# google/deepvariant

Hardware: AMD Instinct MI355X
Metric: candidate pileups/sec (encode+CNN) (higher is better)
Workload: dtype u8 (encoder) / f16 MFMA, f32 accumulate (CNN); 1 GPU; configs[1] shape: synthetic 30x Illumina pileups, WGS 100x221x7, HIP encode + Inception-v3 MFMA on 1 MI355X per rank, random-init weights; parallelism=interval shards x1, all-gather of probs, collective_world_size=1

## Files before the change

deepvariant_amd/csrc/conv_common.h:

```cpp
#ifndef DV_CONV_COMMON_H_
#define DV_CONV_COMMON_H_

#include <hip/hip_runtime.h>

#include <cstddef>
#include <cstdint>

namespace dv {
namespace convk {

typedef _Float16 half8_t __attribute__((ext_vector_type(8)));
typedef _Float16 half4_t __attribute__((ext_vector_type(4)));
typedef float float16_t __attribute__((ext_vector_type(16)));

constexpr int kConvThreads = 256;
constexpr int kChunk = 16;

struct TensorGeom {
  int h, w;
  int halo;
  int hp, wp;
  int groups;
};

struct ConvBranch {
  const float* shift;
  _Float16* out;
  float* out32;
  TensorGeom og;
  int lo_groups;
  int out_goff;
  int Cout;
  int relu;
  int sub0;
  int avgpool;
};

constexpr int kMaxBranches = 4;

struct ConvArgs {
  const _Float16* in;
  const _Float16* w;
  ConvBranch br[kMaxBranches];
  int n_branches;
  TensorGeom ig;
  int N, Cin;
  int OH, OW;
  int KH, KW, stride, pad_h, pad_w;
  int M;
  int n_chunks;
  int n_slabs;
  size_t in_bytes;
  unsigned img_bytes;
  unsigned chunk_stride;
  int n_tiles;
  int band;
  int cu_pair;
  float rcp_ow, rcp_ohow;
  const int* blank_row;
  const _Float16* blank_src;
  const int* blank_need;
  int split;
  int split_tiles;
  _Float16* side_pool_out;
  TensorGeom side_pool_og;
  int side_pool_goff;
  int tile_g, tile_p;
  float rcp_tile_p;
  int wide_in;
  unsigned lo_off;
};

typedef unsigned int uint4_t __attribute__((ext_vector_type(4)));
typedef float float2_t __attribute__((ext_vector_type(2)));
typedef _Float16 half2_t __attribute__((ext_vector_type(2)));

__device__ __forceinline__ void divmod_small(int m, int d, float rcp, int& q, int& r) {
  q = static_cast<int>(static_cast<float>(m) * rcp);
  r = m - q * d;
  if (r < 0) {
    r += d;
    --q;
  }
  if (r >= d) {
    r -= d;
    ++q;
  }
}

__device__ __forceinline__ float avg_finish(float c0, float c1, float c2, float inv, float sh, bool shift_relu) {
#pragma clang fp contract(off)
  const float v = (c0 + c1 + c2) * inv;
  return shift_relu ? fmaxf(v + sh, 0.f) : v;
}

__device__ __forceinline__ void load_shifts(const float* shift, int cbase, int hi, float2_t (&shv)[4][2]) {
#pragma unroll
  for (int q = 0; q < 4; ++q) {
    float4 lo = make_float4(0.f, 0.f, 0.f, 0.f), up = lo;
    if (shift != nullptr) {
      typedef float f4_t __attribute__((ext_vector_type(4)));
      typedef const f4_t __attribute__((address_space(4))) * const_f4_ptr;
      const_f4_ptr sp = (const_f4_ptr)(reinterpret_cast<uintptr_t>(shift + (cbase + 8 * q)));
      const f4_t l4 = sp[0], u4 = sp[1];
      lo = make_float4(l4[0], l4[1], l4[2], l4[3]);
      up = make_float4(u4[0], u4[1], u4[2], u4[3]);
    }
    shv[q][0] = hi ? float2_t{up.x, up.y} : float2_t{lo.x, lo.y};
    shv[q][1] = hi ? float2_t{up.z, up.w} : float2_t{lo.z, lo.w};
  }
}

template <int PT>
__device__ __forceinline__ void epilogue_subtile(const float16_t (&acc)[PT], const ConvBranch& b, int cbase,
                                                 const int (&pn)[PT], const int (&poh)[PT], const int (&pow_)[PT],
                                                 const bool (&mvalid)[PT], int lane) {
  const int hi = lane >> 5;
  const half2_t zero2 = {static_cast<_Float16>(0.f), static_cast<_Float16>(0.f)};
  const unsigned gstride = static_cast<unsigned>(b.og.hp * b.og.wp);
  float2_t shv[4][2];
  load_shifts(b.shift, cbase, hi, shv);
  if (b.out32 != nullptr) {
#pragma unroll
    for (int pt = 0; pt < PT; ++pt) {
      const float16_t a = acc[pt];
      const unsigned obase = static_cast<unsigned>(
          ((pn[pt] * b.og.groups + b.out_goff) * b.og.hp + poh[pt] + b.og.halo) * b.og.wp + pow_[pt] + b.og.halo);
#pragma unroll
      for (int q = 0; q < 4; ++q) {
        float4 v = make_float4(a[4 * q] + shv[q][0][0], a[4 * q + 1] + shv[q][0][1], a[4 * q + 2] + shv[q][1][0],
                               a[4 * q + 3] + shv[q][1][1]);
        if (b.relu) v = make_float4(fmaxf(v.x, 0.f), fmaxf(v.y, 0.f), fmaxf(v.z, 0.f), fmaxf(v.w, 0.f));
        const int group = cbase / 8 + q;
        if (mvalid[pt] && group * 8 < b.Cout) {
          *reinterpret_cast<float4*>(b.out32 + (static_cast<size_t>(obase) + static_cast<size_t>(group) * gstride) * 8 +
                                     4 * hi) = v;
        }
      }
    }
    return;
  }
  uint4_t* outp = reinterpret_cast<uint4_t*>(b.out);
#pragma unroll
  for (int pt = 0; pt < PT; ++pt) {
    const float16_t a = acc[pt];
    const unsigned obase = static_cast<unsigned>(
        ((pn[pt] * b.og.groups + b.out_goff) * b.og.hp + poh[pt] + b.og.halo) * b.og.wp +
        pow_[pt] + b.og.halo);
    unsigned pk[4][2];
    unsigned pl[4][2];
#pragma unroll
    for (int q = 0; q < 4; ++q) {
#pragma unroll
      for (int hq = 0; hq < 2; ++hq) {
        const float2_t v = float2_t{a[4 * q + 2 * hq], a[4 * q + 2 * hq + 1]} + shv[q][hq];
        half2_t h = __builtin_convertvector(v, half2_t);
        if (b.relu) h = __builtin_elementwise_max(h, zero2);
        pk[q][hq] = __builtin_bit_cast(unsigned, h);
        if (b.lo_groups > 0) {
          const float2_t x = b.relu ? float2_t{fmaxf(v[0], 0.f), fmaxf(v[1], 0.f)} : v;
          const float2_t r = x - __builtin_convertvector(h, float2_t);
          pl[q][hq] = __builtin_bit_cast(unsigned, __builtin_convertvector(r, half2_t));
        }
      }
    }
#pragma unroll
    for (int t = 0; t < 2; ++t) {
      const auto d0 = __builtin_amdgcn_permlane32_swap(pk[2 * t][0], pk[2 * t + 1][0], false, false);
      const auto d1 = __builtin_amdgcn_permlane32_swap(pk[2 * t][1], pk[2 * t + 1][1], false, false);
      const uint4_t piece = {d0[0], d1[0], d0[1], d1[1]};
      const int group = cbase / 8 + 2 * t + hi;
#ifdef DV_ABLATE_EPI
      if (mvalid[pt] && group * 8 < b.Cout && piece[0] == 0x7e017e01u) {
#else
      if (mvalid[pt] && group * 8 < b.Cout) {
#endif
        outp[obase + static_cast<unsigned>(group) * gstride] = piece;
      }
      if (b.lo_groups > 0) {
        const auto e0 = __builtin_amdgcn_permlane32_swap(pl[2 * t][0], pl[2 * t + 1][0], false, false);
        const auto e1 = __builtin_amdgcn_permlane32_swap(pl[2 * t][1], pl[2 * t + 1][1], false, false);
        const uint4_t lo_piece = {e0[0], e1[0], e0[1], e1[1]};
        if (mvalid[pt] && group * 8 < b.Cout) {
          outp[obase + static_cast<unsigned>(group + b.lo_groups) * gstride] = lo_piece;
        }
      }
    }
  }
}

__device__ __forceinline__ int branch_of(const ConvArgs& p, int sub) {
  int bi = 0;
#pragma unroll
  for (int i = 1; i < kMaxBranches; ++i) bi += (i < p.n_branches && sub >= p.br[i].sub0) ? 1 : 0;
  return bi;
}

template <int NB, int PT>
__device__ __forceinline__ void conv_epilogue(const float16_t (&acc)[NB][PT], const ConvArgs& p,
                                              int n_tile, const int (&pn)[PT], const int (&poh)[PT],
                                              const int (&pow_)[PT], const bool (&mvalid)[PT],
                                              int lane) {
#pragma unroll
  for (int nb = 0; nb < NB; ++nb) {
    const int sub = n_tile * NB + nb;
    const ConvBranch& b = p.br[branch_of(p, sub)];
    const int cbase = (sub - b.sub0) * 32;
    if (cbase >= b.Cout) continue;
    epilogue_subtile<PT>(acc[nb], b, cbase, pn, poh, pow_, mvalid, lane);
  }
}

__device__ __forceinline__ void avg_pool_group(const float4* src, int y, int x, int H, int W, int lane, float inv,
                                               const float* shift, float (&o)[8]) {
  auto column = [&](int xc, bool wanted, float (&v)[8]) {
    float r[3][8];
#pragma unroll
    for (int dy = 0; dy < 3; ++dy) {
      const int yy = y + dy - 1;
      const bool ok = wanted && yy >= 0 && yy < H;
      float4 lo = make_float4(0.f, 0.f, 0.f, 0.f), up = lo;
      if (ok) {
        lo = src[yy * W + xc];
        up = src[256 + yy * W + xc];
      }
      r[dy][0] = lo.x; r[dy][1] = lo.y; r[dy][2] = lo.z; r[dy][3] = lo.w;
      r[dy][4] = up.x; r[dy][5] = up.y; r[dy][6] = up.z; r[dy][7] = up.w;
    }
#pragma unroll
    for (int j = 0; j < 8; ++j) v[j] = r[0][j] + r[1][j] + r[2][j];
  };
  float col[3][8];
  column(x, true, col[1]);
  const bool first = lane == 0, last = lane == 63;
  const int xe = first ? x - 1 : x + 1;
  float edge[8];
  column(xe, (first || last) && xe >= 0 && xe < W, edge);
#pragma unroll
  for (int j = 0; j < 8; ++j) {
    const int vi = __builtin_bit_cast(int, col[1][j]);
    const float from_left = __builtin_bit_cast(float, __builtin_amdgcn_update_dpp(0, vi, 0x138, 0xf, 0xf, false));
    const float from_right = __builtin_bit_cast(float, __builtin_amdgcn_update_dpp(0, vi, 0x130, 0xf, 0xf, false));
    col[0][j] = x == 0 ? 0.f : first ? edge[j] : from_left;
    col[2][j] = x == W - 1 ? 0.f : last ? edge[j] : from_right;
  }
  float sh[8] = {0, 0, 0, 0, 0, 0, 0, 0};
  if (shift != nullptr) {
    const float4 s0 = *reinterpret_cast<const float4*>(shift);
    const float4 s1 = *reinterpret_cast<const float4*>(shift + 4);
    sh[0] = s0.x; sh[1] = s0.y; sh[2] = s0.z; sh[3] = s0.w;
    sh[4] = s1.x; sh[5] = s1.y; sh[6] = s1.z; sh[7] = s1.w;
  }
#pragma unroll
  for (int j = 0; j < 8; ++j) o[j] = avg_finish(col[0][j], col[1][j], col[2][j], inv, sh[j], shift != nullptr);
}

template <int NB, int PT>
__device__ __forceinline__ void conv_epilogue_avg(const float16_t (&acc)[NB][PT], const ConvArgs& p, int n_tile,
                                                  int pix_block, const int (&pn)[PT], const int (&poh)[PT],
                                                  const int (&pow_)[PT], const bool (&mvalid)[PT], int lane,
                                                  int wave, _Float16* smem) {
  static_assert(PT == 2 && NB % 2 == 0, "256-pixel blocks, subtiles pooled in pairs");
  const int hi = lane >> 5;
  float* tile = reinterpret_cast<float*>(smem);
  const int my_slot = wave * 64 + lane;
  int il, pix, y, x;
  divmod_small(my_slot, p.tile_p, p.rcp_tile_p, il, pix);
  divmod_small(pix, p.OW, p.rcp_ow, y, x);
  const int n = pix_block * p.tile_g + il;
  const bool live = il < p.tile_g && n < p.N;
  const int H = p.OH, W = p.OW;
  const int map0 = il * p.tile_p;
  const float inv = 1.0f / static_cast<float>(((y > 0) + (y < H - 1) + 1) * ((x > 0) + (x < W - 1) + 1));
#pragma unroll
  for (int half = 0; half < NB / 2; ++half) {
    bool any_pooled = false;
#pragma unroll
    for (int nbl = 0; nbl < 2; ++nbl) {
      const int sub = n_tile * NB + 2 * half + nbl;
      const ConvBranch& b = p.br[branch_of(p, sub)];
      const int cbase = (sub - b.sub0) * 32;
      if (cbase >= b.Cout) continue;
      if (b.avgpool == 0) {
        epilogue_subtile<PT>(acc[2 * half + nbl], b, cbase, pn, poh, pow_, mvalid, lane);
      } else {
        any_pooled = true;
      }
    }
    if (!any_pooled) continue;
    __syncthreads();
#pragma unroll
    for (int nbl = 0; nbl < 2; ++nbl) {
      const int sub = n_tile * NB + 2 * half + nbl;
      const ConvBranch& b = p.br[branch_of(p, sub)];
      const int cbase = (sub - b.sub0) * 32;
      if (cbase >= b.Cout || b.avgpool == 0) continue;
#pragma unroll
      for (int pt = 0; pt < PT; ++pt) {
        const float16_t a = acc[2 * half + nbl][pt];
        const int slot = (wave * PT + pt) * 32 + (lane & 31);
#pragma unroll
        for (int q = 0; q < 4; ++q) {
          reinterpret_cast<float4*>(tile)[((nbl * 4 + q) * 2 + hi) * 256 + slot] =
              make_float4(a[4 * q], a[4 * q + 1], a[4 * q + 2], a[4 * q + 3]);
        }
      }
    }
    __syncthreads();
#pragma unroll
    for (int nbl = 0; nbl < 2; ++nbl) {
      const int sub = n_tile * NB + 2 * half + nbl;
      const ConvBranch& b = p.br[branch_of(p, sub)];
      const int cbase = (sub - b.sub0) * 32;
      if (cbase >= b.Cout || b.avgpool == 0 || !live) continue;
      const unsigned gstride = static_cast<unsigned>(b.og.hp * b.og.wp);
      const unsigned obase = static_cast<unsigned>(
          ((n * b.og.groups + b.out_goff) * b.og.hp + y + b.og.halo) * b.og.wp + x + b.og.halo);
      for (int q8 = 0; q8 < 4; ++q8) {
        const int group = cbase / 8 + q8;
        if (group * 8 >= b.Cout) break;
        const float4* src = reinterpret_cast<const float4*>(tile) + (nbl * 4 + q8) * 2 * 256 + map0;
        float o[8];
        avg_pool_group(src, y, x, H, W, lane, inv, b.shift != nullptr ? b.shift + group * 8 : nullptr, o);
        const size_t at = static_cast<size_t>(obase) + static_cast<size_t>(group) * gstride;
        if (b.out32 != nullptr) {
          float4* d = reinterpret_cast<float4*>(b.out32 + at * 8);
          d[0] = make_float4(o[0], o[1], o[2], o[3]);
          d[1] = make_float4(o[4], o[5], o[6], o[7]);
        } else {
          half8_t h;
#pragma unroll
          for (int j = 0; j < 8; ++j) h[j] = static_cast<_Float16>(o[j]);
          reinterpret_cast<uint4_t*>(b.out)[at] = __builtin_bit_cast(uint4_t, h);
          if (b.lo_groups > 0) {
            half8_t l;
#pragma unroll
            for (int j = 0; j < 8; ++j) l[j] = static_cast<_Float16>(o[j] - static_cast<float>(h[j]));
            reinterpret_cast<uint4_t*>(b.out)[at + static_cast<size_t>(b.lo_groups) * gstride] = __builtin_bit_cast(uint4_t, l);
          }
        }
      }
    }
  }
}

}
}

#endif
```

deepvariant_amd/csrc/conv_mfma.hip:

```cpp
#include <algorithm>
#include <cstdlib>
#include <type_traits>

#include "conv_mfma.h"

using namespace dv::convk;

namespace {

constexpr int prefetch_depth(int , int ) { return 4; }

struct ChunkWalk {
  int kh, kw;
  unsigned tap_off;
  unsigned chunk_off;
  __device__ __forceinline__ unsigned off() const { return chunk_off + tap_off; }
  __device__ __forceinline__ void advance(const ConvArgs& p) {
    const bool row_end = ++kw == p.KW;
    kw = row_end ? 0 : kw;
    tap_off += row_end ? static_cast<unsigned>((p.ig.wp - p.KW + 1) * 16) : 16u;
    kh += row_end ? 1 : 0;
    const bool taps_end = kh == p.KH;
    kh = taps_end ? 0 : kh;
    tap_off = taps_end ? 0u : tap_off;
// ... 18 lines not shown
__device__ __forceinline__ void conv_slab(const ConvArgs& p, const __amdgpu_buffer_rsrc_t rsrc,
                                          const _Float16* wslab, ChunkWalk& walk,
                                          const unsigned (&base)[PT],
                                          uint4_t (&xf)[prefetch_depth(NB, PT)][PT],
                                          float16_t (&acc)[NB][PT], SidePool<PT>* sp = nullptr) {
  constexpr int BN = NB * 32;
  constexpr int kPrefetch = prefetch_depth(NB, PT);
  half8_t wf[2][NB];
#pragma unroll
  for (int nb = 0; nb < NB; ++nb) {
    wf[0][nb] = *reinterpret_cast<const half8_t*>(wslab + (nb * 32) * 8);
  }
#pragma unroll
  for (int j = 0; j < R; ++j) {
#ifndef DV_ABLATE_W
    if (j + 1 < R) {
#pragma unroll
      for (int nb = 0; nb < NB; ++nb) {
        wf[(j + 1) & 1][nb] = *reinterpret_cast<const half8_t*>(
            wslab + (j + 1) * BN * kChunk + (nb * 32) * 8);
      }
    }
#else
    if (j + 1 < R) {
#pragma unroll
      for (int nb = 0; nb < NB; ++nb) wf[(j + 1) & 1][nb] = wf[j & 1][nb];
    }
#endif
    __builtin_amdgcn_sched_barrier(0);
    constexpr int kDiv = SPLIT ? 2 : 1;
    const int slot = ((S0 + j) / kDiv) % kPrefetch;
    half8_t xh[PT];
#pragma unroll
    for (int pt = 0; pt < PT; ++pt) xh[pt] = __builtin_bit_cast(half8_t, xf[slot][pt]);
#pragma unroll
    for (int nb = 0; nb < NB; ++nb) {
#pragma unroll
      for (int pt = 0; pt < PT; ++pt) {
        acc[nb][pt] =
            __builtin_amdgcn_mfma_f32_32x32x16_f16(wf[j & 1][nb], xh[pt], acc[nb][pt], 0, 0, 0);
      }
    }
    if constexpr (POOL) {
      if (sp->cc_mod == sp->my_tile) {
#pragma unroll
        for (int pt = 0; pt < PT; ++pt) sp->best[pt] = __builtin_elementwise_max(sp->best[pt], xh[pt]);
      }
      if (sp->tap == sp->taps - 1) {
        if (sp->cc < sp->n_cc && sp->cc_mod == sp->my_tile) {
          const _Float16 lowest = static_cast<_Float16>(-65504.f);
#pragma unroll
          for (int pt = 0; pt < PT; ++pt) {
            if (sp->ok[pt]) sp->out[sp->at[pt]] = __builtin_bit_cast(uint4_t, sp->best[pt]);
            sp->best[pt] = half8_t{lowest, lowest, lowest, lowest, lowest, lowest, lowest, lowest};
          }
        }
#pragma unroll
        for (int pt = 0; pt < PT; ++pt) sp->at[pt] += sp->gstride2;
        sp->tap = 0;
        ++sp->cc;
        sp->cc_mod = sp->cc_mod + 1 == sp->n_tiles ? 0 : sp->cc_mod + 1;
      } else {
        ++sp->tap;
      }
    }
    if (!SPLIT || ((S0 + j) & 1)) {
#ifndef DV_ABLATE_X
      const unsigned soff = walk.off();
#pragma unroll
      for (int pt = 0; pt < PT; ++pt) {
        xf[slot][pt] = __builtin_amdgcn_raw_buffer_load_b128(rsrc, base[pt], soff, 0);
      }
#endif
      walk.advance(p);
    }
    __builtin_amdgcn_sched_barrier(0);
  }
}

template <int NB, int PT, int R>
__device__ __forceinline__ void conv_slab_wide(const ConvArgs& p, const __amdgpu_buffer_rsrc_t rsrc,
                                               const _Float16* wslab, ChunkWalk& walk, const unsigned (&base)[PT],
                                               uint4_t (&xf)[prefetch_depth(NB, PT)][PT], float16_t (&acc)[NB][PT]) {
  constexpr int BN = NB * 32;
  static_assert(prefetch_depth(NB, PT) == 4 && R % 2 == 0, "two (hi, lo) pairs in flight");
  half8_t wf[2][NB];
#pragma unroll
  for (int nb = 0; nb < NB; ++nb) wf[0][nb] = *reinterpret_cast<const half8_t*>(wslab + (nb * 32) * 8);
#pragma unroll
  for (int j = 0; j < R; ++j) {
    if (j + 1 < R) {
#pragma unroll
      for (int nb = 0; nb < NB; ++nb) {
        wf[(j + 1) & 1][nb] = *reinterpret_cast<const half8_t*>(wslab + (j + 1) * BN * kChunk + (nb * 32) * 8);
      }
    }
    __builtin_amdgcn_sched_barrier(0);
#pragma unroll
    for (int part = 0; part < 2; ++part) {
      const int slot = (2 * j + part) & 3;
      half8_t xh[PT];
#pragma unroll
      for (int pt = 0; pt < PT; ++pt) xh[pt] = __builtin_bit_cast(half8_t, xf[slot][pt]);
#pragma unroll
      for (int nb = 0; nb < NB; ++nb) {
#pragma unroll
        for (int pt = 0; pt < PT; ++pt) {
          acc[nb][pt] = __builtin_amdgcn_mfma_f32_32x32x16_f16(wf[j & 1][nb], xh[pt], acc[nb][pt], 0, 0, 0);
        }
      }
      const unsigned soff = walk.off() + (part ? p.lo_off : 0u);
#pragma unroll
      for (int pt = 0; pt < PT; ++pt) xf[slot][pt] = __builtin_amdgcn_raw_buffer_load_b128(rsrc, base[pt], soff, 0);
      if (part) walk.advance(p);
    }
    __builtin_amdgcn_sched_barrier(0);
  }
}

template <int NB, int PT>
__device__ __forceinline__ void copy_blank_wave(const ConvArgs& p, int n_tile, const int (&pn)[PT],
                                                const int (&poh)[PT], const int (&pow_)[PT],
                                                const bool (&mvalid)[PT], int lane) {
  const ConvBranch& b = p.br[0];
  const unsigned gstride = static_cast<unsigned>(b.og.hp * b.og.wp);
  const int hi = lane >> 5;
  const uint4_t* src = reinterpret_cast<const uint4_t*>(p.blank_src);
  uint4_t* dst = reinterpret_cast<uint4_t*>(b.out);
  uint4_t v[PT][NB * 2];
  unsigned at[PT][NB * 2];
  bool ok[PT][NB * 2];
#pragma unroll
  for (int pt = 0; pt < PT; ++pt) {
    const unsigned rel = static_cast<unsigned>((poh[pt] + b.og.halo) * b.og.wp + pow_[pt] + b.og.halo);
#pragma unroll
    for (int j = 0; j < NB * 2; ++j) {
      const int g = n_tile * NB * 4 + 2 * j + hi;
      ok[pt][j] = mvalid[pt] && g * 8 < b.Cout;
      at[pt][j] = static_cast<unsigned>(b.out_goff + g) * gstride + rel;
      v[pt][j] = ok[pt][j] ? src[at[pt][j]] : uint4_t{0u, 0u, 0u, 0u};
    }
  }
#pragma unroll
  for (int pt = 0; pt < PT; ++pt) {
    const unsigned img = static_cast<unsigned>(pn[pt] * b.og.groups) * gstride;
#pragma unroll
    for (int j = 0; j < NB * 2; ++j) {
      if (ok[pt][j]) dst[img + at[pt][j]] = v[pt][j];
    }
  }
}

template <int NB, int PT, int MINB = (NB * PT >= 8 ? 1 : 2), int SLAB = kSlabChunks, int WAVES = 4,
          bool SPLIT = false, bool SIDE_POOL = false, bool AVG = false, bool WIDE = false>
__global__ __launch_bounds__(WAVES * 64, MINB) void conv_mfma_kernel(ConvArgs p) {
  constexpr int BN = NB * 32;
  constexpr int kThreads = WAVES * 64;
  constexpr int SLAB_HALFS = SLAB * BN * kChunk;
  constexpr int SLAB_PIECES = SLAB_HALFS / 8;
  constexpr int W_PER_THREAD = SLAB_PIECES / kThreads;
  static_assert(SLAB_PIECES % kThreads == 0, "slab does not split evenly over the block");
  constexpr int kPrefetch = prefetch_depth(NB, PT);
  extern __shared__ __attribute__((aligned(16))) _Float16 smem[];

  const int tid = threadIdx.x;
  const int lane = tid & 63;
  const int wave = tid >> 6;
  const int nwg = gridDim.x;
  const int xq = nwg >> 3, xr = nwg & 7;
  const int xcd = blockIdx.x & 7;
  int xi = blockIdx.x >> 3;
  if (p.cu_pair) {
    const int cnt = xcd < xr ? xq + 1 : xq;
    if (xi < cnt / 64 * 64) {
      const int w = xi & 63;
      xi = (xi & ~63) + (w & 31) * 2 + (w >> 5);
    }
  }
  const int logical = (xcd < xr ? xcd * (xq + 1) : xr * (xq + 1) + (xcd - xr) * xq) + xi;
  const int n_tile = logical % p.n_tiles;
  int pix_block = logical / p.n_tiles;
  int band_r = 0;
  if (p.band) {
    band_r = pix_block % p.band;
    pix_block /= p.band;
  }
  const int m_block = pix_block * (32 * PT * WAVES);

  int n0 = 0;
  unsigned base[PT];
  int pn[PT], poh[PT], pow_[PT];
  bool mvalid[PT];
  const int ohow = p.OH * p.OW;
#pragma unroll
  for (int pt = 0; pt < PT; ++pt) {
    const int m = m_block + (wave * PT + pt) * 32 + (lane & 31);
    int n, pix, oh, ow, iy;
    if constexpr (AVG) {
      int il;
      divmod_small((wave * PT + pt) * 32 + (lane & 31), p.tile_p, p.rcp_tile_p, il, pix);
      n = pix_block * p.tile_g + il;
      mvalid[pt] = il < p.tile_g && n < p.N;
      n = min(n, p.N - 1);
      divmod_small(pix, p.OW, p.rcp_ow, oh, ow);
      iy = oh * p.stride - p.pad_h + p.ig.halo;
    } else if (p.band) {
      mvalid[pt] = m < p.N * p.OW;
      divmod_small(mvalid[pt] ? m : 0, p.OW, p.rcp_ow, n, ow);
      oh = band_r;
      iy = p.ig.halo;
    } else {
      mvalid[pt] = m < p.M;
      divmod_small(mvalid[pt] ? m : 0, ohow, p.rcp_ohow, n, pix);
      divmod_small(pix, p.OW, p.rcp_ow, oh, ow);
      iy = oh * p.stride - p.pad_h + p.ig.halo;
    }
    const int ix = ow * p.stride - p.pad_w + p.ig.halo;
    if (pt == 0) n0 = __builtin_amdgcn_readfirstlane(n);
    base[pt] = mvalid[pt]
                   ? static_cast<unsigned>(((((n - n0) * p.ig.groups + (lane >> 5)) * p.ig.hp + iy) *
                                                p.ig.wp + ix) * 16)
                   : 0x80000000u;
    pn[pt] = n;
    poh[pt] = oh;
    pow_[pt] = ow;
  }

  bool wave_blank = false;
  if (p.blank_row != nullptr) {
    auto range_blank = [&](int m_lo, int m_hi) -> bool {
      m_hi = min(m_hi, p.M);
      if (m_lo >= m_hi) return false;
      int nf, pf, nl, pl, ohf, owf;
      divmod_small(m_lo, ohow, p.rcp_ohow, nf, pf);
      divmod_small(m_hi - 1, ohow, p.rcp_ohow, nl, pl);
      divmod_small(pf, p.OW, p.rcp_ow, ohf, owf);
      return nf == nl && ohf >= p.blank_row[nf];
    };
    if (range_blank(m_block, m_block + 32 * PT * WAVES)) {
      bool wanted = true;
      if (p.blank_need != nullptr) {
        int nf, pf, ohf, owf;
        divmod_small(m_block, ohow, p.rcp_ohow, nf, pf);
        divmod_small(pf, p.OW, p.rcp_ow, ohf, owf);
        wanted = ohf < p.blank_need[nf];
      }
      if (wanted) copy_blank_wave<NB, PT>(p, n_tile, pn, poh, pow_, mvalid, lane);
      return;
    }
    const int m_wave = m_block + wave * (32 * PT);
    wave_blank = __builtin_amdgcn_readfirstlane(range_blank(m_wave, m_wave + 32 * PT) ? 1 : 0) != 0;
  }

  const size_t in_off = static_cast<size_t>(n0) * p.img_bytes;
  const size_t in_left = p.in_bytes - in_off;
  const __amdgpu_buffer_rsrc_t rsrc = __builtin_amdgcn_make_buffer_rsrc(
      const_cast<char*>(reinterpret_cast<const char*>(p.in) + in_off), 0,
      static_cast<unsigned>(in_left < 0x7fffffffu ? in_left : 0x7fffffffu), 0x00020000);

  const uint4* wsrc = reinterpret_cast<const uint4*>(p.w) +
                      static_cast<size_t>(band_r * p.n_tiles + n_tile) * p.n_slabs * (kSlabChunks * BN * 2);
  uint4_t wreg[W_PER_THREAD];
#define DV_LOAD_SLAB(s_)                                                                   \
  {                                                                                        \
    const uint4_t* src_ = reinterpret_cast<const uint4_t*>(wsrc) +                         \
                          static_cast<size_t>(s_) * SLAB_PIECES + tid;                     \
    _Pragma("unroll") for (int j_ = 0; j_ < W_PER_THREAD; ++j_) wreg[j_] =                \
        src_[j_ * kThreads];                                                           \
  }
#define DV_STORE_SLAB(buf_)                                                                \
  {                                                                                        \
    uint4_t* dst_ = reinterpret_cast<uint4_t*>(smem + (buf_) * SLAB_HALFS) + tid;          \
    _Pragma("unroll") for (int j_ = 0; j_ < W_PER_THREAD; ++j_) dst_[j_ * kThreads] = \
        wreg[j_];                                                                          \
  }

  uint4_t xf[kPrefetch][PT];
  float16_t acc[NB][PT];
#pragma unroll
  for (int nb = 0; nb < NB; ++nb)
#pragma unroll
    for (int pt = 0; pt < PT; ++pt)
#pragma unroll
      for (int i = 0; i < 16; ++i) acc[nb][pt][i] = 0.f;

  ChunkWalk walk{0, 0, 0u, 0u};
  DV_LOAD_SLAB(0)
#pragma unroll
  for (int d = 0; d < kPrefetch; ++d) {
    const unsigned soff = walk.off() + (WIDE && (d & 1) ? p.lo_off : 0u);
#pragma unroll
    for (int pt = 0; pt < PT; ++pt) {
      xf[d][pt] = __builtin_amdgcn_raw_buffer_load_b128(rsrc, base[pt], soff, 0);
    }
    if (!WIDE || (d & 1)) walk.advance(p);
  }
  DV_STORE_SLAB(0)
  __syncthreads();

  const int frag_off = (lane >> 5) * (BN * 8) + (lane & 31) * 8;
  if (wave_blank) {
    const int n_full_b = p.n_chunks / SLAB;
    for (int s = 0; s < n_full_b; ++s) {
      const int next = s + 1 < (p.n_chunks + SLAB - 1) / SLAB ? s + 1 : s;
      DV_LOAD_SLAB(next)
      DV_STORE_SLAB((s + 1) & 1)
      __syncthreads();
    }
    copy_blank_wave<NB, PT>(p, n_tile, pn, poh, pow_, mvalid, lane);
    return;
  }
  SidePool<PT> side;
  auto k_loop = [&](auto split_tag, auto pool_tag, const int n_chunks) {
    constexpr bool S = decltype(split_tag)::value;
    constexpr bool P = decltype(pool_tag)::value;
    SidePool<PT>* const sp = P ? &side : nullptr;
    const int tile_slabs = (n_chunks + SLAB - 1) / SLAB;
#ifdef DV_ABLATE_LOOP
    const int n_full = n_chunks < 0 ? 1 : 0;
    const int rem = 0;
#else
    const int n_full = n_chunks / SLAB;
    const int rem = n_chunks - n_full * SLAB;
#endif
    for (int s = 0; s < n_full; ++s) {
      const int next = s + 1 < tile_slabs ? s + 1 : s;
      DV_LOAD_SLAB(next)
      if constexpr (WIDE) {
        conv_slab_wide<NB, PT, SLAB>(p, rsrc, smem + (s & 1) * SLAB_HALFS + frag_off, walk, base, xf, acc);
      } else {
        conv_slab<NB, PT, SLAB, 0, S, P>(p, rsrc, smem + (s & 1) * SLAB_HALFS + frag_off, walk, base, xf, acc, sp);
      }
      DV_STORE_SLAB((s + 1) & 1)
      __syncthreads();
    }
    if (rem) {
      const _Float16* wslab = smem + (n_full & 1) * SLAB_HALFS + frag_off;
      if constexpr (WIDE) {
        conv_slab_wide<NB, PT, 4>(p, rsrc, wslab, walk, base, xf, acc);
        if constexpr (SLAB > 4) {
          if (rem > 4) conv_slab_wide<NB, PT, 4>(p, rsrc, wslab + 4 * BN * kChunk, walk, base, xf, acc);
        }
      } else {
      conv_slab<NB, PT, 4, 0, S, P>(p, rsrc, wslab, walk, base, xf, acc, sp);
      if constexpr (SLAB > 4) {
        if (rem > 4) conv_slab<NB, PT, 4, 4, S, P>(p, rsrc, wslab + 4 * BN * kChunk, walk, base, xf, acc, sp);
      }
      }
    }
  };
  if constexpr (SPLIT) {
    if (n_tile < p.split_tiles) {
      k_loop(std::true_type{}, std::false_type{}, p.n_chunks);
    } else {
      k_loop(std::false_type{}, std::false_type{}, p.n_chunks >> 1);
    }
  } else if constexpr (SIDE_POOL) {
    side.tap = 0;
    side.cc = 0;
    side.cc_mod = 0;
    side.n_tiles = p.n_tiles;
    side.my_tile = n_tile;
    side.taps = p.KH * p.KW;
    side.n_cc = p.Cin / kChunk;
    side.gstride2 = 2u * static_cast<unsigned>(p.side_pool_og.hp * p.side_pool_og.wp);
    side.out = reinterpret_cast<uint4_t*>(p.side_pool_out);
#pragma unroll
    for (int pt = 0; pt < PT; ++pt) {
      const _Float16 lowest = static_cast<_Float16>(-65504.f);
      side.best[pt] = half8_t{lowest, lowest, lowest, lowest, lowest, lowest, lowest, lowest};
      side.ok[pt] = mvalid[pt];
      side.at[pt] = static_cast<unsigned>(
          ((pn[pt] * p.side_pool_og.groups + p.side_pool_goff + (lane >> 5)) * p.side_pool_og.hp + poh[pt] +
           p.side_pool_og.halo) * p.side_pool_og.wp + pow_[pt] + p.side_pool_og.halo);
    }
    k_loop(std::false_type{}, std::true_type{}, p.n_chunks);
  } else {
    k_loop(std::false_type{}, std::false_type{}, p.n_chunks);
  }
#undef DV_LOAD_SLAB
#undef DV_STORE_SLAB

  if constexpr (AVG) {
    conv_epilogue_avg<NB, PT>(acc, p, n_tile, pix_block, pn, poh, pow_, mvalid, lane, wave, smem);
  } else {
    conv_epilogue<NB, PT>(acc, p, n_tile, pn, poh, pow_, mvalid, lane);
  }
}

template <int NB, int PT>
__global__ __launch_bounds__(512, 1) void conv_resident_kernel(ConvArgs p) {
  constexpr int BN = NB * 32;
  constexpr int WAVES = 8, kThreads = WAVES * 64;
  constexpr int SLAB_HALFS = kSlabChunks * BN * kChunk;
  constexpr int kPrefetch = prefetch_depth(NB, PT);
  extern __shared__ __attribute__((aligned(16))) _Float16 smem[];
  const int tid = threadIdx.x, lane = tid & 63, wave = tid >> 6;
  const int blk = blockIdx.x;
  const int n_tile = (blk >> 3) % p.n_tiles;
  const int seq = (blk & 7) + 8 * ((blk >> 3) / p.n_tiles);
  const int n_seq = 8 * ((static_cast<int>(gridDim.x) >> 3) / p.n_tiles);
  {
    const uint4_t* wsrc = reinterpret_cast<const uint4_t*>(p.w) +
                          static_cast<size_t>(n_tile) * p.n_slabs * (kSlabChunks * BN * 2);
    uint4_t* wdst = reinterpret_cast<uint4_t*>(smem);
    const int pieces = p.n_slabs * (kSlabChunks * BN * 2);
    for (int i = tid; i < pieces; i += kThreads) wdst[i] = wsrc[i];
  }
  __syncthreads();
  const int frag_off = (lane >> 5) * (BN * 8) + (lane & 31) * 8;
  const int ohow = p.OH * p.OW;
  const int n_full = p.n_chunks / kSlabChunks;
  const int rem = p.n_chunks - n_full * kSlabChunks;
  const int n_wave_tiles = (p.M + 32 * PT - 1) / (32 * PT);
  for (int wt = seq * WAVES + wave; wt < n_wave_tiles; wt += n_seq * WAVES) {
    int n0 = 0;
    unsigned base[PT];
    int pn[PT], poh[PT], pow_[PT];
    bool mvalid[PT];
#pragma unroll
    for (int pt = 0; pt < PT; ++pt) {
      const int m = (wt * PT + pt) * 32 + (lane & 31);
      int n, pix, oh, ow;
      mvalid[pt] = m < p.M;
      divmod_small(mvalid[pt] ? m : 0, ohow, p.rcp_ohow, n, pix);
      divmod_small(pix, p.OW, p.rcp_ow, oh, ow);
      const int iy = oh * p.stride - p.pad_h + p.ig.halo;
      const int ix = ow * p.stride - p.pad_w + p.ig.halo;
      if (pt == 0) n0 = __builtin_amdgcn_readfirstlane(n);
      base[pt] = mvalid[pt]
                     ? static_cast<unsigned>(((((n - n0) * p.ig.groups + (lane >> 5)) * p.ig.hp + iy) *
                                                  p.ig.wp + ix) * 16)
                     : 0x80000000u;
      pn[pt] = n;
      poh[pt] = oh;
      pow_[pt] = ow;
    }
    const size_t in_off = static_cast<size_t>(n0) * p.img_bytes;
    const size_t in_left = p.in_bytes - in_off;
    const __amdgpu_buffer_rsrc_t rsrc = __builtin_amdgcn_make_buffer_rsrc(
        const_cast<char*>(reinterpret_cast<const char*>(p.in) + in_off), 0,
        static_cast<unsigned>(in_left < 0x7fffffffu ? in_left : 0x7fffffffu), 0x00020000);
    uint4_t xf[kPrefetch][PT];
    float16_t acc[NB][PT];
#pragma unroll
    for (int nb = 0; nb < NB; ++nb)
#pragma unroll
      for (int pt = 0; pt < PT; ++pt)
#pragma unroll
        for (int i = 0; i < 16; ++i) acc[nb][pt][i] = 0.f;
    ChunkWalk walk{0, 0, 0u, 0u};
#pragma unroll
    for (int d = 0; d < kPrefetch; ++d) {
      const unsigned soff = walk.off();
#pragma unroll
      for (int pt = 0; pt < PT; ++pt) {
        xf[d][pt] = __builtin_amdgcn_raw_buffer_load_b128(rsrc, base[pt], soff, 0);
      }
      walk.advance(p);
    }
    for (int s = 0; s < n_full; ++s) {
      conv_slab<NB, PT, kSlabChunks>(p, rsrc, smem + s * SLAB_HALFS + frag_off, walk, base, xf, acc);
    }
    if (rem) {
      const _Float16* wslab = smem + n_full * SLAB_HALFS + frag_off;
      conv_slab<NB, PT, 4>(p, rsrc, wslab, walk, base, xf, acc);
      if (rem > 4) conv_slab<NB, PT, 4, 4>(p, rsrc, wslab + 4 * BN * kChunk, walk, base, xf, acc);
    }
    conv_epilogue<NB, PT>(acc, p, n_tile, pn, poh, pow_, mvalid, lane);
  }
}

template <int NB, int PT>
__device__ __forceinline__ void resident_rows(const ConvArgs& p, const __amdgpu_buffer_rsrc_t rsrc,
                                              const _Float16* wfrag, const unsigned (&base)[PT],
                                              float16_t (&acc)[NB][PT]) {
  constexpr int BN = NB * 32;
  constexpr int SLAB_HALFS = kSlabChunks * BN * kChunk;
  constexpr int kPrefetch = prefetch_depth(NB, PT);
  const int n_full = p.n_chunks / kSlabChunks;
  const int rem = p.n_chunks - n_full * kSlabChunks;
  uint4_t xf[kPrefetch][PT];
#pragma unroll
  for (int nb = 0; nb < NB; ++nb)
#pragma unroll
    for (int pt = 0; pt < PT; ++pt)
#pragma unroll
      for (int i = 0; i < 16; ++i) acc[nb][pt][i] = 0.f;
  ChunkWalk walk{0, 0, 0u, 0u};
#pragma unroll
  for (int d = 0; d < kPrefetch; ++d) {
    const unsigned soff = walk.off();
#pragma unroll
    for (int pt = 0; pt < PT; ++pt) xf[d][pt] = __builtin_amdgcn_raw_buffer_load_b128(rsrc, base[pt], soff, 0);
    walk.advance(p);
  }
  for (int s = 0; s < n_full; ++s) {
    conv_slab<NB, PT, kSlabChunks>(p, rsrc, wfrag + s * SLAB_HALFS, walk, base, xf, acc);
  }
  if (rem) {
    const _Float16* wslab = wfrag + n_full * SLAB_HALFS;
    conv_slab<NB, PT, 4>(p, rsrc, wslab, walk, base, xf, acc);
    if (rem > 4) conv_slab<NB, PT, 4, 4>(p, rsrc, wslab + 4 * BN * kChunk, walk, base, xf, acc);
  }
}

template <int NB>
__device__ __forceinline__ void pack_row(const float16_t (&acc)[NB], const ConvArgs& p, int n_tile, int hi,
                                         unsigned (&pk)[NB][4][2]) {
  const ConvBranch& b = p.br[0];
  const half2_t zero2 = {static_cast<_Float16>(0.f), static_cast<_Float16>(0.f)};
#pragma unroll
  for (int nb = 0; nb < NB; ++nb) {
    const int cbase = (n_tile * NB + nb) * 32;
#pragma unroll
    for (int q = 0; q < 4; ++q) {
      typedef float f4_t __attribute__((ext_vector_type(4)));
      typedef const f4_t __attribute__((address_space(4))) * const_f4_ptr;
      const_f4_ptr sp = (const_f4_ptr)(reinterpret_cast<uintptr_t>(b.shift + (cbase + 8 * q)));
      const f4_t l4 = sp[0], u4 = sp[1];
      const float2_t s0 = hi ? float2_t{u4[0], u4[1]} : float2_t{l4[0], l4[1]};
      const float2_t s1 = hi ? float2_t{u4[2], u4[3]} : float2_t{l4[2], l4[3]};
      const float2_t v0 = float2_t{acc[nb][4 * q], acc[nb][4 * q + 1]} + s0;
      const float2_t v1 = float2_t{acc[nb][4 * q + 2], acc[nb][4 * q + 3]} + s1;
      pk[nb][q][0] = __builtin_bit_cast(unsigned, __builtin_elementwise_max(__builtin_convertvector(v0, half2_t), zero2));
      pk[nb][q][1] = __builtin_bit_cast(unsigned, __builtin_elementwise_max(__builtin_convertvector(v1, half2_t), zero2));
    }
  }
}

__device__ __forceinline__ unsigned pk_max(unsigned a, unsigned b) {
  return __builtin_bit_cast(unsigned, __builtin_elementwise_max(__builtin_bit_cast(half2_t, a),
                                                                __builtin_bit_cast(half2_t, b)));
}

template <int NB>
__global__ __launch_bounds__(512, 1) void conv_pool_resident_kernel(ConvArgs p) {
  constexpr int BN = NB * 32;
  constexpr int WAVES = 8, kThreads = WAVES * 64;
// ... 192 lines not shown
    for (int i = 0; i < 16; ++i) acc[nb][0][i] = 0.f;

  half8_t win[2][9];
#define DV_LOAD_WINDOW(slot_, cc_)                                                          \
  {                                                                                         \
    const unsigned so_ = static_cast<unsigned>(cc_) * p.chunk_stride;                       \
    _Pragma("unroll") for (int t_ = 0; t_ < 9; ++t_) win[slot_][t_] = __builtin_bit_cast(  \
        half8_t, __builtin_amdgcn_raw_buffer_load_b128(rsrc, base,                          \
                                                       so_ + (t_ / 3) * row_b + (t_ % 3) * 16, 0)); \
  }
  DV_LOAD_WINDOW(0, 0)
  __syncthreads();
  const _Float16* wfrag = smem + (lane >> 5) * (BN * 8) + (lane & 31) * 8;
  for (int cc = 0; cc < p.n_chunks; cc += 2) {
    if (cc + 1 < p.n_chunks) DV_LOAD_WINDOW(1, cc + 1)
#pragma unroll
    for (int half = 0; half < 2; ++half) {
      if (half == 1) {
        if (cc + 1 >= p.n_chunks) break;
        if (cc + 2 < p.n_chunks) DV_LOAD_WINDOW(0, cc + 2)
      }
      half8_t x = win[half][0];
#pragma unroll
      for (int t = 1; t < 9; ++t) x = __builtin_elementwise_max(x, win[half][t]);
      const _Float16* wc = wfrag + (cc + half) * (BN * kChunk);
#pragma unroll
      for (int nb = 0; nb < NB; ++nb) {
        const half8_t wf = *reinterpret_cast<const half8_t*>(wc + nb * 32 * 8);
        acc[nb][0] = __builtin_amdgcn_mfma_f32_32x32x16_f16(wf, x, acc[nb][0], 0, 0, 0);
      }
    }
  }
#undef DV_LOAD_WINDOW
  conv_epilogue<NB, PT>(acc, p, n_tile, pn, poh, pow_, mvalid, lane);
}

template <int NB>
constexpr size_t conv_lds_bytes() {
  return static_cast<size_t>(2) * kSlabChunks * NB * 32 * kChunk * 2;
}

void launch_conv6(const ConvArgs& a, hipStream_t stream) {
  const long rows = a.band ? a.band : 1;
  const long row_px = a.band ? static_cast<long>(a.N) * a.OW : a.M;
  const long blocks = rows * ((row_px + 127) / 128) * a.n_tiles;
  constexpr size_t lds = static_cast<size_t>(2) * 4 * 192 * kChunk * 2;
  if (a.wide_in) {
    hipLaunchKernelGGL((conv_mfma_kernel<6, 1, 2, 4, 4, false, false, false, true>), dim3(static_cast<unsigned>(blocks)),
                       dim3(kConvThreads), lds, stream, a);
    return;
  }
  hipLaunchKernelGGL((conv_mfma_kernel<6, 1, 2, 4>), dim3(static_cast<unsigned>(blocks)), dim3(kConvThreads), lds,
                     stream, a);
}

template <int NB>
void launch_conv(const ConvArgs& a, hipStream_t stream) {
  const int n_tiles = a.n_tiles;
  const long rows = a.band ? a.band : 1;
  const long row_px = a.band ? static_cast<long>(a.N) * a.OW : a.M;
  auto blocks = [&](int px) { return rows * ((row_px + px - 1) / px) * n_tiles; };
  const long blocks2 = blocks(256);
  if constexpr (NB == 4) {
    if (a.side_pool_out != nullptr) {
      if (blocks2 >= 512) {
        hipLaunchKernelGGL((conv_mfma_kernel<NB, 2, 2, kSlabChunks, 4, false, true>), dim3(static_cast<unsigned>(blocks2)),
                           dim3(kConvThreads), conv_lds_bytes<NB>(), stream, a);
      } else {
        hipLaunchKernelGGL((conv_mfma_kernel<NB, 1, 2, kSlabChunks, 4, false, true>), dim3(static_cast<unsigned>(blocks(128))),
                           dim3(kConvThreads), conv_lds_bytes<NB>(), stream, a);
      }
      return;
    }
  }
  if (a.wide_in) {
    if constexpr (NB >= 2 && NB <= 4) {
      if constexpr (NB == 4) {
        if (a.tile_g > 0) {
          const long tiles = (static_cast<long>(a.N) + a.tile_g - 1) / a.tile_g * n_tiles;
          hipLaunchKernelGGL((conv_mfma_kernel<NB, 2, 2, kSlabChunks, 4, false, false, true, true>),
                             dim3(static_cast<unsigned>(tiles)), dim3(kConvThreads), conv_lds_bytes<NB>(), stream, a);
          return;
        }
      }
      if (blocks2 >= 512) {
        hipLaunchKernelGGL((conv_mfma_kernel<NB, 2, 2, kSlabChunks, 4, false, false, false, true>),
                           dim3(static_cast<unsigned>(blocks2)), dim3(kConvThreads), conv_lds_bytes<NB>(), stream, a);
      } else {
        hipLaunchKernelGGL((conv_mfma_kernel<NB, 1, 2, kSlabChunks, 4, false, false, false, true>),
                           dim3(static_cast<unsigned>(blocks(128))), dim3(kConvThreads), conv_lds_bytes<NB>(), stream, a);
      }
      return;
    }
  }
  if constexpr (NB == 4) {
    if (a.tile_g > 0) {
      const long tiles = (static_cast<long>(a.N) + a.tile_g - 1) / a.tile_g * n_tiles;
      hipLaunchKernelGGL((conv_mfma_kernel<NB, 2, 2, kSlabChunks, 4, false, false, true>),
                         dim3(static_cast<unsigned>(tiles)), dim3(kConvThreads), conv_lds_bytes<NB>(), stream, a);
      return;
    }
  }
  if (a.split) {
    static const long pt2_min = getenv("DV_SPLIT_PT2_MIN") ? atol(getenv("DV_SPLIT_PT2_MIN")) : 256;
    if (blocks2 >= pt2_min) {
      hipLaunchKernelGGL((conv_mfma_kernel<NB, 2, 2, kSlabChunks, 4, true>), dim3(static_cast<unsigned>(blocks2)),
                         dim3(kConvThreads), conv_lds_bytes<NB>(), stream, a);
    } else {
      hipLaunchKernelGGL((conv_mfma_kernel<NB, 1, 2, kSlabChunks, 4, true>), dim3(static_cast<unsigned>(blocks(128))),
                         dim3(kConvThreads), conv_lds_bytes<NB>(), stream, a);
    }
    return;
  }
  static const int force_pt = getenv("DV_CONV_PT") ? atoi(getenv("DV_CONV_PT")) : 0;
  static const bool no_pt4 = getenv("DV_NO_PT4") != nullptr;
  if constexpr (NB <= 2) {
    if (!no_pt4 && !force_pt && blocks2 >= 4096 && (NB == 1 || a.KH * a.KW >= 25)) {
      hipLaunchKernelGGL((conv_mfma_kernel<NB, 4>), dim3(static_cast<unsigned>(blocks(512))),
                         dim3(kConvThreads), conv_lds_bytes<NB>(), stream, a);
      return;
    }
  }
  static const bool slab4 = getenv("DV_CONV_SLAB4") != nullptr;
  static const bool w8 = getenv("DV_CONV_W8") != nullptr;
  if constexpr (NB >= 3 && NB <= 4) {
    if (slab4 && blocks2 >= 512) {
      hipLaunchKernelGGL((conv_mfma_kernel<NB, 2, 2, 4>), dim3(static_cast<unsigned>(blocks2)),
                         dim3(kConvThreads), static_cast<size_t>(2) * 4 * NB * 32 * kChunk * 2, stream, a);
      return;
    }
    if (w8 && blocks2 >= 1024) {
      hipLaunchKernelGGL((conv_mfma_kernel<NB, 2, 1, kSlabChunks, 8>), dim3(static_cast<unsigned>(blocks(512))),
                         dim3(512), conv_lds_bytes<NB>(), stream, a);
      return;
    }
  }
  if (force_pt ? force_pt == 2 : blocks2 >= 512) {
    if constexpr (NB == 4) {
      static const bool two = getenv("DV_CONV42_BLOCKS") == nullptr || atoi(getenv("DV_CONV42_BLOCKS")) != 1;
      if (two) {
        hipLaunchKernelGGL((conv_mfma_kernel<NB, 2, 2>), dim3(static_cast<unsigned>(blocks2)),
                           dim3(kConvThreads), conv_lds_bytes<NB>(), stream, a);
        return;
      }
    }
    hipLaunchKernelGGL((conv_mfma_kernel<NB, 2>), dim3(static_cast<unsigned>(blocks2)),
                       dim3(kConvThreads), conv_lds_bytes<NB>(), stream, a);
  } else {
    hipLaunchKernelGGL((conv_mfma_kernel<NB, 1>), dim3(static_cast<unsigned>(blocks(128))),
                       dim3(kConvThreads), conv_lds_bytes<NB>(), stream, a);
  }
}

}
namespace dv {
namespace convk {


template <typename K>
static void allow_big_lds(K kernel) {
  (void)hipFuncSetAttribute(reinterpret_cast<const void*>(kernel), hipFuncAttributeMaxDynamicSharedMemorySize, 160 * 1024);
}

void launch_conv_pool_resident(const ConvArgs& a, int n_cus, hipStream_t stream) {
  static const bool attr = (allow_big_lds(conv_pool_resident_kernel<3>), true);
  (void)attr;
  const long frags = (static_cast<long>(a.N) * a.OW + 29) / 30;
  const int per_set = 8 * a.n_tiles;
  const long want = (frags + 8 * 8 - 1) / (8 * 8) * per_set;
  const int grid = static_cast<int>(std::max<long>(per_set, std::min<long>(want, n_cus / per_set * per_set)));
  hipLaunchKernelGGL((conv_pool_resident_kernel<3>), dim3(grid), dim3(512), resident_lds_bytes(a), stream, a);
}

void launch_conv_pool1x1(const ConvArgs& a, int nb, hipStream_t stream) {
  const size_t lds = static_cast<size_t>(a.n_slabs) * kSlabChunks * nb * 32 * kChunk * 2;
  const dim3 grid(static_cast<unsigned>(((a.M + 127) / 128) * a.n_tiles));
  switch (nb) {
    case 7: {
      static const bool attr = (allow_big_lds(conv_pool1x1_kernel<7, 8>), true);
      (void)attr;
      hipLaunchKernelGGL((conv_pool1x1_kernel<7, 8>), dim3(static_cast<unsigned>((a.M + 255) / 256)), dim3(512), lds, stream, a);
      break;
    }
    case 1: hipLaunchKernelGGL((conv_pool1x1_kernel<1>), grid, dim3(kConvThreads), lds, stream, a); break;
    case 2: hipLaunchKernelGGL((conv_pool1x1_kernel<2>), grid, dim3(kConvThreads), lds, stream, a); break;
    case 3: hipLaunchKernelGGL((conv_pool1x1_kernel<3>), grid, dim3(kConvThreads), lds, stream, a); break;
    default: hipLaunchKernelGGL((conv_pool1x1_kernel<4>), grid, dim3(kConvThreads), lds, stream, a); break;
  }
}

void launch_conv_resident(const ConvArgs& a, int n_cus, hipStream_t stream) {
  static const bool attr = (allow_big_lds(conv_resident_kernel<3, 2>), true);
  (void)attr;
  const int grid = n_cus / (8 * a.n_tiles) * (8 * a.n_tiles);
  hipLaunchKernelGGL((conv_resident_kernel<3, 2>), dim3(grid), dim3(512), resident_lds_bytes(a), stream, a);
}

void launch_conv(const ConvArgs& a, int nb, hipStream_t stream) {
  switch (nb) {
    case 1: ::launch_conv<1>(a, stream); break;
    case 2: ::launch_conv<2>(a, stream); break;
    case 3: ::launch_conv<3>(a, stream); break;
    case 6: launch_conv6(a, stream); break;
    default: ::launch_conv<4>(a, stream); break;
  }
}

}
}
```

deepvariant_amd/csrc/model.hip:

```cpp
#include <algorithm>
#include <map>
#include <atomic>
#include <cmath>
#include <cstdlib>
#include <cstring>
#include <memory>
#include <thread>

#include <hip/hip_fp16.h>

#include "model_graph.h"
#include "model_kernels.h"
#include "block35.h"
#include "mixed3.h"
#include "chain.h"
#include "stem_fused.h"
#include "calib.h"
#include "layer_export.h"

namespace {

static int stem_sub_batch() {
  static const int v = getenv("DV_STEM_SB") ? std::max(1, atoi(getenv("DV_STEM_SB"))) : (1 << 30);
  return v;
}

ExtPtrs* ext_table(const dv_model* m) { return static_cast<ExtPtrs*>(m->d_ext.ptr); }

struct OpTrace {
  hipEvent_t a, b;
  std::string label;
  double flops, bytes;
};
std::vector<OpTrace>* g_trace = nullptr;

struct TraceScope {
  hipStream_t stream;
  bool on;
  TraceScope(hipStream_t s, std::string label, double flops, double bytes) : stream(s), on(g_trace != nullptr) {
    if (!on) return;
    OpTrace t{nullptr, nullptr, std::move(label), flops, bytes};
    (void)hipEventCreate(&t.a);
    (void)hipEventCreate(&t.b);
    (void)hipEventRecord(t.a, stream);
    g_trace->push_back(std::move(t));
  }
  ~TraceScope() {
    if (on) (void)hipEventRecord(g_trace->back().b, stream);
  }
};

void dump_trace(hipStream_t stream) {
  (void)hipStreamSynchronize(stream);
  double tot = 0;
  for (OpTrace& t : *g_trace) {
    float ms = 0;
    (void)hipEventElapsedTime(&ms, t.a, t.b);
    tot += ms;
    fprintf(stderr, "[dv-op] %-58s %8.1f us %7.1f TF/s %7.0f GB/s\n", t.label.c_str(), ms * 1e3,
            t.flops / (ms * 1e-3) / 1e12, t.bytes / (ms * 1e-3) / 1e9);
    (void)hipEventDestroy(t.a);
    (void)hipEventDestroy(t.b);
  }
  fprintf(stderr, "[dv-op] total %.1f us\n", tot * 1e3);
  g_trace->clear();
}

bool resident_ok(const dv_model* m, const Op& op, const ConvArgs& a) {
  const char* env = getenv("DV_RESIDENT");
  const int mode = env ? atoi(env) : 1;
  if (mode == 0 || op.nb != 3 || op.band || op.v2 || op.pool_in || op.split || a.blank_row != nullptr || a.wide_in) return false;
  if (resident_lds_bytes(a) > 150 * 1024 || m->n_cus < 8 * a.n_tiles) return false;
  static const long min_tiles = getenv("DV_RESIDENT_MIN_TILES") ? atol(getenv("DV_RESIDENT_MIN_TILES")) : 4;
  if (static_cast<long>(a.M) < static_cast<long>(m->n_cus) * 8 * 64 * min_tiles) return false;
  if (mode >= 2) return true;
  return m->blank_conv4_op >= 0 && &op == &m->ops[m->blank_conv4_op];
}

struct Pass {
  dv_model* m;
  int n;
  hipStream_t stream;
  int first, last;
  int shifted_buf, out_example_off;
  size_t images_off;
  std::vector<char> side_pooled;
  _Float16* out_ptr(int buf) const {
    const size_t halfs = static_cast<size_t>(out_example_off) * m->buffers[buf].bytes_per_example() / 2;
    return m->buf_ptr(buf) + (buf == shifted_buf ? halfs : 0);
  }
};

dv::C8Geom c8_geom(const BufferDesc& b) {
  const TensorGeom g = b.geom();
  return dv::C8Geom{g.h, g.w, g.halo, g.hp, g.wp, g.groups};
}


int enqueue_stem_a(const Pass& ps, int oi) {
  const dv_model* m = ps.m;
  const int n = ps.n;
  const Op &op = m->ops[oi], &c2 = m->ops[oi + 1];
  dv::StemAArgs a{};
  a.in = nullptr;
  a.in_ind = &ext_table(m)->images;
  a.in_off = ps.images_off;
  a.w1 = m->w_ptr(op);
  a.w2 = m->w_ptr(c2);
  a.shift1 = m->shift_ptr(op);
  a.shift2 = m->shift_ptr(c2);
  a.out = m->buf_ptr(c2.out_buf);
  a.og = c8_geom(m->buffers[c2.out_buf]);
  a.N = n;
  a.H = op.ih;
  a.W = op.iw;
  a.C = op.cin_real;
  a.OH1 = op.oh;
  a.OW1 = op.ow;
  a.OH2 = c2.oh;
  a.OW2 = c2.ow;
  a.tiles_y = (c2.oh + dv::kStemA_TH - 1) / dv::kStemA_TH;
  a.tiles_x = (c2.ow + dv::kStemA_TW - 1) / dv::kStemA_TW;
  a.total_tiles = n * a.tiles_y * a.tiles_x;
  a.in_bytes = static_cast<unsigned>(static_cast<size_t>(n) * op.ih * op.iw * op.cin_real);
  if (m->blank_on()) {
    a.blank_thr = m->blank_thr(1);
    a.blank_src = static_cast<const _Float16*>(m->d_blank_c2.ptr);
    a.blank_need = m->blank_thr(5);
  }
  TraceScope tr(ps.stream, std::string(m->blank_on() ? "[blank tiles copied] " : "") + "stem_a conv3x3s2 " + std::to_string(op.cin_real) + "->32 + conv3x3 32->32 (fused)",
                2.0 * n * (static_cast<double>(op.oh) * op.ow * op.kh * op.kw * op.cin_real * op.cout +
                           static_cast<double>(c2.oh) * c2.ow * 9 * 32 * 32),
                static_cast<double>(n) * (op.ih * op.iw * op.cin_real + 2.0 * c2.oh * c2.ow * 32));
  dv::ProfileScope prof(dv::kProfConv, ps.stream);
  dv::launch_stem_a(a, m->stem_a_grid, ps.stream);
  return 2;
}

void report_stem_b_profile(dv::StemBArgs a, int grid, hipStream_t stream) {
  const size_t words = static_cast<size_t>(grid) * 16;
  unsigned long long* d = nullptr;
  if (hipMalloc(&d, words * 8) != hipSuccess) return;
  (void)hipMemsetAsync(d, 0, words * 8, stream);
  a.prof = d;
  dv::launch_stem_b(a, grid, stream);
  std::vector<unsigned long long> h(words);
  (void)hipStreamSynchronize(stream);
  (void)hipMemcpy(h.data(), d, words * 8, hipMemcpyDeviceToHost);
  (void)hipFree(d);
  for (int w = 0; w < 2; ++w) {
    double sum[7] = {0, 0, 0, 0, 0, 0, 0};
    for (int b = 0; b < grid; ++b)
      for (int i = 0; i < 7; ++i) sum[i] += static_cast<double>(h[(b * 2 + w) * 8 + i]);
    const double tiles = static_cast<double>(a.total_tiles);
    fprintf(stderr, "[dv-stem-b wave %d] cycles/tile: issue %.0f conv3 %.0f dma-wait %.0f barrierA %.0f pool %.0f "
                    "barrierB %.0f conv1x1+store %.0f\n", w ? 7 : 0, sum[0] / tiles, sum[1] / tiles,
            sum[6] / tiles, sum[2] / tiles, sum[3] / tiles, sum[4] / tiles, sum[5] / tiles);
  }
  std::map<unsigned long long, std::vector<int>> where;
  for (int b = 0; b < grid; ++b) {
    const unsigned long long v = h[(b * 2) * 8 + 7];
    const unsigned hw = static_cast<unsigned>(v), xcc = static_cast<unsigned>(v >> 32);
    where[(static_cast<unsigned long long>(xcc) << 16) | ((hw >> 8) & 0xffu)].push_back(b);
  }
  int pairs = 0, same_parity = 0, apart256 = 0;
  for (const auto& kv : where) {
    if (kv.second.size() != 2) continue;
    ++pairs;
    const unsigned t0 = (static_cast<unsigned>(h[(kv.second[0] * 2) * 8 + 7]) >> 16) & 15u;
    const unsigned t1 = (static_cast<unsigned>(h[(kv.second[1] * 2) * 8 + 7]) >> 16) & 15u;
    same_parity += (t0 & 1u) == (t1 & 1u);
    apart256 += kv.second[1] - kv.second[0] == 256;
  }
  fprintf(stderr, "[dv-stem-b placement] %zu places for %d workgroups; %d pairs, %d with TG slots of EQUAL parity, "
                  "%d pairs are blocks b / b+256\n", where.size(), grid, pairs, same_parity, apart256);
  for (int cls = 0; cls < 2; ++cls) {
    double sum[7] = {0, 0, 0, 0, 0, 0, 0};
    int nb = 0;
    for (int b = 0; b < grid; ++b) {
      const unsigned tg = (static_cast<unsigned>(h[(b * 2) * 8 + 7]) >> 16) & 15u;
      if (static_cast<int>(tg & 1u) != cls) continue;
      ++nb;
      for (int i = 0; i < 7; ++i) sum[i] += static_cast<double>(h[(b * 2) * 8 + i]);
    }
    double tot = 0;
    for (double v : sum) tot += v;
    fprintf(stderr, "[dv-stem-b TG parity %d] %d workgroups, share of wave-0 cycles: issue %.3f conv3 %.3f dma-wait %.3f "
                    "barrierA %.3f pool %.3f barrierB %.3f conv1x1+store %.3f; cycles per workgroup %.0f\n", cls, nb,
            sum[0] / tot, sum[1] / tot, sum[6] / tot, sum[2] / tot, sum[3] / tot, sum[4] / tot, sum[5] / tot,
            nb ? tot / nb : 0.0);
  }
}

int enqueue_stem_b(const Pass& ps, int oi) {
  const dv_model* m = ps.m;
  const int n = ps.n;
  const Op &op = m->ops[oi], &c4 = m->ops[oi + 1];
  const BufferDesc& ib = m->buffers[op.in_buf];
  dv::StemBArgs a{};
  a.in = m->buf_ptr(op.in_buf);
  a.w3 = m->w_ptr(op);
  a.w4 = m->w_ptr(c4);
  a.shift3 = m->shift_ptr(op);
  a.shift4 = m->shift_ptr(c4);
  a.out = m->buf_ptr(c4.out_buf);
  a.ig = c8_geom(ib);
  a.og = c8_geom(m->buffers[c4.out_buf]);
  a.N = n;
  a.OH3 = op.oh;
  a.OW3 = op.ow;
  a.PH = c4.oh;
  a.PW = c4.ow;
  a.Cout4 = c4.cout;
  a.tiles_y = (c4.oh + dv::kStemB_PH - 1) / dv::kStemB_PH;
  a.tiles_x = (c4.ow + dv::kStemB_PW - 1) / dv::kStemB_PW;
  a.total_tiles = n * a.tiles_y * a.tiles_x;
  a.in_bytes = static_cast<size_t>(n) * ib.bytes_per_example();
  a.in_img_bytes = static_cast<unsigned>(ib.bytes_per_example());
  if (m->blank_on()) {
    a.blank_thr = m->blank_thr(2);
    a.blank_src = static_cast<const _Float16*>(m->d_blank_b.ptr);
    a.blank_need = m->blank_thr(6);
  }
  TraceScope tr(ps.stream, std::string(m->blank_on() ? "[blank tiles copied] " : "") + "stem_b conv3x3 32->64 + maxpool3s2 + conv1x1 64->" + std::to_string(c4.cout) + " (fused)",
                2.0 * n * (static_cast<double>(op.oh) * op.ow * 9 * 32 * 64 +
                           static_cast<double>(c4.oh) * c4.ow * 64 * c4.cout),
                2.0 * n * (static_cast<double>(op.ih) * op.iw * 32 + static_cast<double>(c4.oh) * c4.ow * c4.cout));
  dv::ProfileScope prof(dv::kProfConv, ps.stream);
  static const bool stem_prof = getenv("DV_STEM_PROF") != nullptr;
  if (stem_prof && g_trace != nullptr) {
    report_stem_b_profile(a, m->stem_b_grid, ps.stream);
  } else {
    dv::launch_stem_b(a, m->stem_b_grid, ps.stream);
  }
  return 2;
}

int enqueue_block35(const Pass& ps, int oi) {
  const dv_model* m = ps.m;
// ... 128 lines not shown
                    "lds epilogue %.0f hbm epilogue %.0f set-up %.0f\n", w, sum[0] / tiles, sum[1] / tiles,
            sum[2] / tiles, sum[3] / tiles, sum[4] / tiles, sum[5] / tiles);
  }
}

int enqueue_chain(const Pass& ps, int oi) {
  const dv_model* m = ps.m;
  const int n = ps.n;
  const Op& op = m->ops[oi];
  const Op& last = m->ops[oi + op.chain_len - 1];
  const BufferDesc& ib = m->buffers[op.in_buf];
  dv::ChainArgs a{};
  a.in = m->buf_ptr(op.in_buf);
  a.ig = ib.geom();
  a.in_img_bytes = static_cast<unsigned>(ib.bytes_per_example());
  a.N = n;
  a.G = op.chain_g;
  a.tpx = op.chain_tpx;
  a.h = op.oh;
  a.w = op.ow;
  a.n_tiles = (n + a.G - 1) / a.G;
  a.n_layers = op.chain_len;
  double tr_flops = 0;
  std::string tr_label = "chain";
  size_t act = 0, slot = 0;
  for (int k = 0; k < op.chain_len; ++k) {
    const Op& o = m->ops[oi + k];
    dv::ChainLayer& cl = a.L[k];
    cl.w = m->w_ptr(o);
    cl.shift = m->shift_ptr(o);
    cl.n_chunks = o.cin / kChunk;
    cl.cout = o.cout;
    cl.cout_pad = (o.cout + 31) / 32 * 32;
    cl.kh = o.kh;
    cl.kw = o.kw;
    cl.slab_bytes = static_cast<unsigned>(o.kh * o.kw * 2 * cl.cout_pad * 16);
    act = std::max(act, static_cast<size_t>(o.cin / 8) * op.chain_tpx * 16);
    slot = std::max(slot, static_cast<size_t>(cl.slab_bytes));
    tr_flops += 2.0 * n * o.oh * o.ow * o.kh * o.kw * o.cin * o.cout;
    tr_label += " " + std::to_string(o.kh) + "x" + std::to_string(o.kw) + ":" + std::to_string(o.cin) + "->" +
                std::to_string(o.cout);
  }
  a.act_bytes = static_cast<unsigned>(act);
  a.slot_bytes = static_cast<unsigned>(slot);
  a.out = m->buf_ptr(last.out_buf);
  a.og = m->buffers[last.out_buf].geom();
  a.out_goff = last.out_coff / 8;
  tr_label += " @" + std::to_string(op.oh) + "x" + std::to_string(op.ow) + " [fused, G=" + std::to_string(a.G) + "]";
  TraceScope tr(ps.stream, tr_label, tr_flops,
                2.0 * n * op.oh * op.ow * (static_cast<double>(op.cin) + last.cout));
  dv::ProfileScope prof(dv::kProfConv, ps.stream);
  static const bool chain_prof = getenv("DV_CHAIN_PROF") != nullptr;
  if (chain_prof && g_trace != nullptr) {
    report_chain_profile(a, m->n_cus, ps.stream);
  } else {
    dv::launch_chain(a, m->n_cus, ps.stream);
  }
  return op.chain_len;
}

int enqueue_first_conv(const Pass& ps, int oi) {
  const dv_model* m = ps.m;
  const int n = ps.n;
  const Op& op = m->ops[oi];
  FirstConvArgs f{};
  f.ext = ext_table(m);
  f.in_off = ps.images_off;
  f.w = m->w_ptr(op);
  f.shift = m->shift_ptr(op);
  f.out = ps.out_ptr(op.out_buf);
  f.og = m->buffers[op.out_buf].geom();
  f.N = n;
  f.H = op.ih;
  f.W = op.iw;
  f.C = op.cin_real;
  f.Cout = op.cout;
  f.OH = op.oh;
  f.OW = op.ow;
  f.KH = op.kh;
  f.KW = op.kw;
  f.stride = op.stride;
  f.M = n * op.oh * op.ow;
  f.n_chunks = op.n_chunks;
  f.wide = op.cin_real > 8 ? 1 : 0;
  f.in_bytes = static_cast<unsigned>(static_cast<size_t>(n) * op.ih * op.iw * op.cin_real);
  f.rcp_ow = 1.0f / static_cast<float>(op.ow);
  f.rcp_ohow = 1.0f / static_cast<float>(op.oh * op.ow);
  TraceScope tr(ps.stream, "conv_first_u8 3x3 s2 " + std::to_string(op.cin_real) + "->" + std::to_string(op.cout),
                2.0 * f.M * op.kh * op.kw * op.cin_real * op.cout,
                static_cast<double>(n) * (op.ih * op.iw * op.cin_real + 2.0 * op.oh * op.ow * op.cout));
  dv::ProfileScope prof(dv::kProfConv, ps.stream);
  launch_conv_first_u8(f, ps.stream);
  return 1;
}

void set_branch_output(const Pass& ps, const Op& o, ConvBranch& br) {
  const BufferDesc& b = ps.m->buffers[o.out_buf];
  br.out = ps.out_ptr(o.out_buf);
  br.out32 = b.f32 ? ps.m->buf_ptr<float>(o.out_buf) : nullptr;
  br.og = b.geom();
  br.lo_groups = b.wide ? b.c / 8 : 0;
  br.out_goff = o.out_coff / 8;
}

int enqueue_conv(Pass& ps, int oi) {
  const dv_model* m = ps.m;
  const int n = ps.n;
  const Op& op = m->ops[oi];
  ConvArgs a{};
  a.in = m->buf_ptr(op.in_buf);
  const BufferDesc& ib = m->buffers[op.in_buf];
  a.ig = ib.geom();
  a.N = n;
  a.Cin = op.cin;
  a.OH = op.oh;
  a.OW = op.ow;
  static const int cu_pair = getenv("DV_CU_PAIR") ? atoi(getenv("DV_CU_PAIR")) : 0;
  a.cu_pair = cu_pair;
  a.band = op.band;
  a.KH = op.band ? op.band : op.kh;
  a.KW = op.kw;
  a.stride = op.stride;
  a.pad_h = op.pad_h;
  a.pad_w = op.pad_w;
  a.chunk_stride = static_cast<unsigned>(2 * a.ig.hp * a.ig.wp * 16);
  a.M = n * op.oh * op.ow;
  a.n_chunks = op.n_chunks;
  a.n_slabs = op.n_steps;
  a.split = op.split ? 1 : 0;
  a.split_tiles = op.split_tiles;
  a.wide_in = op.in_wide ? 1 : 0;
  a.lo_off = op.in_wide ? static_cast<unsigned>(ib.c / 8) * static_cast<unsigned>(a.ig.hp * a.ig.wp) * 16u : 0u;
  a.in_bytes = static_cast<size_t>(n) * ib.bytes_per_example();
  a.img_bytes = static_cast<unsigned>(ib.bytes_per_example());
  a.rcp_ow = 1.0f / static_cast<float>(op.ow);
  a.rcp_ohow = 1.0f / static_cast<float>(op.oh * op.ow);
  int subs = 0;
  a.n_branches = 0;
  double tr_flops = 0, tr_bytes = static_cast<double>(n) * op.ih * op.iw * op.cin * 2.0;
  std::string tr_label = "conv " + std::to_string(op.kh) + "x" + std::to_string(op.kw) + " s" +
                         std::to_string(op.stride) + " " + std::to_string(op.cin) + "->";
  for (int gi = 0; gi <= op.group_followers; ++gi) {
    const Op& bo = m->ops[oi + gi];
    tr_flops += 2.0 * n * op.oh * op.ow * op.kh * op.kw * op.cin_real * bo.cout;
    tr_bytes += 2.0 * n * op.oh * op.ow * bo.cout;
    tr_label += (gi ? "+" : "") + std::to_string(bo.cout);
    ConvBranch& br = a.br[a.n_branches++];
    br.shift = bo.raw ? nullptr : m->shift_ptr(bo);
    set_branch_output(ps, bo, br);
    br.Cout = bo.cout;
    br.relu = bo.raw ? 0 : 1;
    br.sub0 = subs;
    subs += (bo.cout + 31) / 32;
    if (op.avg_tile_g > 0 && bo.avg_partner >= 0 && bo.avg_partner < ps.last) {
      const Op& pl = m->ops[bo.avg_partner];
      br.avgpool = 1;
      br.shift = m->shift_ptr(pl);
      br.relu = 1;
      set_branch_output(ps, pl, br);
      a.tile_g = op.avg_tile_g;
      a.tile_p = op.oh * op.ow;
      a.rcp_tile_p = 1.0f / static_cast<float>(a.tile_p);
    }
  }
  if (a.tile_g > 0) tr_label += " [+ avgpool3s1 in the epilogue, " + std::to_string(a.tile_g) + " maps per block]";
  a.w = m->w_ptr(op);
  const int tiles = (subs + op.nb - 1) / op.nb;
  a.n_tiles = tiles;
  if (m->blank_on() && m->blank_conv4_op >= 0 && &op == &m->ops[m->blank_conv4_op] &&
      a.n_branches == 1 && !op.band && !op.v2 && !op.pool_in) {
    a.blank_row = m->blank_thr(op.pool_out ? 4 : 3);
    a.blank_src = static_cast<const _Float16*>(m->d_blank_conv4.ptr);
    tr_label += " [blank rows copied]";
  }
  if (m->blank_on() && oi == 1 && !m->ops[0].stem_a && a.n_branches == 1 && !op.band && !op.v2 && !op.pool_in &&
      !op.pool_out && !op.split && op.nb <= 4 && m->d_blank_c2.ptr != nullptr) {
    a.blank_row = m->blank_thr(1);
    a.blank_src = static_cast<const _Float16*>(m->d_blank_c2.ptr);
    if (m->ops[2].stem_b) a.blank_need = m->blank_thr(5);
    tr_label += " [blank rows copied]";
  }
  const int oi_last = oi + op.group_followers;
  tr_label += " @" + std::to_string(op.oh) + "x" + std::to_string(op.ow) + " nb" + std::to_string(op.nb) +
              " tiles" + std::to_string(tiles);
  if (op.pool_in) tr_label += " <- maxpool3s2";
  if (op.in_wide) tr_label += " [hi+lo input: 2 MFMAs per weight fragment]";
  if (op.v2) tr_label += " [imgconv G=" + std::to_string(op.v2_g) + "]";
  if (op.band) tr_label += " [band: " + std::to_string(op.band) + " of " + std::to_string(op.kh) + " tap rows]";
  if (op.split) tr_label += " [split W: " + std::to_string(op.split_tiles) + " of " + std::to_string(tiles) + " tiles]";
  if (op.side_pool_partner > oi_last && op.side_pool_partner < ps.last && op.nb == 4 && !resident_ok(m, op, a)) {
    const Op& pl = m->ops[op.side_pool_partner];
    a.side_pool_out = m->buf_ptr(pl.out_buf);
    a.side_pool_og = m->buffers[pl.out_buf].geom();
    a.side_pool_goff = pl.out_coff / 8;
    ps.side_pooled[op.side_pool_partner] = 1;
    tr_label += " + maxpool3s2 on the side";
    tr_bytes += 2.0 * n * pl.oh * pl.ow * pl.cin;
  }
  const bool resident = !op.v2 && !op.pool_in && !op.pool_out && resident_ok(m, op, a);
  if (resident) tr_label += " [weights resident in LDS]";
  if (op.pool_out) tr_label += " [weights resident in LDS] -> maxpool3s2";
  TraceScope tr(ps.stream, tr_label, tr_flops, tr_bytes);
  dv::ProfileScope prof(dv::kProfConv, ps.stream);
  if (op.pool_out) {
    launch_conv_pool_resident(a, m->n_cus, ps.stream);
  } else if (op.v2) {
    dv::ImgConvArgs ia = m->imgconv_geometry(op, op.v2_g);
    ia.c = a;
    ia.n_img_tiles = (n + op.v2_g - 1) / op.v2_g;
    ia.n_cout_tiles = op.v2_tiles;
    dv::launch_imgconv(ia, op.nb, m->n_cus, ps.stream);
  } else if (op.pool_in) {
    a.stride = 2;
    launch_conv_pool1x1(a, op.nb, ps.stream);
  } else if (resident) {
    launch_conv_resident(a, m->n_cus, ps.stream);
  } else {
    launch_conv(a, op.nb, ps.stream);
  }
  return op.group_followers + 1;
}

int enqueue_pool(const Pass& ps, int oi) {
  const dv_model* m = ps.m;
  const int n = ps.n;
  const Op& op = m->ops[oi];
  const BufferDesc &ib = m->buffers[op.in_buf], &ob = m->buffers[op.out_buf];
  PoolArgs p{};
  p.in = m->buf_ptr(op.in_buf);
  p.in32 = m->buf_ptr<float>(op.in_buf);
  p.out = ps.out_ptr(op.out_buf);
  p.out32 = ob.f32 ? m->buf_ptr<float>(op.out_buf) : nullptr;
  p.lo_in_groups = ib.wide ? ib.c / 8 : 0;
  p.lo_out_groups = ob.wide ? ob.c / 8 : 0;
  p.ig = ib.geom();
  p.og = ob.geom();
  p.N = n;
  p.C = op.cin;
  p.OH = op.oh;
  p.OW = op.ow;
  p.out_goff = op.out_coff / 8;
  p.shift = op.pool_shift_relu ? m->shift_ptr(op) : nullptr;
  TraceScope tr(ps.stream, std::string(op.type == kOpMaxPool ? "maxpool3s2 " : "avgpool3s1 ") +
                               std::to_string(op.cin) + " @" + std::to_string(op.oh) + "x" + std::to_string(op.ow),
                0.0, 2.0 * n * op.cin * (static_cast<double>(op.ih) * op.iw + op.oh * op.ow));
  dv::ProfileScope prof(dv::kProfOther, ps.stream);
  if (op.type == kOpMaxPool) {
    if (ib.f32 || ob.f32) return dv::fail(DV_ERR_UNSUPPORTED, "max-pool of a float32 tensor");
    launch_maxpool3s2(p, ps.stream);
  } else {
    if (!ib.f32) return dv::fail(DV_ERR_UNSUPPORTED, "average pool of an fp16 tensor");
    launch_avgpool3s1(p, ps.stream);
  }
  return 1;
}

int run_ops(dv_model* m, int first, int last, int n, hipStream_t stream,
            int shifted_buf = -1, int out_example_off = 0, size_t images_off = 0) {
  Pass ps{m, n, stream, first, last, shifted_buf, out_example_off, images_off, std::vector<char>(m->ops.size(), 0)};
  for (int oi = first; oi < last;) {
    const Op& op = m->ops[oi];
    int ran = 1;
    if (ps.side_pooled[oi]) {
    } else if (op.type == kOpAvgPool && op.avg_partner >= 0 && m->ops[op.avg_partner].avg_partner == oi &&
               op.avg_partner >= first) {
    } else if (op.type != kOpConv) {
      ran = enqueue_pool(ps, oi);
    } else if (op.stem_a) {
      ran = enqueue_stem_a(ps, oi);
    } else if (op.stem_b) {
      ran = enqueue_stem_b(ps, oi);
    } else if (op.b35 == 1) {
      ran = enqueue_block35(ps, oi);
    } else if (op.m3 == 1) {
      ran = enqueue_mixed3(ps, oi);
    } else if (op.chain_len > 0) {
      ran = enqueue_chain(ps, oi);
    } else if (op.first_u8) {
      ran = enqueue_first_conv(ps, oi);
    } else {
      ran = enqueue_conv(ps, oi);
    }
    if (ran < 0) return ran;
    oi += ran;
  }
  DV_HIP_CHECK(hipGetLastError());
  return DV_OK;
}

}

extern "C" {

int dv_model_create(const dv_model_desc* desc, int device, dv_model** out) {
  if (!desc || !out) return dv::fail(DV_ERR_INVALID_ARGUMENT, "dv_model_create: null");
  if (desc->channels < 1 || desc->channels > 16 || desc->num_classes < 1 ||
      desc->num_classes > 8 || desc->max_batch < 1 || desc->max_batch > 8192 ||
      desc->height < 75 ||
      desc->width < 75) {
    return dv::fail(DV_ERR_INVALID_ARGUMENT,
                    "dv_model_create: unsupported shape (need H,W >= 75, C <= 16, max_batch <= 8192)");
  }
  int n_dev = 0;
  if (hipGetDeviceCount(&n_dev) != hipSuccess || n_dev <= 0) {
    return dv::fail(DV_ERR_NO_DEVICE, "no HIP device: libdvhip has no CPU fallback");
  }
  if (device < 0 || device >= n_dev) {
    return dv::fail(DV_ERR_INVALID_ARGUMENT, "bad device ordinal");
  }
  DV_HIP_CHECK(hipSetDevice(device));
  std::unique_ptr<dv_model> m(new dv_model());
  m->device = device;
  m->desc = *desc;
  m->precise = getenv("DV_PRECISE") != nullptr ? atoi(getenv("DV_PRECISE")) != 0 : desc->channels > 8;
  m->build();
  m->stem_a_grid = dv::stem_a_blocks(device);
  m->stem_b_grid = dv::stem_b_blocks(device);
  m->n_cus = dv::stem_a_blocks(device) / 2;
  for (const Op& op : m->ops) {
    const BufferDesc& ob = m->buffers[op.out_buf];
    const double pieces = static_cast<double>(desc->max_batch) * ob.bytes_per_example() / 16.0;
    const double pixels = static_cast<double>(desc->max_batch) * op.oh * op.ow;
    if (pieces >= 2147483648.0 || pixels >= 67108864.0) {
      return dv::fail(DV_ERR_INVALID_ARGUMENT,
                      "dv_model_create: max_batch too large for this image size (N*OH*OW must stay "
                      "below 2^26 and every activation tensor below 2^31 16-byte pieces)");
    }
  }
  if (static_cast<double>(desc->max_batch) * desc->height * desc->width * desc->channels >=
      2147483648.0) {
    return dv::fail(DV_ERR_INVALID_ARGUMENT, "dv_model_create: max_batch * H * W * C must be < 2^31");
  }
  m->dbuf.resize(m->buffers.size());
  for (size_t i = 0; i < m->buffers.size(); ++i) {
    const BufferDesc& b = m->buffers[i];
    const bool stem_buf = static_cast<int>(i) < m->stem_out_buf;
    const size_t examples = std::max(
        static_cast<size_t>(stem_buf ? std::min(desc->max_batch, stem_sub_batch()) : desc->max_batch),
        static_cast<size_t>(b.min_examples));
    const size_t bytes = examples * b.bytes_per_example() +
                         static_cast<size_t>(8) * (b.h + 2 * b.halo) * (b.w + 2 * b.halo) * 16;
    if (int rc = m->dbuf[i].reserve(bytes)) return rc;
    DV_HIP_CHECK(hipMemset(m->dbuf[i].ptr, 0, m->dbuf[i].cap));
  }
  if (int rc = m->d_w.reserve(m->packed_halfs * 2)) return rc;
  if (int rc = m->d_shift.reserve(m->shift_floats * 4)) return rc;
  if (int rc = m->d_dense_w.reserve(static_cast<size_t>(m->feat_c) * desc->num_classes * 4)) return rc;
  if (int rc = m->d_dense_b.reserve(desc->num_classes * 4)) return rc;
  if (int rc = m->d_ext.reserve(sizeof(ExtPtrs))) return rc;
  if (!(getenv("DV_BLANK_SKIP") != nullptr && atoi(getenv("DV_BLANK_SKIP")) == 0) &&
      m->ops[0].first_u8 && m->blank_conv4_op >= 0 && m->ops[m->blank_conv4_op].group_followers == 0 &&
      (static_cast<size_t>(desc->height) * desc->width * desc->channels) % 4 == 0) {
    if (int rc = m->d_blank_thr.reserve(static_cast<size_t>(7) * desc->max_batch * sizeof(int))) return rc;
    DV_HIP_CHECK(hipMemset(m->d_blank_thr.ptr, 0, m->d_blank_thr.cap));
    m->blank_skip = true;
  }
  *out = m.release();
  return DV_OK;
}

void dv_model_destroy(dv_model* m) {
  if (!m) return;
  (void)hipSetDevice(m->device);
  for (auto& b : m->dbuf) b.release();
  m->d_w.release();
  m->d_shift.release();
  m->d_dense_w.release();
  m->d_dense_b.release();
  m->d_tbl.release();
  m->d_blank_thr.release();
  m->d_ext.release();
  m->d_blank_conv4.release();
  m->d_blank_c2.release();
  m->d_blank_b.release();
  for (auto& g : m->graphs) (void)hipGraphExecDestroy(g.exec);
  delete m;
}

int64_t dv_model_num_params(const dv_model* m) { return m ? m->n_params : 0; }

int64_t dv_model_conv_macs(const dv_model* m) {
  if (!m) return 0;
  int64_t macs = 0;
  for (const Op& op : m->ops) {
    if (op.type == kOpConv) {
      macs += static_cast<int64_t>(op.kh) * op.kw * op.cin_real * op.cout * op.oh * op.ow;
    }
  }
  return macs;
}

int dv_model_num_layers(const dv_model* m) {
  return m ? static_cast<int>(m->layers.size()) : 0;
}

int dv_model_layer_info(const dv_model* m, int layer, int32_t* kh, int32_t* kw,
                        int32_t* cin, int32_t* cout, int64_t* param_offset) {
  if (!m || layer < 0 || layer >= static_cast<int>(m->layers.size())) {
    return dv::fail(DV_ERR_INVALID_ARGUMENT, "dv_model_layer_info: bad layer");
  }
  const LayerInfo& l = m->layers[layer];
  if (kh) *kh = l.kh;
  if (kw) *kw = l.kw;
  if (cin) *cin = l.cin;
  if (cout) *cout = l.cout;
  if (param_offset) *param_offset = l.param_off;
  return DV_OK;
}

struct HeadOutputs {
  float* pooled;
  float* logits;
};
static int enqueue_forward(dv_model* m, int n, hipStream_t stream, const HeadOutputs* head_out = nullptr);
static void set_ext(dv_model* m, const uint8_t* images, float* probs, hipStream_t stream,
                    const int32_t* rows_hint = nullptr, int rows_add = 0) {
  launch_set_ext(ext_table(m), images, probs, rows_hint, rows_add, stream);
}

static int prepare_blank_responses(dv_model* m) {
  m->blank_ready = false;
  if (!m->blank_skip) return DV_OK;
  for (auto& g : m->graphs) {
    (void)hipStreamSynchronize(g.stream);
    (void)hipGraphExecDestroy(g.exec);
  }
  m->graphs.clear();
  const size_t img_bytes = static_cast<size_t>(m->desc.height) * m->desc.width * m->desc.channels;
  dv::DeviceBuffer zero_img, probs;
  int rc = zero_img.reserve(img_bytes);
  if (rc == DV_OK) rc = probs.reserve(sizeof(float) * m->desc.num_classes);
  if (rc == DV_OK && hipMemset(zero_img.ptr, 0, img_bytes) != hipSuccess) rc = dv::fail(DV_ERR_HIP, "hipMemset");
  if (rc == DV_OK) {
    set_ext(m, static_cast<const uint8_t*>(zero_img.ptr), static_cast<float*>(probs.ptr), nullptr);
    rc = enqueue_forward(m, 1, nullptr);
  }
  if (rc == DV_OK && hipDeviceSynchronize() != hipSuccess) rc = dv::fail(DV_ERR_HIP, "blank forward failed");
  auto keep = [&](int buf, dv::DeviceBuffer* dst) {
    if (rc != DV_OK || buf < 0 || m->buffers[buf].h <= 1) return;
    const size_t bytes = m->buffers[buf].bytes_per_example();
    rc = dst->reserve(bytes);
    if (rc == DV_OK && hipMemcpy(dst->ptr, m->dbuf[buf].ptr, bytes, hipMemcpyDeviceToDevice) != hipSuccess) {
      rc = dv::fail(DV_ERR_HIP, "copying the blank response");
    }
  };
  keep(m->ops[m->blank_conv4_op].out_buf, &m->d_blank_conv4);
  keep(m->ops[1].out_buf, &m->d_blank_c2);
  if (m->ops[2].stem_b) keep(m->ops[3].out_buf, &m->d_blank_b);
  zero_img.release();
  probs.release();
  if (rc != DV_OK) return rc;
  m->blank_ready = true;
  return DV_OK;
}

int dv_model_load_weights(dv_model* m, const float* weights, int64_t n) {
  if (!m || !weights) return dv::fail(DV_ERR_INVALID_ARGUMENT, "dv_model_load_weights: null");
  if (n != m->n_params) {
    return dv::fail(DV_ERR_INVALID_ARGUMENT,
                    "dv_model_load_weights: expected " + std::to_string(m->n_params) +
                        " values, got " + std::to_string(n));
  }
  DV_HIP_CHECK(hipSetDevice(m->device));
  std::vector<_Float16> packed(m->packed_halfs, static_cast<_Float16>(0.f));
  std::vector<float> shift(m->shift_floats, 0.f);
  for (const Op& op : m->ops) {
    if (op.type != kOpConv) continue;
    const LayerInfo& l = m->layers[op.layer];
    const float* var = weights + l.param_off + static_cast<size_t>(l.kh) * l.kw * l.cin * l.cout + 2 * l.cout;
    for (int co = 0; co < l.cout; ++co) {
      if (!(var[co] + 1e-3f > 0.f)) return dv::fail(DV_ERR_BAD_INPUT, "non-positive BatchNorm variance");
    }
  }
  auto pack_op = [&](size_t oi) {
    const Op& op = m->ops[oi];
    if (op.type != kOpConv) return;
    const LayerInfo& l = m->layers[op.layer];
    const float* w = weights + l.param_off;
    const size_t wn = static_cast<size_t>(l.kh) * l.kw * l.cin * l.cout;
    const float* beta = w + wn;
    const float* mean = beta + l.cout;
    const float* var = mean + l.cout;
    std::vector<float> inv(l.cout);
    for (int co = 0; co < l.cout; ++co) {
      inv[co] = 1.0f / std::sqrt(var[co] + 1e-3f);
      shift[op.shift_off + co] = beta[co] - mean[co] * inv[co];
    }
    if ((m->ops[0].stem_a && oi < 2) || (m->ops[2].stem_b && (oi == 2 || oi == 3))) {
      _Float16* dst = packed.data() + op.w_off;
      if (oi == 0 && l.cin > 8) dv::pack_stem_a_w1_wide(w, inv.data(), l.cin, dst);
      if (oi == 0 && l.cin <= 8) dv::pack_stem_a_w1(w, inv.data(), l.cin, dst);
      if (oi == 1) dv::pack_stem_a_w2(w, inv.data(), dst);
      if (oi == 2) dv::pack_stem_b_w3(w, inv.data(), dst);
      if (oi == 3) dv::pack_stem_b_w4(w, inv.data(), l.cout, dst);
      return;
    }
    if (op.first_u8) {
      const bool wide = l.cin > 8;
      for (int kc = 0; kc < op.n_chunks; ++kc)
        for (int g = 0; g < 2; ++g) {
          const int tap = wide ? kc : 2 * kc + g;
          if (tap >= op.kh * op.kw) continue;
          const int kh = tap / op.kw, kw = tap % op.kw;
          for (int co = 0; co < op.cout; ++co)
            for (int ci = wide ? 8 * g : 0; ci < (wide ? std::min(l.cin, 8 * g + 8) : l.cin); ++ci) {
              const float v = w[((static_cast<size_t>(kh) * l.kw + kw) * l.cin + ci) * l.cout + co];
              packed[op.w_off + ((static_cast<size_t>(kc) * 2 + g) * 32 + co) * 8 + (ci & 7)] =
                  static_cast<_Float16>(v * inv[co]);
            }
        }
      return;
    }
    if (op.b35 >= 1 && op.b35 <= 4) {
      const int pass = op.b35 == 1 || op.b35 == 4 ? 1 : 0, base = op.b35 == 1 || op.b35 == 2 ? 0 : 64;
      const int n_chunks = l.cin / kChunk;
      _Float16* dst = packed.data() + op.w_off;
      for (int cc = 0; cc < n_chunks; ++cc)
        for (int co = 0; co < op.cout; ++co)
          for (int jj = 0; jj < kChunk; ++jj) {
            const float v = w[static_cast<size_t>(cc * kChunk + jj) * l.cout + co];
            dst[(((static_cast<size_t>(pass) * n_chunks + cc) * 2 + jj / 8) * 128 + base + co) * 8 + (jj % 8)] =
                static_cast<_Float16>(v * inv[co]);
          }
      return;
    }
    if (op.m3 == 1) {
      _Float16* dst = packed.data() + op.w_off;
      for (int cc = 0; cc < l.cin / kChunk; ++cc)
        for (int co = 0; co < op.cout; ++co)
          for (int jj = 0; jj < kChunk; ++jj) {
            const float v = w[static_cast<size_t>(cc * kChunk + jj) * l.cout + co];
            dst[((static_cast<size_t>(cc) * 2 + jj / 8) * dv::kMixed3Red + co) * 8 + (jj % 8)] = static_cast<_Float16>(v * inv[co]);
          }
      return;
    }
    if (op.chain_len > 0 || op.in_chain || op.b35 >= 5 || op.m3 >= 2) {
      const int cout_pad = (op.cout + 31) / 32 * 32, taps = op.kh * op.kw;
      _Float16* dst = packed.data() + op.w_off;
      for (int cc = 0; cc < l.cin / kChunk; ++cc)
        for (int tap = 0; tap < taps; ++tap) {
          const int kh = tap / op.kw, kw = tap % op.kw;
          for (int co = 0; co < op.cout; ++co)
            for (int jj = 0; jj < kChunk; ++jj) {
              const int ci = cc * kChunk + jj;
              const float v = w[((static_cast<size_t>(kh) * l.kw + kw) * l.cin + ci) * l.cout + co];
              dst[(((static_cast<size_t>(cc) * taps + tap) * 2 + jj / 8) * cout_pad + co) * 8 + (jj % 8)] =
                  static_cast<_Float16>(v * inv[co]);
            }
        }
      return;
    }
    int sub0 = 0;
    {
      size_t lead = oi;
      while (lead > 0 && m->ops[lead].group_followers == 0 && m->ops[lead - 1].type == kOpConv &&
             m->ops[lead - 1].w_off == op.w_off) {
        --lead;
      }
      for (size_t j = lead; j < oi; ++j) sub0 += (m->ops[j].cout + 31) / 32;
    }
    const int bn = op.nb * 32;
    const int taps = op.kh * op.kw;
    {
      size_t lead = oi;
      while (lead > 0 && m->ops[lead].group_followers == 0 && m->ops[lead - 1].type == kOpConv &&
             m->ops[lead - 1].w_off == op.w_off) {
        --lead;
// ... 97 lines not shown
      c.pad_h = op.pad_h;
      c.pad_w = op.pad_w;
      c.cin = op.cin_real;
      c.cout = op.cout;
      c.w_off = m->layers[op.layer].param_off;
      c.raw = op.raw;
      c.shift_off = static_cast<int64_t>(op.shift_off);
      c.split = op.split_rows;
      c.keep_f32 = m->buffers[op.out_buf].f32 || m->buffers[op.out_buf].wide ? 1 : 0;
      if (op.pool_in) {
        plan.bufs[op.in_buf].h = op.ih;
        plan.bufs[op.in_buf].w = op.iw;
      }
      if (op.pool_out) {
        oh = (oh - 3) / 2 + 1;
        ow = (ow - 3) / 2 + 1;
      }
    } else if (op.type == kOpAvgPool) {
      c.shift_relu = op.pool_shift_relu;
      if (op.pool_shift_relu) c.shift_off = static_cast<int64_t>(op.shift_off);
      c.cout = op.cout;
      c.keep_f32 = m->buffers[op.out_buf].f32 || m->buffers[op.out_buf].wide ? 1 : 0;
    } else {
      c.cout = op.cout;
    }
    plan.bufs[op.out_buf].h = oh;
    plan.bufs[op.out_buf].w = ow;
    plan.ops.push_back(c);
  }
  plan.feat_buf = m->feat_buf;
  plan.num_classes = m->desc.num_classes;
  plan.dense_off = m->layers.back().param_off;
  return plan;
}

int dv_model_calibrate(dv_model* m, const float* weights, int64_t n_weights, const uint8_t* images, int n_images,
                       float* corrections, int64_t capacity) {
  if (!m || !weights || !images) return dv::fail(DV_ERR_INVALID_ARGUMENT, "dv_model_calibrate: null");
  if (!m->loaded) return dv::fail(DV_ERR_INVALID_ARGUMENT, "dv_model_calibrate: load weights first");
  if (n_weights != m->n_params) return dv::fail(DV_ERR_INVALID_ARGUMENT, "dv_model_calibrate: wrong number of weights");
  if (n_images < 1 || n_images > 4096) return dv::fail(DV_ERR_INVALID_ARGUMENT, "dv_model_calibrate: 1..4096 images");
  const dv::CalibPlan plan = calib_plan_of(m);
  std::vector<float> corr, dense_corr;
  if (int rc = dv::run_calibration(plan, m->device, weights, n_weights, m->h_shift, images, n_images, &corr,
                                   &dense_corr)) {
    return rc;
  }
  std::vector<float> shift = m->h_shift, dense_b = m->h_dense_b;
  for (size_t i = 0; i < shift.size(); ++i) shift[i] -= corr[i];
  for (size_t k = 0; k < dense_b.size(); ++k) dense_b[k] -= dense_corr[k];
  DV_HIP_CHECK(hipSetDevice(m->device));
  DV_HIP_CHECK(hipDeviceSynchronize());
  DV_HIP_CHECK(hipMemcpy(m->d_shift.ptr, shift.data(), shift.size() * 4, hipMemcpyHostToDevice));
  DV_HIP_CHECK(hipMemcpy(m->d_dense_b.ptr, dense_b.data(), dense_b.size() * 4, hipMemcpyHostToDevice));
  if (corrections != nullptr) {
    int64_t at = 0;
    for (size_t off : m->correction_shift_offsets()) {
      if (at < capacity) corrections[at++] = corr[off];
    }
    for (size_t k = 0; k < dense_corr.size() && at < capacity; ++k) corrections[at++] = dense_corr[k];
  }
  return prepare_blank_responses(m);
}

int dv_model_apply_corrections(dv_model* m, const float* corrections, int64_t n) {
  if (!m || !corrections) return dv::fail(DV_ERR_INVALID_ARGUMENT, "dv_model_apply_corrections: null");
  if (!m->loaded) return dv::fail(DV_ERR_INVALID_ARGUMENT, "dv_model_apply_corrections: load weights first");
  const std::vector<size_t> offs = m->correction_shift_offsets();
  if (n != static_cast<int64_t>(offs.size() + m->h_dense_b.size())) return dv::fail(DV_ERR_INVALID_ARGUMENT, "dv_model_apply_corrections: wrong number of corrections");
  for (int64_t i = 0; i < n; ++i) {
    if (!std::isfinite(corrections[i])) return dv::fail(DV_ERR_BAD_INPUT, "dv_model_apply_corrections: non-finite correction");
  }
  std::vector<float> shift = m->h_shift, dense_b = m->h_dense_b;
  int64_t at = 0;
  for (size_t off : offs) shift[off] -= corrections[at++];
  for (size_t k = 0; k < dense_b.size(); ++k) dense_b[k] -= corrections[at++];
  DV_HIP_CHECK(hipSetDevice(m->device));
  DV_HIP_CHECK(hipDeviceSynchronize());
  DV_HIP_CHECK(hipMemcpy(m->d_shift.ptr, shift.data(), shift.size() * 4, hipMemcpyHostToDevice));
  DV_HIP_CHECK(hipMemcpy(m->d_dense_b.ptr, dense_b.data(), dense_b.size() * 4, hipMemcpyHostToDevice));
  return prepare_blank_responses(m);
}

int dv_model_num_ops(const dv_model* m) { return m ? static_cast<int>(m->ops.size()) : 0; }

int dv_model_op_label(const dv_model* m, int op_index, char* buf, int capacity) {
  if (!m || !buf || capacity < 1 || op_index < 0 || op_index >= static_cast<int>(m->ops.size())) {
    return dv::fail(DV_ERR_INVALID_ARGUMENT, "dv_model_op_label: bad argument");
  }
  const Op& op = m->ops[op_index];
  const char* kind = op.type == kOpConv ? "conv" : op.type == kOpMaxPool ? "maxpool" : "avgpool";
  snprintf(buf, static_cast<size_t>(capacity), "%s layer=%d k=%dx%d s=%d cin=%d cout=%d out=%dx%d raw=%d in_buf=%d out_buf=%d coff=%d lds_only=%d",
           kind, op.layer, op.kh, op.kw, op.stride, op.cin, op.cout, op.oh, op.ow, op.raw ? 1 : 0, op.in_buf, op.out_buf,
           op.out_coff, (op.type == kOpConv && (op.stem_a || op.stem_b)) || (op_index + 1 < static_cast<int>(m->ops.size()) && m->ops[op_index + 1].in_chain && m->ops[op_index + 1].in_buf == op.out_buf) ||
               (op.b35 >= 2 && op.b35 <= 4) || op.b35 == 6 || op.m3 == 1 || op.m3 == 2 ? 1 : 0);
  return DV_OK;
}

int dv_model_probe_rounding(dv_model* m, const float* weights, int64_t n_weights, const uint8_t* images, int n_images,
                            const uint8_t* keep_f32, int flags, const float* corrections, int64_t n_corrections,
                            float* logits_r, float* logits_e, float* corrections_out) {
  if (!m || !weights || !images || !logits_e) return dv::fail(DV_ERR_INVALID_ARGUMENT, "dv_model_probe_rounding: null");
  if (!m->loaded) return dv::fail(DV_ERR_INVALID_ARGUMENT, "dv_model_probe_rounding: load weights first");
  if (n_weights != m->n_params) return dv::fail(DV_ERR_INVALID_ARGUMENT, "dv_model_probe_rounding: wrong number of weights");
  if (n_images < 1 || n_images > 4096) return dv::fail(DV_ERR_INVALID_ARGUMENT, "dv_model_probe_rounding: 1..4096 images");
  dv::CalibPlan plan = calib_plan_of(m);
  if (keep_f32 != nullptr) {
    for (size_t i = 0; i < plan.ops.size(); ++i) plan.ops[i].keep_f32 = keep_f32[i] ? 1 : 0;
  }
  std::vector<float> corr_in(m->h_shift.size(), 0.f), dense_in(m->h_dense_b.size(), 0.f);
  if (corrections != nullptr) {
    const std::vector<size_t> offs = m->correction_shift_offsets();
    if (n_corrections != static_cast<int64_t>(offs.size() + dense_in.size())) return dv::fail(DV_ERR_INVALID_ARGUMENT, "dv_model_probe_rounding: wrong number of corrections");
    int64_t at = 0;
    for (size_t off : offs) corr_in[off] = corrections[at++];
    for (size_t k = 0; k < dense_in.size(); ++k) dense_in[k] = corrections[at++];
  }
  const bool measure = (flags & 2) != 0;
  if (measure && corrections != nullptr) return dv::fail(DV_ERR_INVALID_ARGUMENT, "dv_model_probe_rounding: measure or apply");
  dv::CalibProbe probe;
  probe.corr_in = measure ? nullptr : corr_in.data();
  probe.dense_corr_in = measure ? nullptr : dense_in.data();
  probe.logits_r = logits_r;
  probe.logits_e = logits_e;
  probe.skip_r = logits_r == nullptr && !measure;
  probe.weights_f32 = (flags & 1) != 0;
  std::vector<float> corr, dense_corr;
  if (int rc = dv::run_calibration(plan, m->device, weights, n_weights, m->h_shift, images, n_images, &corr, &dense_corr,
                                   &probe)) {
    return rc;
  }
  if (corrections_out != nullptr) {
    int64_t at = 0;
    for (size_t off : m->correction_shift_offsets()) corrections_out[at++] = corr[off];
    for (float v : dense_corr) corrections_out[at++] = v;
  }
  return DV_OK;
}

int dv_model_debug_tensor(dv_model* m, int index, int n, void* host_out, int32_t* h,
                          int32_t* w, int32_t* c) {
  if (m && index == -1) index = m->feat_buf;
  if (m && index == -2) index = m->stem_out_buf;
  if (!m || index < 0 || index >= static_cast<int>(m->buffers.size())) {
    return dv::fail(DV_ERR_INVALID_ARGUMENT, "dv_model_debug_tensor: bad index");
  }
  const BufferDesc& b = m->buffers[index];
  if (h) *h = b.h + 2 * b.halo;
  if (w) *w = b.w + 2 * b.halo;
  if (c) *c = b.c;
  if (host_out) {
    DV_HIP_CHECK(hipSetDevice(m->device));
    DV_HIP_CHECK(hipDeviceSynchronize());
    if (b.f32) {
      std::vector<float> tmp(static_cast<size_t>(n) * b.bytes_per_example() / 4);
      DV_HIP_CHECK(hipMemcpy(tmp.data(), m->dbuf[index].ptr, tmp.size() * 4, hipMemcpyDeviceToHost));
      _Float16* dst = static_cast<_Float16*>(host_out);
      for (size_t i = 0; i < tmp.size(); ++i) dst[i] = static_cast<_Float16>(tmp[i]);
    } else if (b.wide) {
      const size_t half_halfs = b.bytes_per_example() / 4;
      std::vector<_Float16> tmp(static_cast<size_t>(n) * half_halfs * 2);
      DV_HIP_CHECK(hipMemcpy(tmp.data(), m->dbuf[index].ptr, tmp.size() * 2, hipMemcpyDeviceToHost));
      _Float16* dst = static_cast<_Float16*>(host_out);
      for (int e = 0; e < n; ++e)
        for (size_t i = 0; i < half_halfs; ++i) {
          dst[static_cast<size_t>(e) * half_halfs + i] = static_cast<_Float16>(
              static_cast<float>(tmp[static_cast<size_t>(e) * 2 * half_halfs + i]) +
              static_cast<float>(tmp[static_cast<size_t>(e) * 2 * half_halfs + half_halfs + i]));
        }
    } else {
      DV_HIP_CHECK(hipMemcpy(host_out, m->dbuf[index].ptr,
                             static_cast<size_t>(n) * b.bytes_per_example(),
                             hipMemcpyDeviceToHost));
    }
  }
  return DV_OK;
}

static int enqueue_forward(dv_model* m, int n, hipStream_t stream, const HeadOutputs* head_out) {
  const size_t img_bytes = static_cast<size_t>(m->desc.height) * m->desc.width * m->desc.channels;
  const ExtPtrs* ext = ext_table(m);
  const int n_parts = (n + m->desc.max_batch - 1) / m->desc.max_batch;
  const int part = n_parts ? (n + n_parts - 1) / n_parts : 0;
  for (int done = 0; done < n; done += part) {
    const int nb = std::min(part, n - done);
    for (int sb0 = 0; sb0 < nb; sb0 += stem_sub_batch()) {
      const int sb = std::min(stem_sub_batch(), nb - sb0);
      const size_t img_off = static_cast<size_t>(done + sb0) * img_bytes;
      if (m->blank_on()) {
        dv::ProfileScope prof(dv::kProfOther, stream);
        const Op& c4 = m->ops[m->blank_conv4_op];
        launch_blank_scan(ext, img_off, done + sb0, sb, m->desc.height, m->desc.width * m->desc.channels,
                          static_cast<int*>(m->d_blank_thr.ptr), m->desc.max_batch, m->ops[1].oh, m->ops[3].oh, c4.ow,
                          c4.pool_out ? m->buffers[c4.out_buf].h : c4.oh, m->ops[2].stem_b ? 1 : 0, c4.pool_out ? 1 : 0,
                          stream);
      }
      if (!m->ops[0].first_u8) {
        dv::ProfileScope prof(dv::kProfOther, stream);
        launch_preprocess(ext, img_off, m->buf_ptr(0), sb, m->desc.channels, m->desc.height, m->desc.width,
                          m->buffers[0].geom(), stream);
      }
      if (int rc = run_ops(m, 0, m->stem_ops_end, sb, stream, m->stem_out_buf, sb0, img_off)) return rc;
    }
    if (int rc = run_ops(m, m->stem_ops_end, static_cast<int>(m->ops.size()), nb, stream)) {
      return rc;
    }
    {
      dv::ProfileScope prof(dv::kProfOther, stream);
      const bool outs = head_out != nullptr;
      launch_head(m->buf_ptr<float>(m->feat_buf), static_cast<const float*>(m->d_dense_w.ptr),
                  static_cast<const float*>(m->d_dense_b.ptr), ext, static_cast<size_t>(done) * m->desc.num_classes,
                  m->buffers[m->feat_buf].geom(), m->desc.num_classes, nb, outs,
                  outs && head_out->pooled ? head_out->pooled + static_cast<size_t>(done) * m->feat_c : nullptr,
                  outs && head_out->logits ? head_out->logits + static_cast<size_t>(done) * m->desc.num_classes : nullptr,
                  stream);
    }
  }
  return DV_OK;
}

int dv_model_infer(dv_model* m, const uint8_t* images, int n, float* probs, void* stream_v) {
  return dv_model_infer_rows(m, images, n, probs, nullptr, 0, stream_v);
}

int dv_model_infer_rows(dv_model* m, const uint8_t* images, int n, float* probs, const int32_t* rows_used, int rows_add,
                        void* stream_v) {
  if (!m || !images || !probs || n < 0) {
    return dv::fail(DV_ERR_INVALID_ARGUMENT, "dv_model_infer: bad argument");
  }
  if (!m->loaded) return dv::fail(DV_ERR_INVALID_ARGUMENT, "dv_model_infer: no weights loaded");
  if (n == 0) return DV_OK;
  hipStream_t stream = static_cast<hipStream_t>(stream_v);
  DV_HIP_CHECK(hipSetDevice(m->device));
  static const bool op_trace = getenv("DV_OP_TRACE") != nullptr;
  static const bool no_graph = getenv("DV_NO_GRAPH") != nullptr || op_trace;
  hipStreamCaptureStatus capturing = hipStreamCaptureStatusNone;
  if (stream != nullptr) (void)hipStreamIsCapturing(stream, &capturing);
  set_ext(m, images, probs, stream, rows_used, rows_add);
  if (no_graph || dv::profiling_enabled() || stream == nullptr ||
      capturing != hipStreamCaptureStatusNone) {
    static std::vector<OpTrace> trace_store;
    g_trace = op_trace ? &trace_store : nullptr;
    if (int rc = enqueue_forward(m, n, stream)) return rc;
    DV_HIP_CHECK(hipGetLastError());
    if (op_trace) dump_trace(stream);
    return DV_OK;
  }
  for (const dv_model::GraphEntry& g : m->graphs) {
    if (g.n == n && g.stream == stream) {
      DV_HIP_CHECK(hipGraphLaunch(g.exec, stream));
      ++m->graph_replays;
      return DV_OK;
    }
  }
  hipGraph_t graph = nullptr;
  DV_HIP_CHECK(hipStreamBeginCapture(stream, hipStreamCaptureModeRelaxed));
  const int rc = enqueue_forward(m, n, stream);
  const hipError_t ce = hipStreamEndCapture(stream, &graph);
  if (rc != DV_OK) {
    if (graph) (void)hipGraphDestroy(graph);
    return rc;
  }
  if (ce != hipSuccess || graph == nullptr) {
    return dv::fail(DV_ERR_HIP, std::string("hipStreamEndCapture: ") + hipGetErrorString(ce));
  }
  dv_model::GraphEntry e{n, stream, nullptr};
  const hipError_t ie = hipGraphInstantiate(&e.exec, graph, nullptr, nullptr, 0);
  (void)hipGraphDestroy(graph);
  if (ie != hipSuccess) {
    return dv::fail(DV_ERR_HIP, std::string("hipGraphInstantiate: ") + hipGetErrorString(ie));
  }
  if (m->graphs.size() >= 8) {
    (void)hipStreamSynchronize(m->graphs.front().stream);
    (void)hipGraphExecDestroy(m->graphs.front().exec);
    m->graphs.erase(m->graphs.begin());
  }
  m->graphs.push_back(e);
  ++m->graph_captures;
  DV_HIP_CHECK(hipGraphLaunch(e.exec, stream));
  return DV_OK;
}

int dv_model_is_precise(const dv_model* m) { return m && m->precise ? 1 : 0; }

int dv_model_set_blank_skip(dv_model* m, int enabled) {
  if (!m) return dv::fail(DV_ERR_INVALID_ARGUMENT, "dv_model_set_blank_skip: null");
  const bool on = enabled != 0;
  if (on == m->blank_enabled) return DV_OK;
  DV_HIP_CHECK(hipSetDevice(m->device));
  for (auto& g : m->graphs) {
    (void)hipStreamSynchronize(g.stream);
    (void)hipGraphExecDestroy(g.exec);
  }
  m->graphs.clear();
  m->blank_enabled = on;
  return DV_OK;
}

int dv_model_blank_thresholds(dv_model* m, int n, int32_t* out) {
  if (!m || !out || n < 1 || n > m->desc.max_batch) return dv::fail(DV_ERR_INVALID_ARGUMENT, "dv_model_blank_thresholds: bad argument");
  if (!m->blank_on()) return dv::fail(DV_ERR_UNSUPPORTED, "dv_model_blank_thresholds: blank-row skipping is off for this model");
  DV_HIP_CHECK(hipSetDevice(m->device));
  DV_HIP_CHECK(hipDeviceSynchronize());
  for (int k = 0; k < 5; ++k) {
    DV_HIP_CHECK(hipMemcpy(out + static_cast<size_t>(k) * n,
                           static_cast<const int*>(m->d_blank_thr.ptr) + static_cast<size_t>(k) * m->desc.max_batch,
                           static_cast<size_t>(n) * sizeof(int), hipMemcpyDeviceToHost));
  }
  return DV_OK;
}

namespace {
struct OutputView {
  int buf = -1;
  int coff = 0, c = 0;
  int h = 1, w = 1;
  bool logits = false;
};
}

static int resolve_output(const dv_model* m, const char* name, OutputView* v, const char* fn) {
  const std::string s = name != nullptr ? name : "";
  std::string known;
  for (const dv_model::NamedView& nv : m->named_views) {
    if (s == nv.name) {
      const BufferDesc& b = m->buffers[nv.buf];
      *v = OutputView{nv.buf, nv.coff, nv.c, b.h, b.w, false};
      return DV_OK;
    }
    known += nv.name + ", ";
  }
  if (s == "prelogits") {
    *v = OutputView{-1, 0, m->feat_c, 1, 1, false};
    return DV_OK;
  }
  if (s == "logits") {
    *v = OutputView{-1, 0, m->desc.num_classes, 1, 1, true};
    return DV_OK;
  }
  return dv::fail(DV_ERR_INVALID_ARGUMENT, std::string(fn) + ": unknown output name '" + s + "' (accepted: " + known +
                                               "prelogits, logits)");
}

int dv_model_output_info(const dv_model* m, const char* name, int32_t* h, int32_t* w, int32_t* c) {
  if (!m) return dv::fail(DV_ERR_INVALID_ARGUMENT, "dv_model_output_info: null");
  OutputView v;
  if (int rc = resolve_output(m, name, &v, "dv_model_output_info")) return rc;
  if (h) *h = v.h;
  if (w) *w = v.w;
  if (c) *c = v.c;
  return DV_OK;
}

int dv_model_infer_outputs(dv_model* m, const uint8_t* images, int n, float* probs, int n_outputs,
                           const char* const* names, float* const* outs, void* stream_v) {
  if (!m || !images || !probs || n < 0 || n_outputs < 0 || (n_outputs > 0 && (!names || !outs))) {
    return dv::fail(DV_ERR_INVALID_ARGUMENT, "dv_model_infer_outputs: bad argument");
  }
  if (n > m->desc.max_batch) {
    return dv::fail(DV_ERR_INVALID_ARGUMENT, "dv_model_infer_outputs: n = " + std::to_string(n) + " is above max_batch = " +
                                                 std::to_string(m->desc.max_batch));
  }
  if (!m->loaded) return dv::fail(DV_ERR_INVALID_ARGUMENT, "dv_model_infer_outputs: no weights loaded");
  std::vector<OutputView> views(n_outputs);
  HeadOutputs head{nullptr, nullptr};
  for (int k = 0; k < n_outputs; ++k) {
    if (int rc = resolve_output(m, names[k], &views[k], "dv_model_infer_outputs")) return rc;
    if (outs[k] == nullptr || reinterpret_cast<uintptr_t>(outs[k]) % 16 != 0) {
      return dv::fail(DV_ERR_INVALID_ARGUMENT, std::string("dv_model_infer_outputs: the output for '") + names[k] +
                                                   "' is null or not 16-byte aligned");
    }
    for (int j = 0; j < k; ++j) {
      if (std::strcmp(names[j], names[k]) == 0) {
        return dv::fail(DV_ERR_INVALID_ARGUMENT, std::string("dv_model_infer_outputs: '") + names[k] + "' requested twice");
      }
    }
    if (views[k].buf < 0) (views[k].logits ? head.logits : head.pooled) = outs[k];
  }
  if (n_outputs == 0) return dv_model_infer(m, images, n, probs, stream_v);
  if (n == 0) return DV_OK;
  hipStream_t stream = static_cast<hipStream_t>(stream_v);
  DV_HIP_CHECK(hipSetDevice(m->device));
  set_ext(m, images, probs, stream);
  if (int rc = enqueue_forward(m, n, stream, &head)) return rc;
  for (int k = 0; k < n_outputs; ++k) {
    const OutputView& v = views[k];
    if (v.buf < 0) continue;
    const BufferDesc& b = m->buffers[v.buf];
    const TensorGeom g = b.geom();
    dv::LayerExportArgs a{};
    a.src = m->dbuf[v.buf].ptr;
    a.kind = b.f32 ? dv::kExportF32 : b.wide ? dv::kExportWide : dv::kExportF16;
    a.n = n;
    a.h = g.h;
    a.w = g.w;
    a.halo = g.halo;
    a.hp = g.hp;
    a.wp = g.wp;
    a.src_groups = g.groups;
    a.lo_groups = b.c / 8;
    a.goff = v.coff / 8;
    a.groups = v.c / 8;
    a.dst = outs[k];
    dv::ProfileScope prof(dv::kProfOther, stream);
    dv::launch_layer_export(a, stream);
  }
  DV_HIP_CHECK(hipGetLastError());
  return DV_OK;
}

int dv_model_graph_stats(const dv_model* m, int64_t* captures, int64_t* replays) {
  if (!m) return dv::fail(DV_ERR_INVALID_ARGUMENT, "dv_model_graph_stats: null");
  if (captures) *captures = m->graph_captures;
  if (replays) *replays = m->graph_replays;
  return DV_OK;
}

}
```

deepvariant_amd/csrc/model_graph.cpp:

```cpp
#include <algorithm>
#include <cstdlib>

#include "model_graph.h"
#include "model_kernels.h"
#include "block35.h"
#include "mixed3.h"
#include "chain.h"
#include "stem_fused.h"

int dv_model::new_buffer(int h, int w, int c) {
  buffers.push_back({h, w, c, 0});
  buffers.back().wide = precise && wide_stage;
  return static_cast<int>(buffers.size()) - 1;
}
int dv_model::pick_nb(int cout) {
  static const bool nb6 = getenv("DV_NB6") != nullptr && atoi(getenv("DV_NB6")) != 0;
  if (nb6 && cout > 128 && cout <= 192) return 6;
  int best = 4, best_cost = 1 << 30, best_waste = 1 << 30;
  for (int nb = 4; nb >= 1; --nb) {
    const int bn = nb * 32;
    const int tiles = (cout + bn - 1) / bn;
    const int cost = tiles * (nb + 1), waste = tiles * bn - cout;
    if (cost < best_cost || (cost == best_cost && waste < best_waste)) {
      best_cost = cost;
// ... 156 lines not shown
        wanted = false;
        for (const char* q = only; *q;) {
          if (atoi(q) == op.kh * op.kw) wanted = true;
          while (*q && *q != ',') ++q;
          if (*q == ',') ++q;
        }
      }
      int subs = 0;
      for (int gi = 0; gi <= followers; ++gi) subs += (ops[i + gi].cout + 31) / 32;
      const int P = op.oh * op.ow;
      for (int g = 512 / P; wanted && g >= 1 && g * P >= 384; --g) {
        const dv::ImgConvArgs a = imgconv_geometry(op, g);
        if (a.act_slab_bytes > 64 * 1024 || dv::imgconv_lds_bytes(a, op.nb) > 160 * 1024) continue;
        op.v2 = true;
        op.v2_g = g;
        op.v2_steps = a.n_steps;
        op.v2_tiles = (subs + op.nb - 1) / op.nb;
        buffers[op.in_buf].min_examples = std::max(buffers[op.in_buf].min_examples, g);
        break;
      }
    }
    i += followers;
  }
}

void dv_model::choose_band() {
  if (getenv("DV_NO_BAND") != nullptr) return;
  for (Op& op : ops) {
    if (op.type != kOpConv || op.first_u8 || op.pool_in || op.pool_out || op.stem_a || op.stem_b || op.v2 ||
        op.chain_len != 0 || op.in_chain || op.group_followers != 0 || op.stride != 1 || op.kh <= 1 || op.oh != op.ih) {
      continue;
    }
    const int h = op.ih;
    if (h >= op.kh || h > std::min(op.pad_h, op.kh - 1 - op.pad_h) + 1 || op.ow < 5) continue;
    bool follower = false;
    for (const Op& lead : ops) {
      if (lead.type == kOpConv && lead.group_followers > 0 && &op > &lead &&
          &op <= &lead + lead.group_followers) {
        follower = true;
      }
    }
    if (follower) continue;
    op.band = h;
    if (op.cout > 128 && op.cout <= 192 && op.nb == 3 && getenv("DV_NO_BAND_NB6") == nullptr) op.nb = 6;
    op.n_chunks = h * op.kw * (op.cin / kChunk);
    op.n_steps = (op.n_chunks + kSlabChunks - 1) / kSlabChunks;
  }
}

void dv_model::choose_side_pool() {
  if (getenv("DV_NO_SIDE_POOL") != nullptr) return;
  for (size_t pi = 0; pi < ops.size(); ++pi) {
    Op& pl = ops[pi];
    if (pl.type != kOpMaxPool) continue;
    for (size_t ci = 0; ci < ops.size(); ++ci) {
      Op& cv = ops[ci];
      if (cv.type != kOpConv || cv.in_buf != pl.in_buf || cv.stride != 2 || cv.kh != 3 || cv.kw != 3 ||
          cv.pad_h != 0 || cv.pad_w != 0 || cv.nb != 4 || cv.group_followers != 0 || cv.first_u8 || cv.pool_in ||
          cv.pool_out || cv.stem_a || cv.stem_b || cv.v2 || cv.band || cv.split || cv.chain_len != 0 || cv.in_chain ||
          cv.raw || cv.cin != pl.cin || cv.cin % kChunk != 0 || cv.cin != buffers[cv.in_buf].c ||
          cv.oh != pl.oh || cv.ow != pl.ow || cv.side_pool_partner >= 0) {
        continue;
      }
      cv.side_pool_partner = static_cast<int>(pi);
      pl.side_pool_partner = static_cast<int>(ci);
      break;
    }
  }
}

void dv_model::choose_split() {
  const int first_layer_env = getenv("DV_SPLIT_FROM") ? atoi(getenv("DV_SPLIT_FROM")) : -1;
  const char* list_env = getenv("DV_SPLIT_LAYERS");
  const char* split_default_env = getenv("DV_SPLIT_DEFAULT");
  auto wanted = [&](const Op& o) {
    if (list_env != nullptr) {
      for (const char* q = list_env; *q;) {
        if (atoi(q) == o.layer) return true;
        while (*q && *q != ',') ++q;
        if (*q == ',') ++q;
      }
      return false;
    }
    if (first_layer_env >= 0) return o.layer >= first_layer_env;
    if (split_default_env == nullptr || atoi(split_default_env) == 0) return false;
    if (o.kh * o.kw == 1 && o.layer >= 30 && o.layer < 70) return o.raw || buffers[o.out_buf].c > o.cout;
    return o.layer >= 70 && std::max(o.kh, o.kw) <= 3;
  };
  for (size_t i = 0; i < ops.size(); ++i) {
    Op& op = ops[i];
    if (op.type != kOpConv) continue;
    const int followers = op.group_followers;
    const bool eligible = !op.first_u8 && !op.pool_in && !op.pool_out && !op.stem_a && !op.stem_b && !op.v2 &&
                          op.chain_len == 0 && !op.in_chain && !(i > 0 && (ops[i - 1].stem_a || ops[i - 1].stem_b)) &&
                          op.nb <= 4 && static_cast<int>(i) != blank_conv4_op && !op.in_wide;
    int n_wanted = 0;
    for (int gi = 0; gi <= followers; ++gi) n_wanted += wanted(ops[i + gi]) ? 1 : 0;
    if (eligible && n_wanted > 0) {
      int split_subs = 0, all_subs = 0;
      bool partial = n_wanted <= followers && wanted(op);
      if (partial) {
        std::stable_partition(ops.begin() + i + 1, ops.begin() + i + 1 + followers,
                              [&](const Op& o) { return wanted(o); });
        for (int gi = 0; gi <= followers; ++gi) {
          if (wanted(ops[i + gi])) split_subs += (ops[i + gi].cout + 31) / 32;
        }
        partial = split_subs % ops[i].nb == 0;
      }
      for (int gi = 0; gi <= followers; ++gi) all_subs += (ops[i + gi].cout + 31) / 32;
      Op& lead = ops[i];
      lead.split_tiles = partial ? split_subs / lead.nb : (all_subs + lead.nb - 1) / lead.nb;
      for (int gi = 0; gi <= followers; ++gi) {
        Op& o = ops[i + gi];
        o.split = true;
        o.split_rows = !partial || wanted(o);
        o.n_chunks *= 2;
        o.n_steps = (o.n_chunks + kSlabChunks - 1) / kSlabChunks;
      }
    }
    i += followers;
  }
}

void dv_model::choose_avg_epilogue() {
  if (getenv("DV_NO_AVG_EPI") != nullptr) return;
  const int min_g = getenv("DV_AVG_EPI_MIN_G") ? atoi(getenv("DV_AVG_EPI_MIN_G")) : 1;
  const int min_fill = getenv("DV_AVG_EPI_MIN_FILL") ? atoi(getenv("DV_AVG_EPI_MIN_FILL")) : 85;
  for (size_t i = 0; i < ops.size(); ++i) {
    Op& lead = ops[i];
    if (lead.type != kOpConv) continue;
    const int followers = lead.group_followers;
    const int px = lead.oh * lead.ow;
    const bool ok = lead.kh == 1 && lead.kw == 1 && lead.stride == 1 && lead.nb == 4 && !lead.split && !lead.pool_in &&
                    !lead.pool_out && !lead.v2 && !lead.band && lead.chain_len == 0 && !lead.in_chain &&
                    !lead.first_u8 && !lead.stem_a && !lead.stem_b && px >= 5 && px <= 256 &&
                    (256 / px) * px * 100 >= 256 * min_fill && 256 / px >= min_g;
    if (ok) {
      for (int gi = 0; gi <= followers; ++gi) {
        Op& c = ops[i + gi];
        if (!c.raw) continue;
        for (size_t j = i + followers + 1; j < ops.size(); ++j) {
          Op& pl = ops[j];
          if (pl.type == kOpAvgPool && pl.in_buf == c.out_buf && pl.pool_shift_relu && pl.avg_partner < 0) {
            c.avg_partner = static_cast<int>(j);
            pl.avg_partner = static_cast<int>(i + gi);
            lead.avg_tile_g = 256 / px;
            break;
          }
        }
      }
    }
    i += followers;
  }
}

void dv_model::choose_chains() {
  if (getenv("DV_NO_CHAIN") != nullptr) return;
  const bool no_2d = getenv("DV_NO_CHAIN2D") != nullptr;
  const int min_len_2d = getenv("DV_CHAIN2D_MIN_LEN") ? atoi(getenv("DV_CHAIN2D_MIN_LEN")) : 2;
  std::vector<int> readers(buffers.size(), 0);
  for (const Op& o : ops) readers[o.in_buf]++;
  auto plain = [&](const Op& o) {
    return o.type == kOpConv && !buffers[o.out_buf].f32 && !o.in_wide && !buffers[o.out_buf].wide && o.stride == 1 && (o.kh & 1) && (o.kw & 1) && o.kh * o.kw > 1 &&
           o.pad_h == (o.kh - 1) / 2 && o.pad_w == (o.kw - 1) / 2 && o.group_followers == 0 &&
           !o.first_u8 && !o.pool_in && !o.pool_out && !o.raw && !o.stem_a && !o.stem_b && o.cin % kChunk == 0 &&
           o.cin == o.cin_real && o.oh == o.ih && o.ow == o.iw;
  };
  auto one_d = [&](const Op& o) {
    return plain(o) && (o.kh == 1) != (o.kw == 1) && std::max(o.kh, o.kw) <= dv::kChainMaxTaps;
  };
  auto two_d = [&](const Op& o) {
    const int subs = (o.cout + 31) / 32;
    return plain(o) && ((o.kh == 3 && o.kw == 3) || (o.kh == 5 && o.kw == 5)) && subs >= 2 && subs <= 3;
  };
  for (size_t i = 0; i < ops.size(); ++i) {
    const int P = ops[i].oh * ops[i].ow;
    const bool big = P > dv::kChainTilePx / 2;
    if (big ? (no_2d || P > dv::kChainTilePxBig || !two_d(ops[i])) : !one_d(ops[i])) continue;
    auto member = [&](const Op& o) { return big ? two_d(o) : one_d(o); };
    size_t len = 1;
    while (i + len < ops.size() && len < static_cast<size_t>(dv::kChainMaxLayers)) {
      const Op& prev = ops[i + len - 1];
      const Op& next = ops[i + len];
      if (!member(next) || next.in_buf != prev.out_buf || prev.out_coff != 0 || readers[prev.out_buf] != 1 ||
          prev.cout % 32 != 0 || buffers[prev.out_buf].c != prev.cout) {
        break;
      }
      ++len;
    }
    if (static_cast<int>(len) < (big ? min_len_2d : 2)) continue;
    const int tpx = big ? dv::kChainTilePxBig : dv::kChainTilePx;
    const int g = tpx / P;
    if (g * P < tpx * 2 / 3) continue;
    size_t act = 0, slot = 0;
    bool fits = true;
    for (size_t k = 0; k < len; ++k) {
      const Op& o = ops[i + k];
      act = std::max(act, static_cast<size_t>(o.cin / 8) * tpx * 16);
      slot = std::max(slot, static_cast<size_t>(o.kh * o.kw) * 2 * ((o.cout + 31) / 32 * 32) * 16);
      if (!big) fits = fits && (o.cout + 31) / 32 >= 4 && (o.cout + 31) / 32 <= 6;
    }
    if (!fits || act + 2 * slot + 16 > 160 * 1024) continue;
    ops[i].chain_len = static_cast<int>(len);
    ops[i].chain_g = g;
    ops[i].chain_tpx = tpx;
    for (size_t k = 1; k < len; ++k) {
      ops[i + k].in_chain = true;
      const int c = ops[i + k - 1].cout;
      buffers[ops[i + k].in_buf] = {1, 1, c, 0};
    }
    buffers[ops[i].in_buf].min_examples = std::max(buffers[ops[i].in_buf].min_examples, g);
    i += len - 1;
  }
}

void dv_model::choose_block35() {
  if (getenv("DV_NO_BLOCK35") != nullptr || getenv("DV_NO_CHAIN") != nullptr) return;
  std::vector<int> readers(buffers.size(), 0);
  for (const Op& o : ops) readers[o.in_buf]++;
  for (size_t i = 0; i + 7 < ops.size(); ++i) {
    const Op &b1 = ops[i], &r5 = ops[i + 1], &r3 = ops[i + 2], &pj = ops[i + 3];
    const Op &c5 = ops[i + 4], &c3a = ops[i + 5], &c3b = ops[i + 6], &ap = ops[i + 7];
    const int P = b1.oh * b1.ow;
    auto plain = [&](const Op& o) {
      return o.type == kOpConv && o.stride == 1 && !o.split && !o.in_wide && !buffers[o.out_buf].wide && !o.pool_in &&
             !o.pool_out && !o.first_u8 && !o.stem_a && !o.stem_b && !o.band && o.cin % kChunk == 0 &&
             o.cin == o.cin_real && o.oh == b1.oh && o.ow == b1.ow && o.ih == b1.oh && o.iw == b1.ow && o.b35 == 0;
    };
    auto head = [&](const Op& o, int cout) {
      return plain(o) && o.kh == 1 && o.kw == 1 && o.in_buf == b1.in_buf && o.cout == cout;
    };
    auto same = [&](const Op& o, int k, int in_buf, int cin, int cout) {
      return plain(o) && o.kh == k && o.kw == k && o.pad_h == k / 2 && o.pad_w == k / 2 && o.in_buf == in_buf &&
             o.cin == cin && o.cout == cout && !o.raw;
    };
    const int O = b1.out_buf;
    const bool ok =
        b1.group_followers == 3 && P <= dv::kBlock35TilePx && head(b1, dv::kBlock35B1) && !b1.raw &&
        head(r5, dv::kBlock35Red5) && !r5.raw && head(r3, dv::kBlock35Red3) && !r3.raw &&
        head(pj, pj.cout) && pj.raw && (pj.cout == 32 || pj.cout == 64) &&
        same(c5, 5, r5.out_buf, dv::kBlock35Red5, dv::kBlock35Out5) &&
        same(c3a, 3, r3.out_buf, dv::kBlock35Red3, dv::kBlock35Out3) &&
        same(c3b, 3, c3a.out_buf, dv::kBlock35Out3, dv::kBlock35Out3) &&
        ap.type == kOpAvgPool && ap.in_buf == pj.out_buf && ap.pool_shift_relu &&
        readers[r5.out_buf] == 1 && readers[r3.out_buf] == 1 && readers[c3a.out_buf] == 1 && readers[pj.out_buf] == 1 &&
        c5.out_buf == O && c3b.out_buf == O && ap.out_buf == O && !buffers[O].f32 && !buffers[O].wide &&
        b1.out_coff % 8 == 0 && c5.out_coff % 8 == 0 && c3b.out_coff % 8 == 0 && ap.out_coff % 8 == 0;
    if (!ok) continue;
    for (int k = 0; k < 8; ++k) {
      Op& o = ops[i + k];
      o.b35 = k + 1;
      o.chain_len = 0;
      o.in_chain = false;
      o.v2 = false;
      o.avg_partner = -1;
      o.avg_tile_g = 0;
    }
    for (int b : {r5.out_buf, r3.out_buf, c3a.out_buf, pj.out_buf}) {
      const bool f32 = buffers[b].f32;
      buffers[b] = {1, 1, buffers[b].c, 0};
      buffers[b].f32 = f32;
    }
    i += 7;
  }
}

void dv_model::choose_mixed3() {
  if (getenv("DV_NO_MIXED3_FUSE") != nullptr || getenv("DV_NO_CHAIN") != nullptr) return;
  std::vector<int> readers(buffers.size(), 0);
  for (const Op& o : ops) readers[o.in_buf]++;
  for (size_t i = 0; i + 2 < ops.size(); ++i) {
    const Op &a = ops[i], &b = ops[i + 1], &c = ops[i + 2];
    auto plain = [&](const Op& o) {
      return o.type == kOpConv && !o.split && !o.in_wide && !buffers[o.out_buf].wide && !buffers[o.out_buf].f32 &&
             !o.pool_in && !o.pool_out && !o.first_u8 && !o.stem_a && !o.stem_b && !o.band && !o.raw &&
             o.group_followers == 0 && o.chain_len == 0 && !o.in_chain && o.b35 == 0 && o.m3 == 0 &&
             o.side_pool_partner < 0 && o.avg_partner < 0 && o.cin % kChunk == 0 && o.cin == o.cin_real;
    };
    bool follower = false;
    for (size_t j = 0; j < i; ++j) follower = follower || (ops[j].type == kOpConv && j + ops[j].group_followers >= i);
    const bool ok =
        !follower && plain(a) && plain(b) && plain(c) &&
        a.kh == 1 && a.kw == 1 && a.stride == 1 && a.cout == dv::kMixed3Red && a.cin == buffers[a.in_buf].c &&
        a.cin / kChunk >= dv::mixed3_min_chunks() && a.out_coff == 0 && buffers[a.out_buf].c == a.cout &&
        readers[a.out_buf] == 1 &&
        b.in_buf == a.out_buf && b.kh == 3 && b.kw == 3 && b.stride == 1 && b.pad_h == 1 && b.pad_w == 1 &&
        b.cin == dv::kMixed3Red && b.cout == dv::kMixed3Mid && b.out_coff == 0 && buffers[b.out_buf].c == b.cout &&
        readers[b.out_buf] == 1 &&
        c.in_buf == b.out_buf && c.kh == 3 && c.kw == 3 && c.stride == 2 && c.pad_h == 0 && c.pad_w == 0 &&
        c.cin == dv::kMixed3Mid && c.cout == dv::kMixed3Out && c.out_coff % 8 == 0 &&
        a.ih >= 3 && a.iw >= 3 && a.ih * a.iw <= dv::kMixed3TilePx && c.oh * c.ow <= dv::kMixed3MaxOutPx;
    if (!ok) continue;
    for (int k = 0; k < 3; ++k) {
      Op& o = ops[i + k];
      o.m3 = k + 1;
      o.v2 = false;
    }
    for (int buf : {a.out_buf, b.out_buf}) buffers[buf] = {1, 1, buffers[buf].c, 0};
    i += 2;
  }
}

void dv_model::build() {
  const int in_buf = new_buffer(desc.height, desc.width, 16);
  TensorRef x = full(in_buf);
  x = conv(x, 32, 3, 3, 2, false, -1, 0, desc.channels);
// ... 6 lines not shown
    f.n_steps = 1;
    buffers[in_buf] = {1, 1, 16, 0};
  }
  x = conv(x, 32, 3, 3, 1, false);
  x = conv(x, 64, 3, 3);
  if (getenv("DV_NO_POOL_FUSE") == nullptr) {
    TensorRef pooled = x;
    pooled.h = (x.h - 3) / 2 + 1;
    pooled.w = (x.w - 3) / 2 + 1;
    const int ih = x.h, iw = x.w;
    x = conv(pooled, 80, 1, 1, 1, false);
    ops.back().pool_in = true;
    ops.back().ih = ih;
    ops.back().iw = iw;
  } else {
    x = pool(kOpMaxPool, x);
    x = conv(x, 80, 1, 1, 1, false);
  }
  if (getenv("DV_NO_STEM_FUSE") == nullptr) {
    const int stem_a_max = getenv("DV_NO_STEM_A_WIDE") == nullptr ? dv::kStemA_MaxChannels : 8;
    if (ops[0].first_u8 && desc.channels <= stem_a_max && ops[3].pool_in && ops[3].cout <= 96) {
      ops[0].stem_a = true;
      buffers[ops[0].out_buf] = {1, 1, 32, 0};
    }
    if (ops[3].pool_in && ops[3].cout <= 96 && (ops[0].stem_a || getenv("DV_NO_STEM_B_ALONE") == nullptr)) {
      ops[2].stem_b = true;
      buffers[ops[2].out_buf] = {1, 1, 64, 0};
    }
  }
  x = conv(x, 192, 3, 3, 1, false);
  blank_conv4_op = static_cast<int>(ops.size()) - 1;
  const bool fuse_pool2 = getenv("DV_NO_POOL2_FUSE") == nullptr && getenv("DV_NO_POOL_FUSE") == nullptr &&
                          getenv("DV_NO_GROUPING") == nullptr;
  const int pool2_ih = x.h, pool2_iw = x.w;
  const bool pool_in_conv = fuse_pool2 && getenv("DV_NO_POOL2_IN_CONV") == nullptr && ops.back().nb == 3 &&
                            x.h >= 3 && x.w >= 3;
  if (pool_in_conv) {
    x.h = (x.h - 3) / 2 + 1;
    x.w = (x.w - 3) / 2 + 1;
    ops.back().pool_out = true;
    buffers[x.buf] = {x.h, x.w, x.c, 0};
  } else if (fuse_pool2) {
    x.h = (x.h - 3) / 2 + 1;
    x.w = (x.w - 3) / 2 + 1;
  } else {
    x = pool(kOpMaxPool, x);
  }
  stem_ops_end = static_cast<int>(ops.size());
  stem_out_buf = x.buf;
  for (int pool_ch : {32, 64, 64}) {
    const int out = new_buffer(x.h, x.w, 64 + 64 + 96 + pool_ch);
    conv(x, 64, 1, 1, 1, true, out, 0);
    TensorRef b5 = conv(x, 48, 1, 1);
    conv(b5, 64, 5, 5, 1, true, out, 64);
    TensorRef b3 = conv(x, 64, 1, 1);
    b3 = conv(b3, 96, 3, 3);
    conv(b3, 96, 3, 3, 1, true, out, 128);
    pooled_projection(x, pool_ch, out, 224);
    named_views.push_back({"mixed" + std::to_string(named_views.size()), out, 0, buffers[out].c});
    if (fuse_pool2 && !pool_in_conv && x.buf == stem_out_buf) {
      for (size_t k = stem_ops_end; k < ops.size(); ++k) {
        if (ops[k].type == kOpConv && ops[k].in_buf == x.buf) {
          ops[k].pool_in = true;
          ops[k].ih = pool2_ih;
          ops[k].iw = pool2_iw;
        }
      }
    }
    x = full(out);
  }
  {
    const int oh = (x.h - 3) / 2 + 1, ow = (x.w - 3) / 2 + 1;
    const int out = new_buffer(oh, ow, 384 + 96 + x.c);
    conv(x, 384, 3, 3, 2, false, out, 0);
    TensorRef b = conv(x, 64, 1, 1);
    b = conv(b, 96, 3, 3);
    conv(b, 96, 3, 3, 2, false, out, 384);
    pool(kOpMaxPool, x, out, 480);
    named_views.push_back({"mixed3", out, 0, buffers[out].c});
    x = full(out);
  }
  wide_stage = true;
  for (int c7 : {128, 160, 160, 192}) {
    const int out = new_buffer(x.h, x.w, 768);
    conv(x, 192, 1, 1, 1, true, out, 0);
    TensorRef b = conv(x, c7, 1, 1);
    b = conv(b, c7, 1, 7);
    conv(b, 192, 7, 1, 1, true, out, 192);
    TensorRef d = conv(x, c7, 1, 1);
    d = conv(d, c7, 7, 1);
    d = conv(d, c7, 1, 7);
    d = conv(d, c7, 7, 1);
    conv(d, 192, 1, 7, 1, true, out, 384);
    pooled_projection(x, 192, out, 576);
    named_views.push_back({"mixed" + std::to_string(named_views.size()), out, 0, buffers[out].c});
    x = full(out);
  }
  {
    const int oh = (x.h - 3) / 2 + 1, ow = (x.w - 3) / 2 + 1;
    const int out = new_buffer(oh, ow, 320 + 192 + x.c);
    TensorRef b = conv(x, 192, 1, 1);
    conv(b, 320, 3, 3, 2, false, out, 0);
    TensorRef d = conv(x, 192, 1, 1);
    d = conv(d, 192, 1, 7);
    d = conv(d, 192, 7, 1);
    conv(d, 192, 3, 3, 2, false, out, 320);
    pool(kOpMaxPool, x, out, 512);
    named_views.push_back({"mixed8", out, 0, buffers[out].c});
    x = full(out);
  }
  for (int i = 0; i < 2; ++i) {
    const int out = new_buffer(x.h, x.w, 2048);
    conv(x, 320, 1, 1, 1, true, out, 0);
    TensorRef b = conv(x, 384, 1, 1);
    conv(b, 384, 1, 3, 1, true, out, 320);
    conv(b, 384, 3, 1, 1, true, out, 704);
    named_views.push_back({"mixed9_" + std::to_string(i), out, 320, 2 * 384});
    TensorRef d = conv(x, 448, 1, 1);
    d = conv(d, 384, 3, 3);
    conv(d, 384, 1, 3, 1, true, out, 1088);
    conv(d, 384, 3, 1, 1, true, out, 1472);
    pooled_projection(x, 192, out, 1856);
    named_views.push_back({"mixed" + std::to_string(9 + i), out, 0, buffers[out].c});
    x = full(out);
  }
  feat_buf = x.buf;
  buffers[feat_buf].f32 = true;
  buffers[feat_buf].wide = false;
  feat_p = x.h * x.w;
  feat_c = x.c;
  group_siblings();
  for (const Op& op : ops) {
    int need = 0;
    if (op.type == kOpConv) need = std::max(op.pad_h, op.pad_w);
    if (op.type == kOpAvgPool) need = 1;
    buffers[op.in_buf].halo = std::max(buffers[op.in_buf].halo, need);
  }
  choose_chains();
  if (getenv("DV_CHAIN_KEEP_HALO") == nullptr) {
    for (BufferDesc& b : buffers) b.halo = 0;
    for (const Op& op : ops) {
      if (op.in_chain) continue;
      int need = 0;
      if (op.type == kOpConv && op.chain_len == 0) need = std::max(op.pad_h, op.pad_w);
      if (op.type == kOpAvgPool) need = 1;
      buffers[op.in_buf].halo = std::max(buffers[op.in_buf].halo, need);
    }
  }
  choose_imgconv();
  choose_band();
  choose_split();
  choose_side_pool();
  choose_avg_epilogue();
  choose_block35();
  choose_mixed3();
  for (size_t i = 0; i < ops.size(); ++i) {
    Op& op = ops[i];
    if (op.type != kOpConv) continue;
    int subs = 0;
    for (int gi = 0; gi <= op.group_followers; ++gi) subs += (ops[i + gi].cout + 31) / 32;
    const int n_tiles = (subs + op.nb - 1) / op.nb;
    for (int gi = 0; gi <= op.group_followers; ++gi) ops[i + gi].w_off = packed_halfs;
    packed_halfs += op.first_u8 ? static_cast<size_t>(kFirstMaxChunks) * 32 * kChunk
                    : op.b35 == 1 ? static_cast<size_t>(2) * (op.cin / kChunk) * 2 * 128 * 8
                    : op.m3 == 1 ? static_cast<size_t>(op.cin / kChunk) * 2 * dv::kMixed3Red * 8
                    : (op.chain_len > 0 || op.in_chain || op.b35 >= 5 || op.m3 >= 2)
                        ? static_cast<size_t>(op.n_chunks) * 2 * ((op.cout + 31) / 32 * 32) * 8
                    : op.v2     ? static_cast<size_t>(op.v2_tiles) * op.v2_steps *
                                      dv::imgconv_wslab_halfs(op.kh, op.kw, op.nb)
                                : static_cast<size_t>(op.band ? op.band : 1) * n_tiles * op.n_steps *
                                      kSlabChunks * (op.nb * 32) * kChunk;
    i += op.group_followers;
  }
  layers.push_back({1, 1, feat_c, desc.num_classes, n_params});
  n_params += static_cast<int64_t>(feat_c) * desc.num_classes + desc.num_classes;
}

std::vector<size_t> dv_model::correction_shift_offsets() const {
  std::vector<const Op*> by_layer(layers.size(), nullptr);
  for (const Op& op : ops) {
    if (op.type == kOpConv) by_layer[op.layer] = &op;
  }
  std::vector<size_t> at;
  for (size_t l = 0; l + 1 < layers.size(); ++l) {
    for (int co = 0; co < by_layer[l]->cout; ++co) at.push_back(by_layer[l]->shift_off + co);
  }
  return at;
}
```

deepvariant_amd/csrc/model_graph.h:

```cpp
#ifndef DV_MODEL_GRAPH_H_
#define DV_MODEL_GRAPH_H_

#include <string>
#include <vector>

#include "dv_internal.h"
#include "conv_mfma.h"
#include "imgconv.h"

namespace dv {
namespace graph {

using namespace convk;

struct TensorRef {
  int buf = -1;
  int h = 0, w = 0, c = 0;
};

struct BufferDesc {
  int h, w, c;
  int halo = 0;
  int min_examples = 1;
  bool f32 = false;
  bool wide = false;
  TensorGeom geom() const {
    return TensorGeom{h, w, halo, h + 2 * halo, w + 2 * halo, (wide ? 2 : 1) * (c / 8)};
  }
  size_t bytes_per_example() const {
    return static_cast<size_t>(h + 2 * halo) * (w + 2 * halo) * c * (f32 ? 4 : wide ? 4 : 2);
  }
};

enum OpType { kOpConv, kOpMaxPool, kOpAvgPool };

struct Op {
  OpType type;
  int in_buf, out_buf;
  int out_coff = 0;
  int layer = -1;
  int kh = 0, kw = 0, stride = 1, pad_h = 0, pad_w = 0;
  int cin = 0, cin_real = 0, cout = 0;
  bool in_wide = false;
  int ih = 0, iw = 0, oh = 0, ow = 0;
  int nb = 4;
  int n_steps = 0, n_chunks = 0;
  size_t w_off = 0;
  size_t shift_off = 0;
  size_t tbl_off = 0;
  bool raw = false;
  int group_followers = 0;
  bool first_u8 = false;
  bool pool_shift_relu = false;
  bool pool_in = false;
  int side_pool_partner = -1;
  int avg_partner = -1;
  int avg_tile_g = 0;
  bool pool_out = false;
  int band = 0;
  bool split = false;
  bool split_rows = false;
  int split_tiles = 0;
  bool v2 = false;
  int v2_g = 0;
  int v2_steps = 0;
  int v2_tiles = 0;
  bool stem_a = false;
  bool stem_b = false;
  int chain_len = 0;
  int chain_g = 0;
  int chain_tpx = 0;
  bool in_chain = false;
  int b35 = 0;
  int m3 = 0;
};

struct LayerInfo {
  int kh, kw, cin, cout;
  int64_t param_off;
};

}
}

using namespace dv::graph;

struct dv_model {
  int device = 0;
  dv_model_desc desc{};
  std::vector<BufferDesc> buffers;
  std::vector<Op> ops;
  std::vector<LayerInfo> layers;
  int64_t n_params = 0;
  int feat_buf = -1, feat_p = 0, feat_c = 0;
  int stem_ops_end = 0, stem_out_buf = -1;
  int stem_a_grid = 512, stem_b_grid = 256;
  int n_cus = 256;
  size_t packed_halfs = 0, shift_floats = 0, tbl_entries = 0;
  std::vector<dv::DeviceBuffer> dbuf;
  dv::DeviceBuffer d_w, d_shift, d_dense_w, d_dense_b, d_tbl;
  bool blank_skip = false;
  bool blank_enabled = true;
  bool blank_ready = false;
  int blank_conv4_op = -1;
  dv::DeviceBuffer d_blank_thr;
  dv::DeviceBuffer d_blank_conv4;
  dv::DeviceBuffer d_blank_c2;
  dv::DeviceBuffer d_blank_b;
  bool blank_on() const { return blank_ready && blank_enabled; }
  bool precise = false;
  bool wide_stage = false;
  bool loaded = false;
  std::vector<float> h_shift, h_dense_b;
  dv::DeviceBuffer d_ext;
  struct GraphEntry {
    int n;
    hipStream_t stream;
    hipGraphExec_t exec;
  };
  std::vector<GraphEntry> graphs;
  int64_t graph_captures = 0, graph_replays = 0;
  struct NamedView {
    std::string name;
    int buf, coff, c;
  };
  std::vector<NamedView> named_views;

  template <typename T = _Float16>
  T* buf_ptr(int buf) const { return static_cast<T*>(dbuf[buf].ptr); }
  const _Float16* w_ptr(const Op& op) const { return static_cast<const _Float16*>(d_w.ptr) + op.w_off; }
  const float* shift_ptr(const Op& op) const { return static_cast<const float*>(d_shift.ptr) + op.shift_off; }
  const int* blank_thr(int row) const { return static_cast<const int*>(d_blank_thr.ptr) + row * desc.max_batch; }

  int new_buffer(int h, int w, int c);
  static int pick_nb(int cout);
  TensorRef conv(TensorRef x, int cout, int kh, int kw, int stride = 1, bool same = true,
                 int dst_buf = -1, int dst_coff = 0, int cin_real = -1);
  TensorRef full(int buf) const;
  void pooled_projection(TensorRef x, int cout, int dst_buf, int dst_coff);
  TensorRef pool(OpType type, TensorRef x, int dst_buf = -1, int dst_coff = 0);
  void group_siblings();
  dv::ImgConvArgs imgconv_geometry(const Op& op, int g) const;
  void choose_imgconv();
  void choose_band();
  void choose_side_pool();
  void choose_split();
  void choose_avg_epilogue();
  void choose_chains();
  void choose_block35();
  void choose_mixed3();
  void build();
  std::vector<size_t> correction_shift_offsets() const;
};

#endif
```

deepvariant_amd/csrc/model_kernels.h:

```cpp
#ifndef DV_MODEL_KERNELS_H_
#define DV_MODEL_KERNELS_H_

#include "conv_common.h"

namespace dv {
namespace convk {

struct ExtPtrs {
  const uint8_t* images;
  float* probs;
  const int32_t* rows_hint;
  int rows_add;
};

struct FirstConvArgs {
  const ExtPtrs* ext;
  size_t in_off;
  const _Float16* w;
  const float* shift;
  _Float16* out;
  TensorGeom og;
  int N, H, W, C, Cout;
  int OH, OW, KH, KW, stride;
  int M, n_chunks;
  unsigned in_bytes;
  float rcp_ow, rcp_ohow;
  int wide;
};

constexpr int kFirstMaxChunks = 13;

struct PoolArgs {
  const _Float16* in;
  const float* in32;
  _Float16* out;
  float* out32;
  int lo_in_groups;
  int lo_out_groups;
  TensorGeom ig, og;
  int N, C, OH, OW;
  int out_goff;
  const float* shift;
};

void launch_set_ext(ExtPtrs* ext, const uint8_t* images, float* probs, const int32_t* rows_hint, int rows_add,
                    hipStream_t stream);
void launch_conv_first_u8(const FirstConvArgs& f, hipStream_t stream);
void launch_preprocess(const ExtPtrs* ext, size_t in_off, _Float16* out, int n, int C, int H, int W, TensorGeom og,
                       hipStream_t stream);
void launch_blank_scan(const ExtPtrs* ext, size_t in_off, int n_hint0, int n, int H, int row_bytes, int* thr, int stride,
                       int oh2, int ph_b, int ow4, int p4, int stem_b_fused, int conv4_walks, hipStream_t stream);
void launch_maxpool3s2(const PoolArgs& p, hipStream_t stream);
void launch_avgpool3s1(const PoolArgs& p, hipStream_t stream);
void launch_head(const float* in, const float* w, const float* b, const ExtPtrs* ext, size_t probs_off, TensorGeom g, int K,
                 int n, bool outputs, float* pooled, float* logits, hipStream_t stream);

}
}

#endif
```

deepvariant_amd/csrc/model_kernels.hip:

```cpp
#include <cstdlib>

#include "model_kernels.h"
#include "stem_fused.h"

using namespace dv::convk;

namespace {

constexpr int kFirstUnroll = 5;

__global__ void set_ext_kernel(ExtPtrs* ext, const uint8_t* images, float* probs, const int32_t* rows_hint, int rows_add) {
  ext->images = images;
  ext->probs = probs;
  ext->rows_hint = rows_hint;
  ext->rows_add = rows_add;
}

__device__ __forceinline__ const uint8_t* ext_images(const ExtPtrs* ext, size_t off) {
  const unsigned long long v = reinterpret_cast<unsigned long long>(ext->images + off);
  const unsigned lo = __builtin_amdgcn_readfirstlane(static_cast<unsigned>(v));
  const unsigned up = __builtin_amdgcn_readfirstlane(static_cast<unsigned>(v >> 32));
  return reinterpret_cast<const uint8_t*>((static_cast<unsigned long long>(up) << 32) | lo);
}

// ... 180 lines not shown
  const bool hinted = ext->rows_hint != nullptr;
  const int hinted_rows = hinted ? max(0, min(H, ext->rows_hint[n_hint0 + n] + ext->rows_add)) : 0;
  for (int hi = hinted ? 0 : n_dw; hi > 0; hi -= 256 * kPer) {
    uint32_t v[kPer];
#pragma unroll
    for (int k = 0; k < kPer; ++k) {
      const int i = hi - 1 - (k * 256 + tid);
      v[k] = i >= 0 ? img[i] : 0u;
    }
    int mine = -1;
#pragma unroll
    for (int k = 0; k < kPer; ++k) {
      const int i = hi - 1 - (k * 256 + tid);
      if (v[k] != 0) mine = max(mine, 4 * i + 3 - (__clz(v[k]) >> 3));
    }
    if (mine >= 0) atomicMax(&last, mine);
    __syncthreads();
    if (last >= 0) break;
  }
  if (tid == 0) {
    const int r = hinted ? hinted_rows : last < 0 ? 0 : last / row_bytes + 1;
    const int t2 = (r + 1) / 2, t3 = t2 + 1, t4 = (t3 + 1) / 2;
    thr[n] = r;
    thr[stride + n] = t2;
    thr[2 * stride + n] = t4;
    thr[3 * stride + n] = t4;
    thr[4 * stride + n] = (t4 + 1) / 2;
  }
}

__global__ void maxpool3s2_kernel(PoolArgs p) {
  const int cg = p.C / 8;
  const size_t total = static_cast<size_t>(p.N) * cg * p.OH * p.OW;
  const size_t i = blockIdx.x * static_cast<size_t>(blockDim.x) + threadIdx.x;
  if (i >= total) return;
  const int ow = i % p.OW;
  size_t t = i / p.OW;
  const int oh = t % p.OH;
  t /= p.OH;
  const int g = t % cg;
  const int n = t / cg;
  const size_t plane = static_cast<size_t>(p.ig.hp) * p.ig.wp;
  const half8_t* src = reinterpret_cast<const half8_t*>(p.in) + (static_cast<size_t>(n) * p.ig.groups + g) * plane;
  const half8_t* src_lo = src + static_cast<size_t>(p.lo_in_groups) * plane;
  half8_t best, best_lo;
#pragma unroll
  for (int j = 0; j < 8; ++j) {
    best[j] = static_cast<_Float16>(-65504.f);
    best_lo[j] = static_cast<_Float16>(0.f);
  }
  const size_t at0 = static_cast<size_t>(oh * 2 + p.ig.halo) * p.ig.wp + ow * 2 + p.ig.halo;
  if (p.lo_in_groups > 0) {
    half8_t v[9], l[9];
#pragma unroll
    for (int t9 = 0; t9 < 9; ++t9) {
      const size_t at = at0 + static_cast<size_t>(t9 / 3) * p.ig.wp + t9 % 3;
      v[t9] = src[at];
      l[t9] = src_lo[at];
    }
#pragma unroll
    for (int t9 = 0; t9 < 9; ++t9) {
#pragma unroll
      for (int j = 0; j < 8; ++j) {
        const bool take = v[t9][j] > best[j] || (v[t9][j] == best[j] && l[t9][j] > best_lo[j]);
        best[j] = take ? v[t9][j] : best[j];
        best_lo[j] = take ? l[t9][j] : best_lo[j];
      }
    }
  } else {
    for (int dh = 0; dh < 3; ++dh)
      for (int dw = 0; dw < 3; ++dw) {
        const half8_t v = src[at0 + static_cast<size_t>(dh) * p.ig.wp + dw];
#pragma unroll
        for (int j = 0; j < 8; ++j) best[j] = v[j] > best[j] ? v[j] : best[j];
      }
  }
  const size_t oplane = static_cast<size_t>(p.og.hp) * p.og.wp;
  half8_t* dst = reinterpret_cast<half8_t*>(p.out) + (static_cast<size_t>(n) * p.og.groups + p.out_goff + g) * oplane +
                 static_cast<size_t>(oh + p.og.halo) * p.og.wp + ow + p.og.halo;
  *dst = best;
  if (p.lo_out_groups > 0) dst[static_cast<size_t>(p.lo_out_groups) * oplane] = best_lo;
}

__global__ void avgpool3s1_kernel(PoolArgs p) {
  const int cg = p.C / 8;
  const int H = p.ig.h, W = p.ig.w;
  const int W2 = (W + 1) >> 1;
  const size_t total = static_cast<size_t>(p.N) * cg * H * W2;
  const size_t i = blockIdx.x * static_cast<size_t>(blockDim.x) + threadIdx.x;
  if (i >= total) return;
  const int ow = 2 * static_cast<int>(i % W2);
  size_t t = i / W2;
  const int oh = t % H;
  t /= H;
  const int g = t % cg;
  const int n = t / cg;
  const bool two = ow + 1 < W;
  const float4* src = reinterpret_cast<const float4*>(p.in32) +
                      (((static_cast<size_t>(n) * p.ig.groups + g) * p.ig.hp + oh + p.ig.halo - 1) *
                           p.ig.wp + ow + p.ig.halo - 1) * 2;
  const int last = two ? 3 : 2;
  float col[4][8];
#pragma unroll
  for (int dw = 0; dw < 4; ++dw) {
    const int c = dw < 3 ? dw : last;
#pragma unroll
    for (int hf = 0; hf < 2; ++hf) {
      const float4 a = src[2 * c + hf], b = src[2 * (p.ig.wp + c) + hf], d = src[2 * (2 * p.ig.wp + c) + hf];
      col[dw][4 * hf + 0] = a.x + b.x + d.x;
      col[dw][4 * hf + 1] = a.y + b.y + d.y;
      col[dw][4 * hf + 2] = a.z + b.z + d.z;
      col[dw][4 * hf + 3] = a.w + b.w + d.w;
    }
  }
  const int rows = (oh > 0) + (oh < H - 1) + 1;
  float sh[8] = {0, 0, 0, 0, 0, 0, 0, 0};
  if (p.shift != nullptr) {
    const float4 s0 = *reinterpret_cast<const float4*>(p.shift + g * 8);
    const float4 s1 = *reinterpret_cast<const float4*>(p.shift + g * 8 + 4);
    sh[0] = s0.x; sh[1] = s0.y; sh[2] = s0.z; sh[3] = s0.w;
    sh[4] = s1.x; sh[5] = s1.y; sh[6] = s1.z; sh[7] = s1.w;
  }
  const size_t at = ((static_cast<size_t>(n) * p.og.groups + p.out_goff + g) * p.og.hp + oh + p.og.halo) * p.og.wp +
                    ow + p.og.halo;
#pragma unroll
  for (int k = 0; k < 2; ++k) {
    if (k == 1 && !two) break;
    const int x = ow + k;
    const float inv = 1.0f / static_cast<float>(rows * ((x > 0) + (x < W - 1) + 1));
    float o[8];
#pragma unroll
    for (int j = 0; j < 8; ++j) {
      o[j] = avg_finish(col[k][j], col[k + 1][j], col[k + 2][j], inv, sh[j], p.shift != nullptr);
    }
    if (p.out32 != nullptr) {
      float4* d = reinterpret_cast<float4*>(p.out32 + (at + k) * 8);
      d[0] = make_float4(o[0], o[1], o[2], o[3]);
      d[1] = make_float4(o[4], o[5], o[6], o[7]);
    } else {
      half8_t h;
#pragma unroll
      for (int j = 0; j < 8; ++j) h[j] = static_cast<_Float16>(o[j]);
      reinterpret_cast<half8_t*>(p.out)[at + k] = h;
      if (p.lo_out_groups > 0) {
        half8_t l;
#pragma unroll
        for (int j = 0; j < 8; ++j) l[j] = static_cast<_Float16>(o[j] - static_cast<float>(h[j]));
        reinterpret_cast<half8_t*>(p.out)[at + k + static_cast<size_t>(p.lo_out_groups) * p.og.hp * p.og.wp] = l;
      }
    }
  }
}

template <bool OUT>
__device__ __forceinline__ void head_body(const float* in, const float* w, const float* b, float* probs, TensorGeom g,
                                          int K, float* pooled, float* logits) {
  __shared__ float red[8][4];
  const int n = blockIdx.x;
  const int tid = threadIdx.x;
  const int C = g.groups * 8;
  const size_t plane = static_cast<size_t>(g.hp) * g.wp * 8;
  float part[8] = {0, 0, 0, 0, 0, 0, 0, 0};
  const float* x = in + static_cast<size_t>(n) * g.groups * plane;
  const float invP = 1.0f / static_cast<float>(g.h * g.w);
  for (int grp = tid; grp * 8 < C; grp += 256) {
    float s[8] = {0, 0, 0, 0, 0, 0, 0, 0};
    const float4* xg = reinterpret_cast<const float4*>(x + static_cast<size_t>(grp) * plane);
    for (int y = 0; y < g.h; ++y)
      for (int xx = 0; xx < g.w; ++xx) {
        const float4 lo = xg[((y + g.halo) * g.wp + xx + g.halo) * 2], up = xg[((y + g.halo) * g.wp + xx + g.halo) * 2 + 1];
        s[0] += lo.x; s[1] += lo.y; s[2] += lo.z; s[3] += lo.w;
        s[4] += up.x; s[5] += up.y; s[6] += up.z; s[7] += up.w;
      }
#pragma unroll
    for (int j = 0; j < 8; ++j) {
      const float m = s[j] * invP;
      if (OUT && pooled != nullptr) pooled[static_cast<size_t>(n) * C + grp * 8 + j] = m;
      for (int k = 0; k < K; ++k) part[k] += m * w[static_cast<size_t>(grp * 8 + j) * K + k];
    }
  }
  for (int k = 0; k < K; ++k) {
    float v = part[k];
    for (int off = 32; off > 0; off >>= 1) v += __shfl_down(v, off);
    if ((tid & 63) == 0) red[k][tid >> 6] = v;
  }
  __syncthreads();
  if (tid == 0) {
    float logit[8], mx = -1e30f;
    for (int k = 0; k < K; ++k) {
      logit[k] = red[k][0] + red[k][1] + red[k][2] + red[k][3] + b[k];
      if (OUT && logits != nullptr) logits[static_cast<size_t>(n) * K + k] = logit[k];
      mx = fmaxf(mx, logit[k]);
    }
    float sum = 0.f;
    for (int k = 0; k < K; ++k) {
      logit[k] = expf(logit[k] - mx);
      sum += logit[k];
    }
    for (int k = 0; k < K; ++k) probs[static_cast<size_t>(n) * K + k] = logit[k] / sum;
  }
}

__global__ __launch_bounds__(256) void head_kernel(const float* in, const float* w,
                                                   const float* b, const ExtPtrs* ext, size_t probs_off,
                                                   TensorGeom g, int K) {
  head_body<false>(in, w, b, ext->probs + probs_off, g, K, nullptr, nullptr);
}

__global__ __launch_bounds__(256) void head_outputs_kernel(const float* in, const float* w, const float* b,
                                                           const ExtPtrs* ext, size_t probs_off, TensorGeom g, int K,
                                                           float* pooled, float* logits) {
  head_body<true>(in, w, b, ext->probs + probs_off, g, K, pooled, logits);
}

}

namespace dv {
namespace convk {

void launch_set_ext(ExtPtrs* ext, const uint8_t* images, float* probs, const int32_t* rows_hint, int rows_add,
                    hipStream_t stream) {
  hipLaunchKernelGGL(set_ext_kernel, dim3(1), dim3(1), 0, stream, ext, images, probs, rows_hint, rows_add);
}

void launch_conv_first_u8(const FirstConvArgs& f, hipStream_t stream) {
  static const bool first4 = getenv("DV_FIRST_PT2") == nullptr;
  static const bool wide4 = getenv("DV_FIRST_WIDE_PT2") == nullptr;
  if (f.wide && wide4) {
    hipLaunchKernelGGL((conv_first_u8_kernel<4, 9>), dim3((f.M + 511) / 512), dim3(kConvThreads), 0,
                       stream, f);
  } else if (f.wide) {
    hipLaunchKernelGGL((conv_first_u8_kernel<2, 9>), dim3((f.M + 255) / 256), dim3(kConvThreads), 0,
                       stream, f);
  } else if (first4) {
    hipLaunchKernelGGL((conv_first_u8_kernel<4>), dim3((f.M + 511) / 512), dim3(kConvThreads), 0,
                       stream, f);
  } else {
    hipLaunchKernelGGL((conv_first_u8_kernel<2>), dim3((f.M + 255) / 256), dim3(kConvThreads), 0,
                       stream, f);
  }
}

void launch_preprocess(const ExtPtrs* ext, size_t in_off, _Float16* out, int n, int C, int H, int W, TensorGeom og,
                       hipStream_t stream) {
  const size_t n_pix = static_cast<size_t>(n) * H * W;
  hipLaunchKernelGGL(preprocess_kernel, dim3(static_cast<unsigned>((n_pix + 255) / 256)), dim3(256), 0, stream, ext, in_off,
                     out, n_pix, C, H, W, og);
}

void launch_blank_scan(const ExtPtrs* ext, size_t in_off, int n_hint0, int n, int H, int row_bytes, int* thr, int stride,
                       int oh2, int ph_b, int ow4, int p4, int stem_b_fused, int conv4_walks, hipStream_t stream) {
  hipLaunchKernelGGL(blank_rows_kernel, dim3(n), dim3(256), 0, stream, ext, in_off, n_hint0, H, row_bytes, thr, stride);
  hipLaunchKernelGGL(blank_need_kernel, dim3((n + 255) / 256), dim3(256), 0, stream, thr, stride, n, oh2, ph_b, ow4, p4,
                     stem_b_fused, conv4_walks);
}

void launch_maxpool3s2(const PoolArgs& p, hipStream_t stream) {
  const size_t total = static_cast<size_t>(p.N) * p.OH * p.OW * (p.C / 8);
  hipLaunchKernelGGL(maxpool3s2_kernel, dim3(static_cast<unsigned>((total + 255) / 256)), dim3(256), 0, stream, p);
}

void launch_avgpool3s1(const PoolArgs& p, hipStream_t stream) {
  const size_t total = static_cast<size_t>(p.N) * p.OH * ((p.OW + 1) / 2) * (p.C / 8);
  hipLaunchKernelGGL(avgpool3s1_kernel, dim3(static_cast<unsigned>((total + 255) / 256)), dim3(256), 0, stream, p);
}

void launch_head(const float* in, const float* w, const float* b, const ExtPtrs* ext, size_t probs_off, TensorGeom g, int K,
                 int n, bool outputs, float* pooled, float* logits, hipStream_t stream) {
  if (outputs) {
    hipLaunchKernelGGL(head_outputs_kernel, dim3(n), dim3(256), 0, stream, in, w, b, ext, probs_off, g, K, pooled, logits);
  } else {
    hipLaunchKernelGGL(head_kernel, dim3(n), dim3(256), 0, stream, in, w, b, ext, probs_off, g, K);
  }
}

}
}
```

Before: 510,700 candidates/s.

## Fuse global average pool into final Inception block conv epilogues

The last Inception block's conv epilogues now reduce each map's spatial positions with DPP row shifts and write per-example channel sums straight into a compact feature buffer. This skips writing the full final feature map and re-reading it in the head kernel. Blocks are regrouped so whole maps fit within 32-lane slots. The full feature map is recomputed lazily only when a host readback asks for it. The plain head path also gains an 8-wide unrolled load loop.

```diff
diff --git a/deepvariant_amd/csrc/conv_common.h b/deepvariant_amd/csrc/conv_common.h
--- a/deepvariant_amd/csrc/conv_common.h
+++ b/deepvariant_amd/csrc/conv_common.h
@@ -69,6 +69,10 @@
   float rcp_tile_p;
   int wide_in;
   unsigned lo_off;
+  float* gap_out;
+  int gap_c;
+  int gap_mpf;
+  unsigned gap_mask;
 };
 
 typedef unsigned int uint4_t __attribute__((ext_vector_type(4)));
@@ -86,6 +90,23 @@
     r -= d;
     ++q;
   }
+}
+
+__device__ __forceinline__ void gap_slot(const ConvArgs& p, int slot, int& il, int& pix, bool& ok) {
+  int q;
+  divmod_small(slot & 31, p.tile_p, p.rcp_tile_p, q, pix);
+  il = (slot >> 5) * p.gap_mpf + q;
+  ok = q < p.gap_mpf;
+}
+
+__device__ __forceinline__ float gap_sum(float v, int P) {
+  float s = 0.f + v;
+  int t = __builtin_bit_cast(int, v);
+  for (int i = 1; i < P; ++i) {
+    t = __builtin_amdgcn_update_dpp(0, t, 0x130, 0xf, 0xf, false);
+    s += __builtin_bit_cast(float, t);
+  }
+  return s;
 }
 
 __device__ __forceinline__ float avg_finish(float c0, float c1, float c2, float inv, float sh, bool shift_relu) {
@@ -111,15 +132,35 @@
   }
 }
 
-template <int PT>
+template <int PT, bool GAP = false>
 __device__ __forceinline__ void epilogue_subtile(const float16_t (&acc)[PT], const ConvBranch& b, int cbase,
                                                  const int (&pn)[PT], const int (&poh)[PT], const int (&pow_)[PT],
-                                                 const bool (&mvalid)[PT], int lane) {
+                                                 const bool (&mvalid)[PT], int lane, float* gap_out = nullptr,
+                                                 int gap_c = 0, int gap_p = 0) {
   const int hi = lane >> 5;
   const half2_t zero2 = {static_cast<_Float16>(0.f), static_cast<_Float16>(0.f)};
   const unsigned gstride = static_cast<unsigned>(b.og.hp * b.og.wp);
   float2_t shv[4][2];
   load_shifts(b.shift, cbase, hi, shv);
+  if constexpr (GAP) {
+    if (gap_out != nullptr) {
+#pragma unroll
+      for (int pt = 0; pt < PT; ++pt) {
+        const float16_t a = acc[pt];
+        const bool first = mvalid[pt] && poh[pt] == 0 && pow_[pt] == 0;
+        float* dst = gap_out + static_cast<size_t>(pn[pt]) * gap_c + (b.out_goff * 8 + cbase + 4 * hi);
+#pragma unroll
+        for (int q = 0; q < 4; ++q) {
+          float4 v = make_float4(a[4 * q] + shv[q][0][0], a[4 * q + 1] + shv[q][0][1], a[4 * q + 2] + shv[q][1][0],
+                                 a[4 * q + 3] + shv[q][1][1]);
+          if (b.relu) v = make_float4(fmaxf(v.x, 0.f), fmaxf(v.y, 0.f), fmaxf(v.z, 0.f), fmaxf(v.w, 0.f));
+          const float4 s = make_float4(gap_sum(v.x, gap_p), gap_sum(v.y, gap_p), gap_sum(v.z, gap_p), gap_sum(v.w, gap_p));
+          if (first && cbase + 8 * q < b.Cout) *reinterpret_cast<float4*>(dst + 8 * q) = s;
+        }
+      }
+      return;
+    }
+  }
   if (b.out32 != nullptr) {
 #pragma unroll
     for (int pt = 0; pt < PT; ++pt) {
@@ -196,7 +237,7 @@
   return bi;
 }
 
-template <int NB, int PT>
+template <int NB, int PT, bool GAP = false>
 __device__ __forceinline__ void conv_epilogue(const float16_t (&acc)[NB][PT], const ConvArgs& p,
                                               int n_tile, const int (&pn)[PT], const int (&poh)[PT],
                                               const int (&pow_)[PT], const bool (&mvalid)[PT],
@@ -204,10 +245,16 @@
 #pragma unroll
   for (int nb = 0; nb < NB; ++nb) {
     const int sub = n_tile * NB + nb;
-    const ConvBranch& b = p.br[branch_of(p, sub)];
+    const int bi = branch_of(p, sub);
+    const ConvBranch& b = p.br[bi];
     const int cbase = (sub - b.sub0) * 32;
     if (cbase >= b.Cout) continue;
-    epilogue_subtile<PT>(acc[nb], b, cbase, pn, poh, pow_, mvalid, lane);
+    if constexpr (GAP) {
+      epilogue_subtile<PT, true>(acc[nb], b, cbase, pn, poh, pow_, mvalid, lane,
+                                 (p.gap_mask >> bi) & 1u ? p.gap_out : nullptr, p.gap_c, p.tile_p);
+    } else {
+      epilogue_subtile<PT>(acc[nb], b, cbase, pn, poh, pow_, mvalid, lane);
+    }
   }
 }
 
@@ -265,12 +312,17 @@
   float* tile = reinterpret_cast<float*>(smem);
   const int my_slot = wave * 64 + lane;
   int il, pix, y, x;
-  divmod_small(my_slot, p.tile_p, p.rcp_tile_p, il, pix);
+  bool slot_ok = true;
+  if (p.gap_mpf > 0) {
+    gap_slot(p, my_slot, il, pix, slot_ok);
+  } else {
+    divmod_small(my_slot, p.tile_p, p.rcp_tile_p, il, pix);
+  }
   divmod_small(pix, p.OW, p.rcp_ow, y, x);
   const int n = pix_block * p.tile_g + il;
-  const bool live = il < p.tile_g && n < p.N;
+  const bool live = slot_ok && il < p.tile_g && n < p.N;
   const int H = p.OH, W = p.OW;
-  const int map0 = il * p.tile_p;
+  const int map0 = my_slot - pix;
   const float inv = 1.0f / static_cast<float>(((y > 0) + (y < H - 1) + 1) * ((x > 0) + (x < W - 1) + 1));
 #pragma unroll
   for (int half = 0; half < NB / 2; ++half) {
@@ -278,11 +330,13 @@
 #pragma unroll
     for (int nbl = 0; nbl < 2; ++nbl) {
       const int sub = n_tile * NB + 2 * half + nbl;
-      const ConvBranch& b = p.br[branch_of(p, sub)];
+      const int bi = branch_of(p, sub);
+      const ConvBranch& b = p.br[bi];
       const int cbase = (sub - b.sub0) * 32;
       if (cbase >= b.Cout) continue;
       if (b.avgpool == 0) {
-        epilogue_subtile<PT>(acc[2 * half + nbl], b, cbase, pn, poh, pow_, mvalid, lane);
+        epilogue_subtile<PT, true>(acc[2 * half + nbl], b, cbase, pn, poh, pow_, mvalid, lane,
+                                   (p.gap_mask >> bi) & 1u ? p.gap_out : nullptr, p.gap_c, p.tile_p);
       } else {
         any_pooled = true;
       }
@@ -310,9 +364,11 @@
 #pragma unroll
     for (int nbl = 0; nbl < 2; ++nbl) {
       const int sub = n_tile * NB + 2 * half + nbl;
-      const ConvBranch& b = p.br[branch_of(p, sub)];
+      const int bi = branch_of(p, sub);
+      const ConvBranch& b = p.br[bi];
       const int cbase = (sub - b.sub0) * 32;
       if (cbase >= b.Cout || b.avgpool == 0 || !live) continue;
+      const bool gap = ((p.gap_mask >> bi) & 1u) != 0;
       const unsigned gstride = static_cast<unsigned>(b.og.hp * b.og.wp);
       const unsigned obase = static_cast<unsigned>(
           ((n * b.og.groups + b.out_goff) * b.og.hp + y + b.og.halo) * b.og.wp + x + b.og.halo);
@@ -323,7 +379,15 @@
         float o[8];
         avg_pool_group(src, y, x, H, W, lane, inv, b.shift != nullptr ? b.shift + group * 8 : nullptr, o);
         const size_t at = static_cast<size_t>(obase) + static_cast<size_t>(group) * gstride;
-        if (b.out32 != nullptr) {
+        if (gap) {
+#pragma unroll
+          for (int j = 0; j < 8; ++j) o[j] = gap_sum(o[j], p.tile_p);
+          if (pix == 0) {
+            float4* d = reinterpret_cast<float4*>(p.gap_out + static_cast<size_t>(n) * p.gap_c + (b.out_goff + group) * 8);
+            d[0] = make_float4(o[0], o[1], o[2], o[3]);
+            d[1] = make_float4(o[4], o[5], o[6], o[7]);
+          }
+        } else if (b.out32 != nullptr) {
           float4* d = reinterpret_cast<float4*>(b.out32 + at * 8);
           d[0] = make_float4(o[0], o[1], o[2], o[3]);
           d[1] = make_float4(o[4], o[5], o[6], o[7]);
diff --git a/deepvariant_amd/csrc/conv_mfma.hip b/deepvariant_amd/csrc/conv_mfma.hip
--- a/deepvariant_amd/csrc/conv_mfma.hip
+++ b/deepvariant_amd/csrc/conv_mfma.hip
@@ -194,8 +194,9 @@
 }
 
 template <int NB, int PT, int MINB = (NB * PT >= 8 ? 1 : 2), int SLAB = kSlabChunks, int WAVES = 4,
-          bool SPLIT = false, bool SIDE_POOL = false, bool AVG = false, bool WIDE = false>
+          bool SPLIT = false, bool SIDE_POOL = false, bool AVG = false, bool WIDE = false, bool GAP = false>
 __global__ __launch_bounds__(WAVES * 64, MINB) void conv_mfma_kernel(ConvArgs p) {
+  static_assert(!(AVG && GAP), "the AVG kernel takes the global pool at run time (ConvArgs::gap_mpf)");
   constexpr int BN = NB * 32;
   constexpr int kThreads = WAVES * 64;
   constexpr int SLAB_HALFS = SLAB * BN * kChunk;
@@ -238,14 +239,19 @@
   for (int pt = 0; pt < PT; ++pt) {
     const int m = m_block + (wave * PT + pt) * 32 + (lane & 31);
     int n, pix, oh, ow, iy;
-    if constexpr (AVG) {
+    if constexpr (AVG || GAP) {
       int il;
-      divmod_small((wave * PT + pt) * 32 + (lane & 31), p.tile_p, p.rcp_tile_p, il, pix);
+      bool slot_ok = true;
+      if (GAP || p.gap_mpf > 0) {
+        gap_slot(p, (wave * PT + pt) * 32 + (lane & 31), il, pix, slot_ok);
+      } else {
+        divmod_small((wave * PT + pt) * 32 + (lane & 31), p.tile_p, p.rcp_tile_p, il, pix);
+      }
       n = pix_block * p.tile_g + il;
-      mvalid[pt] = il < p.tile_g && n < p.N;
+      mvalid[pt] = slot_ok && il < p.tile_g && n < p.N;
       n = min(n, p.N - 1);
       divmod_small(pix, p.OW, p.rcp_ow, oh, ow);
-      iy = oh * p.stride - p.pad_h + p.ig.halo;
+      iy = GAP && p.band ? p.ig.halo : oh * p.stride - p.pad_h + p.ig.halo;
     } else if (p.band) {
       mvalid[pt] = m < p.N * p.OW;
       divmod_small(mvalid[pt] ? m : 0, p.OW, p.rcp_ow, n, ow);
@@ -426,7 +432,7 @@
   if constexpr (AVG) {
     conv_epilogue_avg<NB, PT>(acc, p, n_tile, pix_block, pn, poh, pow_, mvalid, lane, wave, smem);
   } else {
-    conv_epilogue<NB, PT>(acc, p, n_tile, pn, poh, pow_, mvalid, lane);
+    conv_epilogue<NB, PT, GAP>(acc, p, n_tile, pn, poh, pow_, mvalid, lane);
   }
 }
 
@@ -925,6 +931,31 @@
   }
 }
 
+void launch_conv_gap(const ConvArgs& a, hipStream_t stream) {
+  const long frags = (static_cast<long>(a.N) + a.gap_mpf - 1) / a.gap_mpf;
+  const long rows = a.band ? a.band : 1;
+  auto blocks = [&](int f) { return rows * ((frags + f - 1) / f) * a.n_tiles; };
+  const int pt = blocks(8) >= 512 ? 2 : 1;
+  ConvArgs g = a;
+  g.tile_g = 4 * pt * a.gap_mpf;
+  const dim3 grid(static_cast<unsigned>(blocks(4 * pt)));
+  if (a.wide_in) {
+    if (pt == 2) {
+      hipLaunchKernelGGL((conv_mfma_kernel<4, 2, 2, kSlabChunks, 4, false, false, false, true, true>), grid,
+                         dim3(kConvThreads), conv_lds_bytes<4>(), stream, g);
+    } else {
+      hipLaunchKernelGGL((conv_mfma_kernel<4, 1, 2, kSlabChunks, 4, false, false, false, true, true>), grid,
+                         dim3(kConvThreads), conv_lds_bytes<4>(), stream, g);
+    }
+  } else if (pt == 2) {
+    hipLaunchKernelGGL((conv_mfma_kernel<4, 2, 2, kSlabChunks, 4, false, false, false, false, true>), grid,
+                       dim3(kConvThreads), conv_lds_bytes<4>(), stream, g);
+  } else {
+    hipLaunchKernelGGL((conv_mfma_kernel<4, 1, 2, kSlabChunks, 4, false, false, false, false, true>), grid,
+                       dim3(kConvThreads), conv_lds_bytes<4>(), stream, g);
+  }
+}
+
 }
 namespace dv {
 namespace convk {
@@ -970,6 +1001,10 @@
 }
 
 void launch_conv(const ConvArgs& a, int nb, hipStream_t stream) {
+  if (a.gap_mpf > 0 && a.tile_g == 0) {
+    launch_conv_gap(a, stream);
+    return;
+  }
   switch (nb) {
     case 1: ::launch_conv<1>(a, stream); break;
     case 2: ::launch_conv<2>(a, stream); break;
diff --git a/deepvariant_amd/csrc/model.hip b/deepvariant_amd/csrc/model.hip
--- a/deepvariant_amd/csrc/model.hip
+++ b/deepvariant_amd/csrc/model.hip
@@ -85,6 +85,7 @@
   int shifted_buf, out_example_off;
   size_t images_off;
   std::vector<char> side_pooled;
+  bool gap = false;
   _Float16* out_ptr(int buf) const {
     const size_t halfs = static_cast<size_t>(out_example_off) * m->buffers[buf].bytes_per_example() / 2;
     return m->buf_ptr(buf) + (buf == shifted_buf ? halfs : 0);
@@ -519,8 +520,10 @@
     br.relu = bo.raw ? 0 : 1;
     br.sub0 = subs;
     subs += (bo.cout + 31) / 32;
+    if (ps.gap && bo.gap) a.gap_mask |= 1u << gi;
     if (op.avg_tile_g > 0 && bo.avg_partner >= 0 && bo.avg_partner < ps.last) {
       const Op& pl = m->ops[bo.avg_partner];
+      if (ps.gap && pl.gap) a.gap_mask |= 1u << gi;
       br.avgpool = 1;
       br.shift = m->shift_ptr(pl);
       br.relu = 1;
@@ -530,7 +533,16 @@
       a.rcp_tile_p = 1.0f / static_cast<float>(a.tile_p);
     }
   }
+  if (a.gap_mask != 0) {
+    a.gap_out = static_cast<float*>(m->d_gap.ptr);
+    a.gap_c = m->feat_c;
+    a.gap_mpf = m->gap_mpf;
+    a.tile_p = op.oh * op.ow;
+    a.rcp_tile_p = 1.0f / static_cast<float>(a.tile_p);
+    if (a.tile_g > 0) a.tile_g = 8 * a.gap_mpf;
+  }
   if (a.tile_g > 0) tr_label += " [+ avgpool3s1 in the epilogue, " + std::to_string(a.tile_g) + " maps per block]";
+  if (a.gap_mask != 0) tr_label += " [+ global pool in the epilogue]";
   a.w = m->w_ptr(op);
   const int tiles = (subs + op.nb - 1) / op.nb;
   a.n_tiles = tiles;
@@ -623,8 +635,8 @@
 }
 
 int run_ops(dv_model* m, int first, int last, int n, hipStream_t stream,
-            int shifted_buf = -1, int out_example_off = 0, size_t images_off = 0) {
-  Pass ps{m, n, stream, first, last, shifted_buf, out_example_off, images_off, std::vector<char>(m->ops.size(), 0)};
+            int shifted_buf = -1, int out_example_off = 0, size_t images_off = 0, bool gap = false) {
+  Pass ps{m, n, stream, first, last, shifted_buf, out_example_off, images_off, std::vector<char>(m->ops.size(), 0), gap};
   for (int oi = first; oi < last;) {
     const Op& op = m->ops[oi];
     int ran = 1;
@@ -715,6 +727,10 @@
   if (int rc = m->d_dense_w.reserve(static_cast<size_t>(m->feat_c) * desc->num_classes * 4)) return rc;
   if (int rc = m->d_dense_b.reserve(desc->num_classes * 4)) return rc;
   if (int rc = m->d_ext.reserve(sizeof(ExtPtrs))) return rc;
+  if (m->gap_mpf > 0) {
+    if (int rc = m->d_gap.reserve(static_cast<size_t>(desc->max_batch) * m->feat_c * sizeof(float))) return rc;
+    DV_HIP_CHECK(hipMemset(m->d_gap.ptr, 0, m->d_gap.cap));
+  }
   if (!(getenv("DV_BLANK_SKIP") != nullptr && atoi(getenv("DV_BLANK_SKIP")) == 0) &&
       m->ops[0].first_u8 && m->blank_conv4_op >= 0 && m->ops[m->blank_conv4_op].group_followers == 0 &&
       (static_cast<size_t>(desc->height) * desc->width * desc->channels) % 4 == 0) {
@@ -737,6 +753,7 @@
   m->d_tbl.release();
   m->d_blank_thr.release();
   m->d_ext.release();
+  m->d_gap.release();
   m->d_blank_conv4.release();
   m->d_blank_c2.release();
   m->d_blank_b.release();
@@ -779,7 +796,8 @@
   float* pooled;
   float* logits;
 };
-static int enqueue_forward(dv_model* m, int n, hipStream_t stream, const HeadOutputs* head_out = nullptr);
+static int enqueue_forward(dv_model* m, int n, hipStream_t stream, const HeadOutputs* head_out = nullptr,
+                           bool need_map = false);
 static void set_ext(dv_model* m, const uint8_t* images, float* probs, hipStream_t stream,
                     const int32_t* rows_hint = nullptr, int rows_add = 0) {
   launch_set_ext(ext_table(m), images, probs, rows_hint, rows_add, stream);
@@ -1183,6 +1201,11 @@
   if (host_out) {
     DV_HIP_CHECK(hipSetDevice(m->device));
     DV_HIP_CHECK(hipDeviceSynchronize());
+    if (index == m->feat_buf && m->feat_stale && m->last_n > 0) {
+      if (int rc = run_ops(m, m->gap_first_op, static_cast<int>(m->ops.size()), m->last_n, nullptr)) return rc;
+      DV_HIP_CHECK(hipDeviceSynchronize());
+      m->feat_stale = false;
+    }
     if (b.f32) {
       std::vector<float> tmp(static_cast<size_t>(n) * b.bytes_per_example() / 4);
       DV_HIP_CHECK(hipMemcpy(tmp.data(), m->dbuf[index].ptr, tmp.size() * 4, hipMemcpyDeviceToHost));
@@ -1208,7 +1231,16 @@
   return DV_OK;
 }
 
-static int enqueue_forward(dv_model* m, int n, hipStream_t stream, const HeadOutputs* head_out) {
+static void note_forward(dv_model* m, int n, bool fused) {
+  const int n_parts = (n + m->desc.max_batch - 1) / m->desc.max_batch;
+  const int part = n_parts ? (n + n_parts - 1) / n_parts : 0;
+  m->last_n = n_parts ? n - (n_parts - 1) * part : 0;
+  m->feat_stale = fused;
+}
+
+static int enqueue_forward(dv_model* m, int n, hipStream_t stream, const HeadOutputs* head_out, bool need_map) {
+  const bool fused = m->gap_mpf > 0 && !need_map;
+  note_forward(m, n, fused);
   const size_t img_bytes = static_cast<size_t>(m->desc.height) * m->desc.width * m->desc.channels;
   const ExtPtrs* ext = ext_table(m);
   const int n_parts = (n + m->desc.max_batch - 1) / m->desc.max_batch;
@@ -1233,15 +1265,16 @@
       }
       if (int rc = run_ops(m, 0, m->stem_ops_end, sb, stream, m->stem_out_buf, sb0, img_off)) return rc;
     }
-    if (int rc = run_ops(m, m->stem_ops_end, static_cast<int>(m->ops.size()), nb, stream)) {
+    if (int rc = run_ops(m, m->stem_ops_end, static_cast<int>(m->ops.size()), nb, stream, -1, 0, 0, fused)) {
       return rc;
     }
     {
       dv::ProfileScope prof(dv::kProfOther, stream);
       const bool outs = head_out != nullptr;
-      launch_head(m->buf_ptr<float>(m->feat_buf), static_cast<const float*>(m->d_dense_w.ptr),
+      launch_head(fused ? static_cast<const float*>(m->d_gap.ptr) : m->buf_ptr<float>(m->feat_buf),
+                  static_cast<const float*>(m->d_dense_w.ptr),
                   static_cast<const float*>(m->d_dense_b.ptr), ext, static_cast<size_t>(done) * m->desc.num_classes,
-                  m->buffers[m->feat_buf].geom(), m->desc.num_classes, nb, outs,
+                  m->buffers[m->feat_buf].geom(), m->desc.num_classes, nb, fused, outs,
                   outs && head_out->pooled ? head_out->pooled + static_cast<size_t>(done) * m->feat_c : nullptr,
                   outs && head_out->logits ? head_out->logits + static_cast<size_t>(done) * m->desc.num_classes : nullptr,
                   stream);
@@ -1277,10 +1310,12 @@
     if (op_trace) dump_trace(stream);
     return DV_OK;
   }
+  const bool fused = m->gap_mpf > 0;
   for (const dv_model::GraphEntry& g : m->graphs) {
-    if (g.n == n && g.stream == stream) {
+    if (g.n == n && g.stream == stream && g.gap == fused) {
       DV_HIP_CHECK(hipGraphLaunch(g.exec, stream));
       ++m->graph_replays;
+      note_forward(m, n, fused);
       return DV_OK;
     }
   }
@@ -1295,7 +1330,7 @@
   if (ce != hipSuccess || graph == nullptr) {
     return dv::fail(DV_ERR_HIP, std::string("hipStreamEndCapture: ") + hipGetErrorString(ce));
   }
-  dv_model::GraphEntry e{n, stream, nullptr};
+  dv_model::GraphEntry e{n, stream, nullptr, fused};
   const hipError_t ie = hipGraphInstantiate(&e.exec, graph, nullptr, nullptr, 0);
   (void)hipGraphDestroy(graph);
   if (ie != hipSuccess) {
@@ -1395,6 +1430,7 @@
   if (!m->loaded) return dv::fail(DV_ERR_INVALID_ARGUMENT, "dv_model_infer_outputs: no weights loaded");
   std::vector<OutputView> views(n_outputs);
   HeadOutputs head{nullptr, nullptr};
+  bool need_map = false;
   for (int k = 0; k < n_outputs; ++k) {
     if (int rc = resolve_output(m, names[k], &views[k], "dv_model_infer_outputs")) return rc;
     if (outs[k] == nullptr || reinterpret_cast<uintptr_t>(outs[k]) % 16 != 0) {
@@ -1407,13 +1443,14 @@
       }
     }
     if (views[k].buf < 0) (views[k].logits ? head.logits : head.pooled) = outs[k];
+    need_map = need_map || views[k].buf == m->feat_buf;
   }
   if (n_outputs == 0) return dv_model_infer(m, images, n, probs, stream_v);
   if (n == 0) return DV_OK;
   hipStream_t stream = static_cast<hipStream_t>(stream_v);
   DV_HIP_CHECK(hipSetDevice(m->device));
   set_ext(m, images, probs, stream);
-  if (int rc = enqueue_forward(m, n, stream, &head)) return rc;
+  if (int rc = enqueue_forward(m, n, stream, &head, need_map)) return rc;
   for (int k = 0; k < n_outputs; ++k) {
     const OutputView& v = views[k];
     if (v.buf < 0) continue;
diff --git a/deepvariant_amd/csrc/model_graph.cpp b/deepvariant_amd/csrc/model_graph.cpp
--- a/deepvariant_amd/csrc/model_graph.cpp
+++ b/deepvariant_amd/csrc/model_graph.cpp
@@ -332,6 +332,65 @@
     }
     i += followers;
   }
+}
+
+void dv_model::choose_gap_epilogue() {
+  if (getenv("DV_NO_GAP_EPI") != nullptr || feat_buf < 0) return;
+  const int P = feat_p;
+  if (P < 3 || P > 32 || (32 / P) * P * 100 < 32 * 85) return;
+  for (const Op& o : ops) {
+    if (o.in_buf == feat_buf) return;
+  }
+  std::vector<int> leader(ops.size());
+  for (size_t i = 0; i < ops.size(); ++i) {
+    const int followers = ops[i].type == kOpConv ? ops[i].group_followers : 0;
+    for (int gi = 0; gi <= followers; ++gi) leader[i + gi] = static_cast<int>(i);
+    i += followers;
+  }
+  int pair_raw = -1, pair_pool = -1;
+  for (size_t j = 0; j < ops.size(); ++j) {
+    const Op& pl = ops[j];
+    if (pl.out_buf != feat_buf || pl.type == kOpConv) continue;
+    if (pl.type != kOpAvgPool) return;
+    if (pl.avg_partner >= 0) continue;
+    if (pair_pool >= 0 || !pl.pool_shift_relu || P >= 5 || getenv("DV_NO_AVG_EPI") != nullptr) return;
+    for (size_t i = 0; i < j; ++i) {
+      if (ops[i].type == kOpConv && ops[i].raw && ops[i].out_buf == pl.in_buf && ops[i].avg_partner < 0) pair_raw = static_cast<int>(i);
+    }
+    if (pair_raw < 0) return;
+    const Op& lead = ops[leader[pair_raw]];
+    if (!(lead.kh == 1 && lead.kw == 1 && lead.stride == 1 && lead.nb == 4 && !lead.split && !lead.pool_in && !lead.pool_out &&
+          !lead.v2 && !lead.band && lead.chain_len == 0 && !lead.in_chain && !lead.first_u8 && !lead.stem_a && !lead.stem_b &&
+          lead.avg_tile_g == 0)) {
+      return;
+    }
+    pair_pool = static_cast<int>(j);
+  }
+  int first = -1;
+  for (size_t i = 0; i < ops.size(); ++i) {
+    const Op& c = ops[i];
+    if (c.type != kOpConv) continue;
+    const bool pooled_here = c.raw && (c.avg_partner >= 0 ? ops[c.avg_partner].out_buf == feat_buf : static_cast<int>(i) == pair_raw);
+    if (c.out_buf != feat_buf && !pooled_here) continue;
+    const Op& lead = ops[leader[i]];
+    const bool heads = lead.avg_tile_g > 0 || (pair_raw >= 0 && leader[pair_raw] == leader[i]);
+    const bool plain = lead.group_followers == 0 && c.nb == 4 && c.stride == 1 && !c.split && !c.v2 && c.chain_len == 0 &&
+                       !c.in_chain && !c.pool_in && !c.pool_out && !c.first_u8 && !c.stem_a && !c.stem_b && c.b35 == 0 &&
+                       c.m3 == 0 && c.side_pool_partner < 0 && !c.raw && (c.band == 0 || c.oh == 1);
+    if (!heads && !plain) return;
+    if (first < 0) first = leader[i];
+  }
+  if (first < 0) return;
+  if (pair_raw >= 0) {
+    ops[pair_raw].avg_partner = pair_pool;
+    ops[pair_pool].avg_partner = pair_raw;
+    ops[leader[pair_raw]].avg_tile_g = 256 / P;
+  }
+  for (Op& o : ops) {
+    if (o.out_buf == feat_buf) o.gap = true;
+  }
+  gap_mpf = 32 / P;
+  gap_first_op = first;
 }
 
 void dv_model::choose_chains() {
@@ -644,6 +703,7 @@
   choose_split();
   choose_side_pool();
   choose_avg_epilogue();
+  choose_gap_epilogue();
   choose_block35();
   choose_mixed3();
   for (size_t i = 0; i < ops.size(); ++i) {
diff --git a/deepvariant_amd/csrc/model_graph.h b/deepvariant_amd/csrc/model_graph.h
--- a/deepvariant_amd/csrc/model_graph.h
+++ b/deepvariant_amd/csrc/model_graph.h
@@ -56,6 +56,7 @@
   int side_pool_partner = -1;
   int avg_partner = -1;
   int avg_tile_g = 0;
+  bool gap = false;
   bool pool_out = false;
   int band = 0;
   bool split = false;
@@ -93,6 +94,10 @@
   std::vector<LayerInfo> layers;
   int64_t n_params = 0;
   int feat_buf = -1, feat_p = 0, feat_c = 0;
+  int gap_mpf = 0, gap_first_op = -1;
+  dv::DeviceBuffer d_gap;
+  bool feat_stale = false;
+  int last_n = 0;
   int stem_ops_end = 0, stem_out_buf = -1;
   int stem_a_grid = 512, stem_b_grid = 256;
   int n_cus = 256;
@@ -117,6 +122,7 @@
     int n;
     hipStream_t stream;
     hipGraphExec_t exec;
+    bool gap;
   };
   std::vector<GraphEntry> graphs;
   int64_t graph_captures = 0, graph_replays = 0;
@@ -146,6 +152,7 @@
   void choose_side_pool();
   void choose_split();
   void choose_avg_epilogue();
+  void choose_gap_epilogue();
   void choose_chains();
   void choose_block35();
   void choose_mixed3();
diff --git a/deepvariant_amd/csrc/model_kernels.h b/deepvariant_amd/csrc/model_kernels.h
--- a/deepvariant_amd/csrc/model_kernels.h
+++ b/deepvariant_amd/csrc/model_kernels.h
@@ -53,7 +53,7 @@
 void launch_maxpool3s2(const PoolArgs& p, hipStream_t stream);
 void launch_avgpool3s1(const PoolArgs& p, hipStream_t stream);
 void launch_head(const float* in, const float* w, const float* b, const ExtPtrs* ext, size_t probs_off, TensorGeom g, int K,
-                 int n, bool outputs, float* pooled, float* logits, hipStream_t stream);
+                 int n, bool sums, bool outputs, float* pooled, float* logits, hipStream_t stream);
 
 }
 }
diff --git a/deepvariant_amd/csrc/model_kernels.hip b/deepvariant_amd/csrc/model_kernels.hip
--- a/deepvariant_amd/csrc/model_kernels.hip
+++ b/deepvariant_amd/csrc/model_kernels.hip
@@ -356,7 +356,7 @@
   }
 }
 
-template <bool OUT>
+template <bool OUT, bool POOLED>
 __device__ __forceinline__ void head_body(const float* in, const float* w, const float* b, float* probs, TensorGeom g,
                                           int K, float* pooled, float* logits) {
   __shared__ float red[8][4];
@@ -365,17 +365,35 @@
   const int C = g.groups * 8;
   const size_t plane = static_cast<size_t>(g.hp) * g.wp * 8;
   float part[8] = {0, 0, 0, 0, 0, 0, 0, 0};
-  const float* x = in + static_cast<size_t>(n) * g.groups * plane;
+  const float* x = in + static_cast<size_t>(n) * (POOLED ? static_cast<size_t>(C) : g.groups * plane);
   const float invP = 1.0f / static_cast<float>(g.h * g.w);
   for (int grp = tid; grp * 8 < C; grp += 256) {
     float s[8] = {0, 0, 0, 0, 0, 0, 0, 0};
-    const float4* xg = reinterpret_cast<const float4*>(x + static_cast<size_t>(grp) * plane);
-    for (int y = 0; y < g.h; ++y)
-      for (int xx = 0; xx < g.w; ++xx) {
-        const float4 lo = xg[((y + g.halo) * g.wp + xx + g.halo) * 2], up = xg[((y + g.halo) * g.wp + xx + g.halo) * 2 + 1];
-        s[0] += lo.x; s[1] += lo.y; s[2] += lo.z; s[3] += lo.w;
-        s[4] += up.x; s[5] += up.y; s[6] += up.z; s[7] += up.w;
-      }
+    if constexpr (POOLED) {
+      const float4 lo = reinterpret_cast<const float4*>(x)[grp * 2], up = reinterpret_cast<const float4*>(x)[grp * 2 + 1];
+      s[0] = lo.x; s[1] = lo.y; s[2] = lo.z; s[3] = lo.w;
+      s[4] = up.x; s[5] = up.y; s[6] = up.z; s[7] = up.w;
+    } else {
+      const float4* xg = reinterpret_cast<const float4*>(x + static_cast<size_t>(grp) * plane);
+      for (int y = 0; y < g.h; ++y)
+        for (int x0 = 0; x0 < g.w; x0 += 8) {
+          float4 lo[8], up[8];
+#pragma unroll
+          for (int k = 0; k < 8; ++k) {
+            if (x0 + k < g.w) {
+              lo[k] = xg[((y + g.halo) * g.wp + x0 + k + g.halo) * 2];
+              up[k] = xg[((y + g.halo) * g.wp + x0 + k + g.halo) * 2 + 1];
+            }
+          }
+#pragma unroll
+          for (int k = 0; k < 8; ++k) {
+            if (x0 + k < g.w) {
+              s[0] += lo[k].x; s[1] += lo[k].y; s[2] += lo[k].z; s[3] += lo[k].w;
+              s[4] += up[k].x; s[5] += up[k].y; s[6] += up[k].z; s[7] += up[k].w;
+            }
+          }
+        }
+    }
 #pragma unroll
     for (int j = 0; j < 8; ++j) {
       const float m = s[j] * invP;
@@ -408,13 +426,24 @@
 __global__ __launch_bounds__(256) void head_kernel(const float* in, const float* w,
                                                    const float* b, const ExtPtrs* ext, size_t probs_off,
                                                    TensorGeom g, int K) {
-  head_body<false>(in, w, b, ext->probs + probs_off, g, K, nullptr, nullptr);
+  head_body<false, false>(in, w, b, ext->probs + probs_off, g, K, nullptr, nullptr);
 }
 
 __global__ __launch_bounds__(256) void head_outputs_kernel(const float* in, const float* w, const float* b,
                                                            const ExtPtrs* ext, size_t probs_off, TensorGeom g, int K,
                                                            float* pooled, float* logits) {
-  head_body<true>(in, w, b, ext->probs + probs_off, g, K, pooled, logits);
+  head_body<true, false>(in, w, b, ext->probs + probs_off, g, K, pooled, logits);
+}
+
+__global__ __launch_bounds__(256) void head_pooled_kernel(const float* sums, const float* w, const float* b,
+                                                          const ExtPtrs* ext, size_t probs_off, TensorGeom g, int K) {
+  head_body<false, true>(sums, w, b, ext->probs + probs_off, g, K, nullptr, nullptr);
+}
+
+__global__ __launch_bounds__(256) void head_pooled_outputs_kernel(const float* sums, const float* w, const float* b,
+                                                                  const ExtPtrs* ext, size_t probs_off, TensorGeom g, int K,
+                                                                  float* pooled, float* logits) {
+  head_body<true, true>(sums, w, b, ext->probs + probs_off, g, K, pooled, logits);
 }
 
 }
@@ -470,8 +499,12 @@
 }
 
 void launch_head(const float* in, const float* w, const float* b, const ExtPtrs* ext, size_t probs_off, TensorGeom g, int K,
-                 int n, bool outputs, float* pooled, float* logits, hipStream_t stream) {
-  if (outputs) {
+                 int n, bool sums, bool outputs, float* pooled, float* logits, hipStream_t stream) {
+  if (sums && outputs) {
+    hipLaunchKernelGGL(head_pooled_outputs_kernel, dim3(n), dim3(256), 0, stream, in, w, b, ext, probs_off, g, K, pooled, logits);
+  } else if (sums) {
+    hipLaunchKernelGGL(head_pooled_kernel, dim3(n), dim3(256), 0, stream, in, w, b, ext, probs_off, g, K);
+  } else if (outputs) {
     hipLaunchKernelGGL(head_outputs_kernel, dim3(n), dim3(256), 0, stream, in, w, b, ext, probs_off, g, K, pooled, logits);
   } else {
     hipLaunchKernelGGL(head_kernel, dim3(n), dim3(256), 0, stream, in, w, b, ext, probs_off, g, K);
```

Measured after the change: 512,900 candidates/s, median of 4. Within noise of the previous version (+0.4%).
